# freudh/lbt

Measured on NVIDIA B200. Metric: quantized train imgs/sec, higher is better.
Workload: dtype s8/u8 mantissas, s32 accumulate (8-bit dfxp); fp32 master weights

## Files before the change

### include/lbt.h

```cpp
#ifndef LBT_H_
#define LBT_H_

#include <stddef.h>
#include <stdint.h>

#ifdef __cplusplus
extern "C" {
#endif

#define LBT_VERSION 100

enum lbt_status {
  LBT_OK = 0,
  LBT_EINVAL = -1,
  LBT_EUNSUPPORTED = -2,
  LBT_EARCH = -3,
  LBT_ECUDA = -4,
  LBT_EWORKSPACE = -5
};

enum lbt_round_mode {
  LBT_ROUND_NEAREST = 0,
  LBT_ROUND_STOCHASTIC_NOISE = 1,
  LBT_ROUND_STOCHASTIC_PHILOX = 2,
  LBT_STATS_MINMAX = 0x100
};

enum lbt_mant_kind {
  LBT_MANT_NONE = 0,
  LBT_MANT_S8 = 1,
  LBT_MANT_U8 = 2,
  LBT_MANT_S16 = 3,
  LBT_MANT_S9C3 = 4,
  LBT_MANT_PREPARED = 0x100
};

#define LBT_CNT_OVER 0
#define LBT_CNT_OVER_HALF 1
#define LBT_CNT_NUMEL 2
#define LBT_CNT_TICKET 3
#define LBT_CNT_WORDS 4

int lbt_version(void);
const char* lbt_strerror(int status);
const char* lbt_last_cuda_error(void);
uint64_t lbt_launch_count(void);

int lbt_quantize(const float* x, size_t n_outer, size_t n_inner, int bits, int32_t* integer_bits,
                 float target_overflow_rate, int mode, const float* noise, uint64_t seed,
                 uint64_t offset, const uint64_t* dev_step, float* out_fp32, void* out_mant,
                 int mant_kind, uint64_t* counters, int update_range, void* stream);

int lbt_noise_fill(float* u, size_t n_inner, uint64_t seed, uint64_t offset, const uint64_t* dev_step,
                   void* stream);

int lbt_update_ranges(int32_t* ranges, uint64_t* counters, const int32_t* bits, const float* target,
                      size_t n, void* stream);

int lbt_step_advance(uint64_t* dev_step, void* stream);

typedef struct lbt_qsite {
  int32_t bits;
  int32_t stats_minmax;
  const int32_t* ib;
  const float* noise;
  uint64_t seed, offset;
  const uint64_t* dev_step;
  uint64_t* counters;
} lbt_qsite;

enum lbt_gemm_epilogue {
  LBT_EPI_F32 = 0,
  LBT_EPI_ACC64 = 1
};

int lbt_gemm_i8(const void* A, int a_kind, size_t lda, const void* B, int b_kind, size_t ldb, size_t M,
                size_t N, size_t K, int epilogue, const int32_t* ibA, const int32_t* ibB, int exp_const,
                const float* bias, float* out_f32, int64_t* acc64, size_t ldc, int alpha, int k_splits,
                const lbt_qsite* q_out, int8_t* k_out, int64_t* sums, size_t rows_per_image, const float* addend,
                void* stream);

int lbt_gemm_i8_dual(const int8_t* A_hi, const uint8_t* A_lo, size_t lda, const void* B, int b_kind, size_t ldb, size_t M,
                     size_t N, size_t K, const int32_t* ibA, const int32_t* ibB, int exp_const, float* out_f32, size_t ldc,
                     const float* addend, void* stream);

int lbt_acc64_finalize(const int64_t* acc64, size_t n, const int32_t* ibA, const int32_t* ibB, int exp_const,
                       const float* add, float add_scale, float* out, void* stream);

int lbt_im2col_i8(const void* src, int src_kind, int N, int H, int W, int C, int OH, int OW, int kh, int kw,
                  int sh, int sw, int pad_top, int pad_left, int transposed, void* out, size_t ld,
                  void* stream);

int lbt_conv_i8_fprop(const void* src, int src_kind, int N, int H, int W, int C, const void* wp, int w_kind,
                      size_t ldw, int Cout, int kh, int kw, int sh, int sw, int pad_top, int pad_left, int OH,
                      int OW, const int32_t* ib_src, const int32_t* ib_w, int exp_const, const float* bias,
                      float* out, size_t ldc, const lbt_qsite* q_out, int8_t* k_out, int64_t* sums, const float* addend,
                      void* stream);

int lbt_conv_i8_fprop_dual(const int8_t* src_hi, const uint8_t* src_lo, int N, int H, int W, int C, const void* wp, int w_kind,
                           size_t ldw, int Cout, int kh, int kw, int pad_top, int pad_left, int OH, int OW,
                           const int32_t* ib_src, const int32_t* ib_w, int exp_const, float* out, size_t ldc,
                           const float* addend, void* stream);

int lbt_conv_i8_dgrad(const void* g, int g_kind, int N, int OH, int OW, int Cout, const void* wp, int w_kind,
                      size_t ldw, int Cin, int kh, int kw, int sh, int sw, int pad_top, int pad_left, int H, int W,
                      const int32_t* ib_g, const int32_t* ib_w, int exp_const, float* dx, size_t ldc, const float* addend,
                      void* stream);

int lbt_conv_i8_wgrad(const void* src, int src_kind, int N, int H, int W, int C, const void* g, int g_kind, int Cout,
                      int kh, int kw, int sh, int sw, int pad_top, int pad_left, int OH, int OW, int64_t* acc64,
                      int alpha, int k_splits, void* stream);

int lbt_conv_i8_wgrad_dual(const void* src, int src_kind, int N, int H, int W, int C, const int8_t* g_hi, const uint8_t* g_lo,
                           int Cout, int kh, int kw, int sh, int sw, int pad_top, int pad_left, int OH, int OW,
                           int64_t* acc64, int alpha, int k_splits, void* stream);

size_t lbt_stem_pack8_bytes(int N, int H, int OW);
int lbt_stem_pack8(const int8_t* x16, int N, int H, int W, int OW, int pad_left, int8_t* work8, void* stream);
int lbt_conv_i8_wgrad_c3(const int8_t* x16, int N, int H, int W, const void* g, int g_kind, int Cout, int kh, int kw,
                         int pad_top, int pad_left, int OH, int OW, int8_t* work8, int repack, int64_t* acc8, int alpha,
                         void* stream);

int lbt_split_s16(const int16_t* in, size_t n, int8_t* hi, uint8_t* lo, void* stream);

int lbt_transpose_i8(const void* in, size_t R, size_t C, size_t ld_in, void* out, size_t ld_out,
                     void* stream);

int lbt_colsum_i(const void* in, int kind, size_t R, size_t C, int64_t* acc64, void* stream);

typedef struct lbt_finalize_job {
  const int64_t* acc64;
  uint64_t n;
  const int32_t* ibA;
  const int32_t* ibB;
  int32_t exp_const;
  float add_scale;
  const float* add;
  float* out;
  uint64_t start;
} lbt_finalize_job;
int lbt_finalize_multi(const lbt_finalize_job* jobs_dev, size_t njobs, uint64_t total, void* stream);

typedef struct lbt_noise_job {
  float* u;
  uint64_t n;
  uint64_t offset;
  uint64_t start;
} lbt_noise_job;
int lbt_noise_fill_multi(const lbt_noise_job* jobs_dev, size_t njobs, uint64_t total_groups, uint64_t seed,
                         const uint64_t* dev_step, void* stream);

enum lbt_prep_layout { LBT_PREP_VECTOR = 0, LBT_PREP_CONV = 1, LBT_PREP_DENSE = 2 };
typedef struct lbt_prep_job {
  const float* x;
  uint64_t n_outer, n_inner;
  const int32_t* ib;
  uint64_t* counters;
  uint64_t offset;
  float* out_f32;
  int8_t* out_a;
  int8_t* out_b;
  uint64_t ld_a, ld_b;
  int32_t bits, layout;
  uint32_t kh, kw, Cin, Cout;
  int32_t c3pad, rot180;
  int32_t sh, sw;
} lbt_prep_job;
int lbt_param_prep(const lbt_prep_job* jobs_dev, const uint32_t* block_job_dev, const uint32_t* block_chunk_dev,
                   size_t nblocks, uint32_t chunk_elems, uint64_t seed, const uint64_t* dev_step, void* stream);

int lbt_sgd_momentum(float* w, float* accum, const float* grad, size_t n, float lr, const float* dev_lr,
                     float momentum, float grad_scale, void* stream);

int lbt_bn_fwd_quant_stats(const float* x, size_t n_outer, size_t n_inner, int C, int bits, const int32_t* ib,
                           const float* noise, uint64_t seed, uint64_t offset, const uint64_t* dev_step,
                           int8_t* k1, int64_t* sums, uint64_t* counters, int stats_minmax, void* stream);
int lbt_bn_fwd_apply(const int8_t* k1, size_t n_outer, size_t n_inner, int C, int bits1, const int32_t* ib1,
                     const int64_t* sums, float eps, int bits2, const int32_t* ib2, const float* noise2,
                     uint64_t seed, uint64_t offset2, const uint64_t* dev_step, uint64_t* counters2,
                     const float* gamma_q, const float* beta_q, const float* add, int relu, int8_t* k2,
                     float* out, float* batch_mean, float* batch_var, float* run_mean, float* run_var,
                     double momentum, int stats_minmax, const lbt_qsite* q_next, void* next_mant, int next_kind,
                     void* stream);
int lbt_bn_fwd_apply2(const int8_t* k1, size_t n_outer, size_t n_inner, int C, int bits1, const int32_t* ib1,
                      const int64_t* sums, float eps, int bits2, const int32_t* ib2, const float* noise2,
                      uint64_t seed, uint64_t offset2, const uint64_t* dev_step, uint64_t* counters2,
                      const float* gamma_q, const float* beta_q, const float* add, int relu, int8_t* k2,
                      float* out, float* batch_mean, float* batch_var, float* run_mean, float* run_var,
                      double momentum, int stats_minmax, const lbt_qsite* q_next, void* next_mant, int next_kind,
                      const lbt_qsite* q_next2, void* next_mant2, int next_kind2, void* stream);
int lbt_bn_fwd_apply_pooled(const int8_t* k1, size_t n_outer, int H, int W, int C, int bits1, const int32_t* ib1,
                            const int64_t* sums, float eps, int bits2, const int32_t* ib2, const float* noise2,
                            uint64_t seed, uint64_t offset2, const uint64_t* dev_step, uint64_t* counters2,
                            const float* gamma_q, const float* beta_q, int relu, int8_t* k2, float* run_mean,
                            float* run_var, double momentum, int stats_minmax, int k, int s, int pad_top, int pad_left,
                            int POH, int POW, float* pooled, uint8_t* pidx, const lbt_qsite* q_next, void* next_mant,
                            int next_kind, void* stream);
int lbt_bn_fwd_apply_running(const int8_t* k1, size_t n_outer, size_t n_inner, int C, int bits1, const int32_t* ib1,
                             const float* run_mean, const float* run_var, float eps, int bits2, const int32_t* ib2,
                             const float* noise2, uint64_t seed, uint64_t offset2, const uint64_t* dev_step,
                             uint64_t* counters2, const float* gamma_q, const float* beta_q, const float* add, int relu,
                             int8_t* k2, float* out, int stats_minmax, const lbt_qsite* q_next, void* next_mant,
                             int next_kind, const lbt_qsite* q_next2, void* next_mant2, int next_kind2, void* stream);
int lbt_bn_fwd_apply_running_pooled(const int8_t* k1, size_t n_outer, int H, int W, int C, int bits1, const int32_t* ib1,
                                    const float* run_mean, const float* run_var, float eps, int bits2, const int32_t* ib2,
                                    const float* noise2, uint64_t seed, uint64_t offset2, const uint64_t* dev_step,
                                    uint64_t* counters2, const float* gamma_q, const float* beta_q, int relu, int8_t* k2,
                                    int stats_minmax, int k, int s, int pad_top, int pad_left, int POH, int POW,
                                    float* pooled, uint8_t* pidx, const lbt_qsite* q_next, void* next_mant, int next_kind,
                                    void* stream);
int lbt_bn_bwd_quant_stats(const float* g, const float* out, int relu, const int8_t* k2, const int8_t* k1,
                           size_t n_outer, size_t n_inner, int C, int bits2, const int32_t* ib2,
                           const float* gamma_q, const float* beta_q, int bits_g2, const int32_t* ib_g2,
                           const float* noise_g2, uint64_t offset_g2, uint64_t* counters_g2, int bits_g1,
                           const int32_t* ib_g1, const float* noise_g1, uint64_t offset_g1,
                           uint64_t* counters_g1, uint64_t seed, const uint64_t* dev_step, float* d_add,
                           void* kg1, int64_t* sums, int stats_minmax, int kg1_kind, void* stream);
typedef struct lbt_pool_geom {
  const uint8_t* idx;
  int32_t H, W;
  int32_t k, s, pad_top, pad_left;
  int32_t OH, OW;
} lbt_pool_geom;
int lbt_bn_bwd_quant_stats_pooled(const float* g_pooled, const lbt_pool_geom* pool, int relu, const int8_t* k2,
                                  const int8_t* k1, size_t n_outer, size_t n_inner, int C, int bits2, const int32_t* ib2,
                                  const float* gamma_q, const float* beta_q, int bits_g2, const int32_t* ib_g2,
                                  const float* noise_g2, uint64_t offset_g2, uint64_t* counters_g2, int bits_g1,
                                  const int32_t* ib_g1, const float* noise_g1, uint64_t offset_g1,
                                  uint64_t* counters_g1, uint64_t seed, const uint64_t* dev_step, void* kg1,
                                  int64_t* sums, int stats_minmax, int kg1_kind, void* stream);
int lbt_bn_bwd_apply(const void* kg1, const int8_t* k1, size_t n_outer, size_t n_inner, int C, int bits1,
                     const int32_t* ib1, const int64_t* fwd_sums, float eps, int bits_g1, const int32_t* ib_g1,
                     const int64_t* bwd_sums, float* dx, const lbt_qsite* q_grad, int8_t* g_mant, int kg1_kind,
                     uint8_t* g_mant_lo, void* stream);

typedef struct lbt_bn_bwd_args {
  const float* g;
  const float* out;
  const int8_t* k2;
  const int8_t* k1;
  uint64_t n_outer, n_inner;
  int32_t C, relu;
  int32_t bits2, bits1;
  const int32_t* ib2;
  const int32_t* ib1;
  const float* gamma_q;
  const float* beta_q;
  lbt_qsite q_g2, q_g1;
  float* d_add;
  int64_t* bwd_sums;
  const int64_t* fwd_sums;
  float eps;
  int32_t has_q_grad;
  lbt_qsite q_grad;
  float* dx;
  int8_t* g_mant;
  uint64_t* barrier;
} lbt_bn_bwd_args;
int lbt_bn_bwd_fused(const lbt_bn_bwd_args* args, void* stream);

int lbt_maxpool_fwd(const float* x, int N, int H, int W, int C, int k, int s, int pad_top, int pad_left, int OH, int OW,
                    float* out, uint8_t* idx, void* stream);
int lbt_maxpool_bwd(const float* g, const uint8_t* idx, int N, int H, int W, int C, int k, int s, int pad_top,
                    int pad_left, int OH, int OW, float* dx, void* stream);

int lbt_avgpool_fwd(const float* x, int N, int H, int W, int C, int k, int s, int OH, int OW, float* out, void* stream);
int lbt_avgpool_bwd(const float* g, int N, int H, int W, int C, int k, int s, int OH, int OW, float* dx, void* stream);

int lbt_softmax_xent_fwd(const float* logits, const int64_t* labels, int B, int C, float* probs, float* loss, void* stream);
int lbt_softmax_xent_bwd(const float* probs, const int64_t* labels, const float* grad_loss, int B, int C, float* dlogits,
                         void* stream);

int lbt_relu(const float* x, const float* g, float* out, size_t n, void* stream);
int lbt_dropout(const float* x, const float* u, float keep_prob, uint64_t seed, uint64_t offset, const uint64_t* dev_step,
                float* out, size_t n, void* stream);

#define LBT_DP_MAX_WORLD 8
#define LBT_DP_PAD_READY 0
#define LBT_DP_PAD_DONE 8
#define LBT_DP_PAD_EPOCH 16
#define LBT_DP_PAD_TICKET 17
#define LBT_DP_PAD_ERROR 18
#define LBT_DP_PAD_WORDS 32
#define LBT_DP_HANDLE_BYTES 64
typedef struct lbt_dp_peers {
  int32_t world, rank;
  const float* grad[LBT_DP_MAX_WORLD];
  float* w[LBT_DP_MAX_WORLD];
  const uint64_t* counters[LBT_DP_MAX_WORLD];
  uint32_t* pad[LBT_DP_MAX_WORLD];
} lbt_dp_peers;
int lbt_dp_step(const lbt_dp_peers* peers, float* accum, size_t n, float lr, const float* dev_lr, float momentum,
                int shard, int32_t* ranges, const int32_t* bits, const float* target, size_t n_sites, uint64_t* dev_step,
                void* stream);
int lbt_dp_export(const void* ptr, void* handle64, size_t* offset);
int lbt_dp_open(const void* handle64, void** base);
int lbt_dp_close(void* base);

int lbt_augment_batch(const uint8_t* src, const double* mean, const int64_t* index, int B, int H, int W, int C, int pad,
                      int do_flip, const int32_t* params, uint64_t seed, uint64_t offset, const int64_t* labels,
                      int64_t* labels_out, float* out, void* stream);

int lbt_quantize_residual(const float* grad, size_t n_grad_rows, float* buffer, size_t n_outer, size_t n_inner, int bits,
                          int32_t* integer_bits, int mode, const float* noise, uint64_t seed, uint64_t offset,
                          const uint64_t* dev_step, float* out, uint64_t* counters, void* stream);

typedef struct lbt_bn_bwd_link {
  lbt_qsite q_g2, q_g1;
  int32_t bits2, relu;
  const int32_t* ib2;
  const float* gamma_q;
  const float* beta_q;
  const int8_t* k2;
  const int8_t* k1;
  int8_t* kg1;
  int64_t* sums;
} lbt_bn_bwd_link;
int lbt_conv_i8_dgrad_bn(const void* g, int g_kind, int N, int H, int W, int C, const void* wp, int w_kind, size_t ldw, int Cout,
                         int kh, int kw, int pad_top, int pad_left, int OH, int OW, const int32_t* ib_g, const int32_t* ib_w,
                         int exp_const, const lbt_bn_bwd_link* link, void* stream);

int lbt_conv_i8_dgrad_strided(const void* g, int g_kind, int N, int OH, int OW, int Cout, const void* w2, int w_kind, size_t ldw,
                              int Cin, int kh, int kw, int sh, int sw, int pad_top, int pad_left, int H, int W,
                              const int32_t* ib_g, const int32_t* ib_w, int exp_const, float* dx, size_t ldc,
                              const float* addend, void* stream);
int lbt_conv_i8_dgrad_strided_dual(const int8_t* g_hi, const uint8_t* g_lo, int N, int OH, int OW, int Cout, const void* w2,
                                   int w_kind, size_t ldw, int Cin, int kh, int kw, int sh, int sw, int pad_top, int pad_left,
                                   int H, int W, const int32_t* ib_g, const int32_t* ib_w, int exp_const, float* dx, size_t ldc,
                                   const float* addend, void* stream);

#ifdef __cplusplus
}
#endif
#endif
```

### lbt_b200/_lib.py

```python
import ctypes
import os

import torch

_HERE = os.path.dirname(os.path.abspath(__file__))
LIB_PATH = os.environ.get('LBT_LIB') or os.path.join(_HERE, 'liblbt_b200.so')

c_void_p, c_int, c_size_t, c_float = ctypes.c_void_p, ctypes.c_int, ctypes.c_size_t, ctypes.c_float
c_u64, c_char_p = ctypes.c_uint64, ctypes.c_char_p

SIGNATURES = {
    'lbt_version': (c_int, []),
    'lbt_strerror': (c_char_p, [c_int]),
    'lbt_last_cuda_error': (c_char_p, []),
    'lbt_launch_count': (c_u64, []),
    'lbt_quantize': (c_int, [c_void_p, c_size_t, c_size_t, c_int, c_void_p, c_float, c_int, c_void_p, c_u64, c_u64,
                             c_void_p, c_void_p, c_void_p, c_int, c_void_p, c_int, c_void_p]),
    'lbt_noise_fill': (c_int, [c_void_p, c_size_t, c_u64, c_u64, c_void_p, c_void_p]),
    'lbt_update_ranges': (c_int, [c_void_p, c_void_p, c_void_p, c_void_p, c_size_t, c_void_p]),
    'lbt_step_advance': (c_int, [c_void_p, c_void_p]),
    'lbt_gemm_i8': (c_int, [c_void_p, c_int, c_size_t, c_void_p, c_int, c_size_t, c_size_t, c_size_t, c_size_t, c_int,
                            c_void_p, c_void_p, c_int, c_void_p, c_void_p, c_void_p, c_size_t, c_int, c_int,
                            c_void_p, c_void_p, c_void_p, c_size_t, c_void_p, c_void_p]),
    'lbt_gemm_i8_dual': (c_int, [c_void_p, c_void_p, c_size_t, c_void_p, c_int, c_size_t, c_size_t, c_size_t, c_size_t, c_void_p,
                                 c_void_p, c_int, c_void_p, c_size_t, c_void_p, c_void_p]),
    'lbt_acc64_finalize': (c_int, [c_void_p, c_size_t, c_void_p, c_void_p, c_int, c_void_p, c_float, c_void_p,
                                   c_void_p]),
    'lbt_im2col_i8': (c_int, [c_void_p, c_int] + [c_int] * 13 + [c_void_p, c_size_t, c_void_p]),
    'lbt_conv_i8_fprop': (c_int, [c_void_p, c_int, c_int, c_int, c_int, c_int, c_void_p, c_int, c_size_t] + [c_int] * 9 +
                          [c_void_p, c_void_p, c_int, c_void_p, c_void_p, c_size_t, c_void_p, c_void_p, c_void_p, c_void_p,
                           c_void_p]),
    'lbt_conv_i8_fprop_dual': (c_int, [c_void_p, c_void_p, c_int, c_int, c_int, c_int, c_void_p, c_int, c_size_t] + [c_int] * 7 +
                               [c_void_p, c_void_p, c_int, c_void_p, c_size_t, c_void_p, c_void_p]),
    'lbt_conv_i8_dgrad': (c_int, [c_void_p, c_int, c_int, c_int, c_int, c_int, c_void_p, c_int, c_size_t] + [c_int] * 9 +
                          [c_void_p, c_void_p, c_int, c_void_p, c_size_t, c_void_p, c_void_p]),
    'lbt_conv_i8_wgrad': (c_int, [c_void_p, c_int, c_int, c_int, c_int, c_int, c_void_p, c_int] + [c_int] * 9 +
                          [c_void_p, c_int, c_int, c_void_p]),
    'lbt_conv_i8_wgrad_dual': (c_int, [c_void_p, c_int, c_int, c_int, c_int, c_int, c_void_p, c_void_p] + [c_int] * 9 +
                               [c_void_p, c_int, c_int, c_void_p]),
    'lbt_stem_pack8_bytes': (c_size_t, [c_int, c_int, c_int]),
    'lbt_stem_pack8': (c_int, [c_void_p, c_int, c_int, c_int, c_int, c_int, c_void_p, c_void_p]),
    'lbt_conv_i8_wgrad_c3': (c_int, [c_void_p, c_int, c_int, c_int, c_void_p] + [c_int] * 8 + [c_void_p, c_int, c_void_p, c_int, c_void_p]),
    'lbt_split_s16': (c_int, [c_void_p, c_size_t, c_void_p, c_void_p, c_void_p]),
    'lbt_transpose_i8': (c_int, [c_void_p, c_size_t, c_size_t, c_size_t, c_void_p, c_size_t, c_void_p]),
    'lbt_colsum_i': (c_int, [c_void_p, c_int, c_size_t, c_size_t, c_void_p, c_void_p]),
    'lbt_bn_bwd_fused': (c_int, [c_void_p, c_void_p]),
    'lbt_maxpool_fwd': (c_int, [c_void_p] + [c_int] * 10 + [c_void_p, c_void_p, c_void_p]),
    'lbt_maxpool_bwd': (c_int, [c_void_p, c_void_p] + [c_int] * 10 + [c_void_p, c_void_p]),
    'lbt_avgpool_fwd': (c_int, [c_void_p] + [c_int] * 8 + [c_void_p, c_void_p]),
    'lbt_avgpool_bwd': (c_int, [c_void_p] + [c_int] * 8 + [c_void_p, c_void_p]),
    'lbt_softmax_xent_fwd': (c_int, [c_void_p, c_void_p, c_int, c_int, c_void_p, c_void_p, c_void_p]),
    'lbt_softmax_xent_bwd': (c_int, [c_void_p, c_void_p, c_void_p, c_int, c_int, c_void_p, c_void_p]),
    'lbt_relu': (c_int, [c_void_p, c_void_p, c_void_p, c_size_t, c_void_p]),
    'lbt_dropout': (c_int, [c_void_p, c_void_p, c_float, c_u64, c_u64, c_void_p, c_void_p, c_size_t, c_void_p]),
    'lbt_sgd_momentum': (c_int, [c_void_p, c_void_p, c_void_p, c_size_t, c_float, c_void_p, c_float, c_float,
                                 c_void_p]),
    'lbt_finalize_multi': (c_int, [c_void_p, c_size_t, c_u64, c_void_p]),
    'lbt_noise_fill_multi': (c_int, [c_void_p, c_size_t, c_u64, c_u64, c_void_p, c_void_p]),
    'lbt_param_prep': (c_int, [c_void_p, c_void_p, c_void_p, c_size_t, ctypes.c_uint32, c_u64, c_void_p, c_void_p]),
    'lbt_bn_fwd_quant_stats': (c_int, [c_void_p, c_size_t, c_size_t, c_int, c_int, c_void_p, c_void_p, c_u64, c_u64,
                                       c_void_p, c_void_p, c_void_p, c_void_p, c_int, c_void_p]),
    'lbt_bn_fwd_apply': (c_int, [c_void_p, c_size_t, c_size_t, c_int, c_int, c_void_p, c_void_p, c_float, c_int,
                                 c_void_p, c_void_p, c_u64, c_u64, c_void_p, c_void_p, c_void_p, c_void_p, c_void_p,
                                 c_int, c_void_p, c_void_p, c_void_p, c_void_p, c_void_p, c_void_p, ctypes.c_double, c_int,
                                 c_void_p, c_void_p, c_int, c_void_p]),
    'lbt_bn_fwd_apply2': (c_int, [c_void_p, c_size_t, c_size_t, c_int, c_int, c_void_p, c_void_p, c_float, c_int,
                                  c_void_p, c_void_p, c_u64, c_u64, c_void_p, c_void_p, c_void_p, c_void_p, c_void_p,
                                  c_int, c_void_p, c_void_p, c_void_p, c_void_p, c_void_p, c_void_p, ctypes.c_double, c_int,
                                  c_void_p, c_void_p, c_int, c_void_p, c_void_p, c_int, c_void_p]),
    'lbt_bn_fwd_apply_pooled': (c_int, [c_void_p, c_size_t, c_int, c_int, c_int, c_int, c_void_p, c_void_p, c_float, c_int,
                                        c_void_p, c_void_p, c_u64, c_u64, c_void_p, c_void_p, c_void_p, c_void_p, c_int,
                                        c_void_p, c_void_p, c_void_p, ctypes.c_double, c_int, c_int, c_int, c_int, c_int,
                                        c_int, c_int, c_void_p, c_void_p, c_void_p, c_void_p, c_int, c_void_p]),
    'lbt_bn_fwd_apply_running': (c_int, [c_void_p, c_size_t, c_size_t, c_int, c_int, c_void_p, c_void_p, c_void_p, c_float, c_int,
                                         c_void_p, c_void_p, c_u64, c_u64, c_void_p, c_void_p, c_void_p, c_void_p, c_void_p, c_int,
                                         c_void_p, c_void_p, c_int, c_void_p, c_void_p, c_int, c_void_p, c_void_p, c_int, c_void_p]),
    'lbt_bn_fwd_apply_running_pooled': (c_int, [c_void_p, c_size_t, c_int, c_int, c_int, c_int, c_void_p, c_void_p, c_void_p,
                                                c_float, c_int, c_void_p, c_void_p, c_u64, c_u64, c_void_p, c_void_p, c_void_p,
                                                c_void_p, c_int, c_void_p, c_int, c_int, c_int, c_int, c_int, c_int, c_int,
                                                c_void_p, c_void_p, c_void_p, c_void_p, c_int, c_void_p]),
    'lbt_bn_bwd_quant_stats': (c_int, [c_void_p, c_void_p, c_int, c_void_p, c_void_p, c_size_t, c_size_t, c_int, c_int,
                                       c_void_p, c_void_p, c_void_p, c_int, c_void_p, c_void_p, c_u64, c_void_p, c_int,
                                       c_void_p, c_void_p, c_u64, c_void_p, c_u64, c_void_p, c_void_p, c_void_p,
                                       c_void_p, c_int, c_int, c_void_p]),
    'lbt_bn_bwd_quant_stats_pooled': (c_int, [c_void_p, c_void_p, c_int, c_void_p, c_void_p, c_size_t, c_size_t, c_int, c_int,
                                              c_void_p, c_void_p, c_void_p, c_int, c_void_p, c_void_p, c_u64, c_void_p, c_int,
                                              c_void_p, c_void_p, c_u64, c_void_p, c_u64, c_void_p, c_void_p,
                                              c_void_p, c_int, c_int, c_void_p]),
    'lbt_bn_bwd_apply': (c_int, [c_void_p, c_void_p, c_size_t, c_size_t, c_int, c_int, c_void_p, c_void_p, c_float,
                                 c_int, c_void_p, c_void_p, c_void_p, c_void_p, c_void_p, c_int, c_void_p, c_void_p]),
    'lbt_conv_i8_dgrad_strided_dual': (c_int, [c_void_p, c_void_p, c_int, c_int, c_int, c_int, c_void_p, c_int, c_size_t] + [c_int] * 9 +
                                       [c_void_p, c_void_p, c_int, c_void_p, c_size_t, c_void_p, c_void_p]),
    'lbt_conv_i8_dgrad_strided': (c_int, [c_void_p, c_int, c_int, c_int, c_int, c_int, c_void_p, c_int, c_size_t, c_int, c_int, c_int,
                                          c_int, c_int, c_int, c_int, c_int, c_int, c_void_p, c_void_p, c_int, c_void_p, c_size_t,
                                          c_void_p, c_void_p]),
    'lbt_dp_step': (c_int, [c_void_p, c_void_p, c_size_t, c_float, c_void_p, c_float, c_int, c_void_p, c_void_p, c_void_p,
                            c_size_t, c_void_p, c_void_p]),
    'lbt_dp_export': (c_int, [c_void_p, c_void_p, c_void_p]),
    'lbt_dp_open': (c_int, [c_void_p, c_void_p]),
    'lbt_dp_close': (c_int, [c_void_p]),
    'lbt_conv_i8_dgrad_bn': (c_int, [c_void_p, c_int, c_int, c_int, c_int, c_int, c_void_p, c_int, c_size_t] + [c_int] * 7 +
                             [c_void_p, c_void_p, c_int, c_void_p, c_void_p]),
    'lbt_quantize_residual': (c_int, [c_void_p, c_size_t, c_void_p, c_size_t, c_size_t, c_int, c_void_p, c_int, c_void_p, c_u64,
                                      c_u64, c_void_p, c_void_p, c_void_p, c_void_p]),
    'lbt_augment_batch': (c_int, [c_void_p, c_void_p, c_void_p, c_int, c_int, c_int, c_int, c_int, c_int, c_void_p, c_u64, c_u64,
                                  c_void_p, c_void_p, c_void_p, c_void_p]),
}

_INTERNAL = {
    'lbt_quantize_tune': (c_int, [c_int, c_int]),
    'lbt_gemm_debug_error': (c_int, []),
    'lbt_conv_debug_error': (c_int, []),
    'lbt_conv_ldg_debug_error': (c_int, []),
    'lbt_conv_set_path': (c_int, [c_int]),
    'lbt_conv_set_halo': (c_int, [c_int]),
    'lbt_conv_halo_launches': (ctypes.c_longlong, []),
    'lbt_gemm_set_pair': (c_int, [c_int]),
    'lbt_set_pdl': (c_int, [c_int]),
    'lbt_set_carveout': (c_int, [c_int]),
    'lbt_test_fdiv': (c_int, [c_u64, c_u64, c_void_p, c_void_p, c_void_p]),
    'lbt_bn_set_debug': (c_int, [c_void_p]),
    'lbt_conv_ldg_set_debug': (c_int, [c_void_p]),
    'lbt_dp_tune': (c_int, [c_int]),
    'lbt_dp_emulate_scratch_bytes': (c_size_t, [c_int]),
    'lbt_dp_step_emulate': (c_int, [c_int, c_void_p, c_void_p, c_size_t, c_float, c_void_p, c_float, c_int, c_void_p, c_void_p,
                                    c_void_p, c_size_t, c_void_p, c_void_p, c_void_p]),
    'lbt_bn_debug_error': (c_int, []),
}


class LbtError(RuntimeError):
    pass


class FinalizeJob(ctypes.Structure):
    _fields_ = [('acc64', c_void_p), ('n', c_u64), ('ibA', c_void_p), ('ibB', c_void_p), ('exp_const', ctypes.c_int32),
                ('add_scale', c_float), ('add', c_void_p), ('out', c_void_p), ('start', c_u64)]


class QSiteStruct(ctypes.Structure):
    _fields_ = [('bits', ctypes.c_int32), ('stats_minmax', ctypes.c_int32), ('ib', c_void_p), ('noise', c_void_p),
                ('seed', c_u64), ('offset', c_u64), ('dev_step', c_void_p), ('counters', c_void_p)]


class PoolGeom(ctypes.Structure):
    _fields_ = [('idx', c_void_p), ('H', ctypes.c_int32), ('W', ctypes.c_int32), ('k', ctypes.c_int32), ('s', ctypes.c_int32),
                ('pad_top', ctypes.c_int32), ('pad_left', ctypes.c_int32), ('OH', ctypes.c_int32), ('OW', ctypes.c_int32)]


class BnBwdLink(ctypes.Structure):
    _fields_ = [('q_g2', QSiteStruct), ('q_g1', QSiteStruct), ('bits2', ctypes.c_int32), ('relu', ctypes.c_int32), ('ib2', c_void_p),
                ('gamma_q', c_void_p), ('beta_q', c_void_p), ('k2', c_void_p), ('k1', c_void_p), ('kg1', c_void_p), ('sums', c_void_p)]


class BnBwdArgs(ctypes.Structure):
    _fields_ = [('g', c_void_p), ('out', c_void_p), ('k2', c_void_p), ('k1', c_void_p), ('n_outer', c_u64), ('n_inner', c_u64),
                ('C', ctypes.c_int32), ('relu', ctypes.c_int32), ('bits2', ctypes.c_int32), ('bits1', ctypes.c_int32),
                ('ib2', c_void_p), ('ib1', c_void_p), ('gamma_q', c_void_p), ('beta_q', c_void_p), ('q_g2', QSiteStruct),
                ('q_g1', QSiteStruct), ('d_add', c_void_p), ('bwd_sums', c_void_p), ('fwd_sums', c_void_p), ('eps', c_float),
                ('has_q_grad', ctypes.c_int32), ('q_grad', QSiteStruct), ('dx', c_void_p), ('g_mant', c_void_p),
                ('barrier', c_void_p)]


DP_MAX_WORLD, DP_PAD_WORDS, DP_PAD_ERROR, DP_HANDLE_BYTES = 8, 32, 18, 64


class DpPeers(ctypes.Structure):
    _fields_ = [('world', ctypes.c_int32), ('rank', ctypes.c_int32), ('grad', c_void_p * DP_MAX_WORLD),
                ('w', c_void_p * DP_MAX_WORLD), ('counters', c_void_p * DP_MAX_WORLD), ('pad', c_void_p * DP_MAX_WORLD)]


class NoiseJob(ctypes.Structure):
    _fields_ = [('u', c_void_p), ('n', c_u64), ('offset', c_u64), ('start', c_u64)]


class PrepJob(ctypes.Structure):
    _fields_ = [('x', c_void_p), ('n_outer', c_u64), ('n_inner', c_u64), ('ib', c_void_p), ('counters', c_void_p),
                ('offset', c_u64), ('out_f32', c_void_p), ('out_a', c_void_p), ('out_b', c_void_p), ('ld_a', c_u64),
                ('ld_b', c_u64), ('bits', ctypes.c_int32), ('layout', ctypes.c_int32), ('kh', ctypes.c_uint32),
                ('kw', ctypes.c_uint32), ('Cin', ctypes.c_uint32), ('Cout', ctypes.c_uint32), ('c3pad', ctypes.c_int32),
                ('rot180', ctypes.c_int32), ('sh', ctypes.c_int32), ('sw', ctypes.c_int32)]


def to_device_table(structs, device, keep=None):
    arr = (type(structs[0]) * len(structs))(*structs)
    host = torch.frombuffer(bytearray(bytes(arr)), dtype=torch.uint8).pin_memory()
    if keep is not None:
        keep.append(host)
    return host.to(device, non_blocking=True)


_lib = None


def lib():
    global _lib
    if _lib is None:
        if not os.path.exists(LIB_PATH):
            raise LbtError('%s not found — build it with `python -m lbt_b200.build` (needs nvcc); '
                           'there is no CPU or PyTorch fallback for the DFXP hot path' % LIB_PATH)
        h = ctypes.CDLL(LIB_PATH)
        for table in (SIGNATURES, _INTERNAL):
            for name, (res, args) in table.items():
                fn = getattr(h, name)
                fn.restype, fn.argtypes = res, args
        _lib = h
    return _lib


def check(status):
    if status != 0:
        h = lib()
        msg = h.lbt_strerror(status).decode()
        if status == -4:
            msg += ': ' + h.lbt_last_cuda_error().decode()
        raise LbtError('liblbt_b200: %s (status %d)' % (msg, status))


class Profiler:

    def __init__(self, external=False):
        self.records = []
        self.keep = []
        self.external = external

    def event(self):
        return torch.cuda.Event(enable_timing=True, external=True) if self.external else torch.cuda.Event(enable_timing=True)

    def summary(self):
        torch.cuda.synchronize()
        out = {}
        for name, a, b, meta in self.records:
            d = out.setdefault(name, dict(launches=0, ms=0.0, bytes=0, ops=0))
            d['launches'] += 1
            d['ms'] += a.elapsed_time(b)
            d['bytes'] += (meta or {}).get('bytes', 0)
            d['ops'] += (meta or {}).get('ops', 0)
        return out


profiler = None


def call(name, *args, meta=None):
    fn = getattr(lib(), name)
    if profiler is None:
        check(fn(*args))
        return
    a, b = profiler.event(), profiler.event()
    a.record()
    rc = fn(*args)
    b.record()
    profiler.records.append((name, a, b, meta))
    check(rc)


def try_call(name, *args, meta=None):
    fn = getattr(lib(), name)
    if profiler is None:
        rc = fn(*args)
    else:
        a, b = profiler.event(), profiler.event()
        a.record()
        rc = fn(*args)
        b.record()
        if rc == 0:
            profiler.records.append((name, a, b, meta))
        else:
            profiler.keep.append((a, b))
    if rc == -2:
        return False
    check(rc)
    return True


def ptr(t):
    if t is None:
        return None
    if not t.is_cuda:
        raise LbtError('lbt_b200 operates on CUDA tensors only (no CPU fallback); got a %s tensor' % t.device)
    return t.data_ptr()


def stream():
    return torch.cuda.current_stream().cuda_stream


def launch_count():
    return int(lib().lbt_launch_count())
```

### lbt_b200/csrc/conv_dgrad.cu

```cuda
#include "conv_classes.h"
#include "conv_internal.h"
#include "common.cuh"

namespace lbt {
namespace {

__global__ void __launch_bounds__(256) dgrad_fill_kernel(float* __restrict__ out, const float* __restrict__ addend, uint32_t Hc,
                                                          uint32_t Wc, uint32_t c4, long long sn, long long sy, long long sx,
                                                          size_t total) {
  pdl_trigger();
  pdl_wait();
  for (size_t i = (size_t)blockIdx.x * 256 + threadIdx.x; i < total; i += (size_t)gridDim.x * 256) {
    const uint32_t c = (uint32_t)(i % c4);
    size_t t = i / c4;
    const uint32_t x = (uint32_t)(t % Wc);
    t /= Wc;
    const uint32_t y = (uint32_t)(t % Hc), n = (uint32_t)(t / Hc);
    const long long o = (long long)n * sn + (long long)y * sy + (long long)x * sx + 4ll * c;
    const float4 v = addend ? __ldcs(reinterpret_cast<const float4*>(addend + o)) : make_float4(0.f, 0.f, 0.f, 0.f);
    *reinterpret_cast<float4*>(out + o) = v;
  }
}

}
}

using namespace lbt;

static int dgrad_strided_run(const void* g, int g_kind, const void* g_lo, int N, int OH, int OW, int Cout, const void* w2, int w_kind,
                             size_t ldw, int Cin, int kh, int kw, int sh, int sw, int pad_top, int pad_left, int H, int W,
                             const int32_t* ib_g, const int32_t* ib_w, int exp_const, float* dx, size_t ldc,
                             const float* addend, void* stream) {
  if (!g || !w2 || !dx) return LBT_EINVAL;
  if ((g_kind != LBT_MANT_S8 && g_kind != LBT_MANT_U8)) return LBT_EINVAL;
  if (g_lo && (g_kind != LBT_MANT_S8 || Cin < 64 || (Cout != 64 && Cout % 128))) return LBT_EUNSUPPORTED;
  if (N <= 0 || H <= 0 || W <= 0 || Cin <= 0 || Cout <= 0 || kh <= 0 || kw <= 0 || sh <= 0 || sw <= 0 || OH <= 0 || OW <= 0)
    return LBT_EINVAL;
  if (pad_top < 0 || pad_left < 0 || ldc < (size_t)Cin || ldw < (size_t)kh * kw * Cout) return LBT_EINVAL;
  if (sh > 4 || sw > 4 || (Cout & 15) || (Cin & 3) || (ldc & 3) || (reinterpret_cast<uintptr_t>(dx) & 15) ||
      (addend && (reinterpret_cast<uintptr_t>(addend) & 15)))
    return LBT_EUNSUPPORTED;
  for (int a = 0; a < sh; ++a) {
    const int r0 = (a + pad_top) % sh, nr = class_count(r0, kh, sh);
    if (nr && nr - 1 - (a + pad_top) / sh < 0) return LBT_EUNSUPPORTED;
  }
  for (int b = 0; b < sw; ++b) {
    const int s0 = (b + pad_left) % sw, nc = class_count(s0, kw, sw);
    if (nc && nc - 1 - (b + pad_left) / sw < 0) return LBT_EUNSUPPORTED;
  }
  LBT_REQUIRE_ARCH();
  cudaStream_t st = reinterpret_cast<cudaStream_t>(stream);
  for (int a = 0; a < sh && a < H; ++a)
    for (int b = 0; b < sw && b < W; ++b) {
      const int Hc = (H - a + sh - 1) / sh, Wc = (W - b + sw - 1) / sw;
      const int r0 = (a + pad_top) % sh, s0 = (b + pad_left) % sw;
      const int nr = class_count(r0, kh, sh), nc = class_count(s0, kw, sw);
      OutRemap rm{(long long)H * W * (long long)ldc, (long long)sh * W * (long long)ldc, (long long)sw * (long long)ldc};
      float* out = dx + ((size_t)a * W + b) * ldc;
      const float* ad = addend ? addend + ((size_t)a * W + b) * ldc : nullptr;
      if (nr == 0 || nc == 0) {
        const size_t total = (size_t)N * Hc * Wc * (Cin / 4);
        const size_t blocks = (total + 255) / 256, cap = (size_t)device_info().sm_count * 8;
        launch_pdl(dgrad_fill_kernel, (unsigned)(blocks < cap ? blocks : cap), 256, 0, st, out, ad, (uint32_t)Hc, (uint32_t)Wc,
                   (uint32_t)(Cin / 4), rm.sn, rm.sy, rm.sx, total);
        const int rc = check_launch("lbt_conv_i8_dgrad_strided (fill)");
        if (rc) return rc;
        continue;
      }
      const int pt2 = nr - 1 - (a + pad_top) / sh, pl2 = nc - 1 - (b + pad_left) / sw;
      const uint8_t* wp = reinterpret_cast<const uint8_t*>(w2) + (size_t)class_group_offset(r0, s0, kh, kw, sh, sw) * Cout;
      const int rc = conv_fprop_run(g, g_kind, N, OH, OW, Cout, wp, w_kind, ldw, Cin, nr, nc, 1, 1, pt2, pl2, Hc, Wc, ib_g, ib_w,
                                    exp_const, nullptr, out, ldc, nullptr, nullptr, nullptr, ad, stream, &rm, g_lo);
      if (rc) return rc;
    }
  return LBT_OK;
}

extern "C" int lbt_conv_i8_dgrad_strided(const void* g, int g_kind, int N, int OH, int OW, int Cout, const void* w2, int w_kind,
                                         size_t ldw, int Cin, int kh, int kw, int sh, int sw, int pad_top, int pad_left, int H, int W,
                                         const int32_t* ib_g, const int32_t* ib_w, int exp_const, float* dx, size_t ldc,
                                         const float* addend, void* stream) {
  return dgrad_strided_run(g, g_kind, nullptr, N, OH, OW, Cout, w2, w_kind, ldw, Cin, kh, kw, sh, sw, pad_top, pad_left, H, W, ib_g, ib_w,
                           exp_const, dx, ldc, addend, stream);
}

extern "C" int lbt_conv_i8_dgrad_strided_dual(const int8_t* g_hi, const uint8_t* g_lo, int N, int OH, int OW, int Cout, const void* w2,
                                              int w_kind, size_t ldw, int Cin, int kh, int kw, int sh, int sw, int pad_top, int pad_left,
                                              int H, int W, const int32_t* ib_g, const int32_t* ib_w, int exp_const, float* dx, size_t ldc,
                                              const float* addend, void* stream) {
  if (!g_lo) return LBT_EINVAL;
  return dgrad_strided_run(g_hi, LBT_MANT_S8, g_lo, N, OH, OW, Cout, w2, w_kind, ldw, Cin, kh, kw, sh, sw, pad_top, pad_left, H, W, ib_g,
                           ib_w, exp_const, dx, ldc, addend, stream);
}
```

### lbt_b200/csrc/conv_i8.cu

```cuda
#include "conv_internal.h"
#include "qsite.cuh"
#include "tcgen05.cuh"

namespace lbt {
namespace {

using namespace tc;

constexpr int kBlockM = 128;
constexpr int kStageK = 128;
constexpr int kThreads = 192;
constexpr int kEpiWarps = 8;
constexpr int kThreadsF = 32 * (2 + kEpiWarps);

__device__ int g_conv_error = 0;

struct ConvParams {
  uint32_t M, N;
  uint32_t OW, OHW;
  FastDiv d_OW, d_OHW;
  int lower_w, lower_h;
  int sw, sh;
  uint32_t kw;
  uint32_t taps, cchunks;
  uint32_t ksteps;
  uint32_t ksteps_real;
  uint32_t cb;
  uint32_t mode;
  uint32_t C;
  uint32_t m_tiles, n_tiles;
  const int32_t* ibA;
  const int32_t* ibB;
  int exp_const;
  const float* bias;
  const float* addend;
  float* out;
  size_t ldc;
  uint32_t idesc;
  uint32_t idesc2;
  BnqParams bnq;
  int remap;
  long long rs_n, rs_y, rs_x;
};

template <int BN>
struct Cfg {
  static constexpr int kStageA = kBlockM * kStageK;
  static constexpr int kStageB = BN * kStageK;
  static constexpr int kStageBytes = kStageA + kStageB;
  static constexpr int kCtasPerSm = BN <= 16 ? 3 : (BN <= 128 ? 2 : 1);
  static constexpr int kStages = BN <= 64 ? 4 : (BN == 128 ? 3 : 4);
  static constexpr int kSmemBytes = kStages * kStageBytes + 1024;
  static constexpr int kAccStages = BN <= 64 ? 4 : 2;
  static constexpr int kTmemCols = (kAccStages * BN) < 32 ? 32 : (kAccStages * BN);
  static_assert(kCtasPerSm * kSmemBytes <= 227 * 1024, "shared memory budget");
  static_assert(kCtasPerSm * kTmemCols <= 512, "tensor memory budget");
};

inline int ctas_per_sm(int bn) { return bn <= 16 ? 3 : (bn <= 128 ? 2 : 1); }

template <int BN, bool DUAL>
struct FCfg {
  static constexpr int kStageA = Cfg<BN>::kStageA;
  static constexpr int kStageB = Cfg<BN>::kStageB;
  static constexpr int kStageBytes = (DUAL ? 2 : 1) * kStageA + kStageB;
  static constexpr int kCtasPerSm = DUAL ? 1 : Cfg<BN>::kCtasPerSm;
  static constexpr int kStages = DUAL ? ((226 * 1024) / kStageBytes > 4 ? 4 : (226 * 1024) / kStageBytes) : Cfg<BN>::kStages;
  static constexpr int kSmemBytes = kStages * kStageBytes + 1024;
  static constexpr int kAccW = (DUAL ? 2 : 1) * BN;
  static constexpr int kAccStages = DUAL ? (512 / kAccW > 4 ? 4 : 512 / kAccW) : Cfg<BN>::kAccStages;
  static constexpr int kTmemCols = (kAccStages * kAccW) < 32 ? 32 : (kAccStages * kAccW);
  static_assert(kStages >= 2 && kAccStages >= 1, "fprop ring");
  static_assert(kCtasPerSm * kSmemBytes <= 227 * 1024, "shared memory budget");
  static_assert(kCtasPerSm * kTmemCols <= 512, "tensor memory budget");
};

template <int BN, bool DUAL>
struct WCfg {
  static constexpr int kStageA = Cfg<BN>::kStageA;
  static constexpr int kStageB1 = Cfg<BN>::kStageB;
  static constexpr int kStageBytes = kStageA + (DUAL ? 2 : 1) * kStageB1;
  static constexpr int kCtasPerSm = Cfg<BN>::kCtasPerSm;
  static constexpr int kBudget = (227 * 1024) / kCtasPerSm - 1024;
  static constexpr int kStages = !DUAL ? Cfg<BN>::kStages : (kBudget / kStageBytes > 4 ? 4 : kBudget / kStageBytes);
  static constexpr int kSmemBytes = kStages * kStageBytes + 1024;
  static constexpr int kAccW = (DUAL ? 2 : 1) * BN;
  static constexpr int kAccStages = !DUAL ? Cfg<BN>::kAccStages : ((512 / kCtasPerSm) / kAccW > 4 ? 4 : (512 / kCtasPerSm) / kAccW);
  static constexpr int kTmemCols = (kAccStages * kAccW) < 32 ? 32 : (kAccStages * kAccW);
  static_assert(kStages >= 2 && kAccStages >= 1, "wgrad ring");
  static_assert(kCtasPerSm * kSmemBytes <= 227 * 1024, "shared memory budget");
  static_assert(kCtasPerSm * kTmemCols <= 512, "tensor memory budget");
};

template <int BN, bool DUAL = false>
__global__ void __launch_bounds__(kThreadsF, FCfg<BN, DUAL>::kCtasPerSm)
conv_fprop_kernel(const __grid_constant__ CUtensorMap tmA, const __grid_constant__ CUtensorMap tmA2, const __grid_constant__ CUtensorMap tmB,
                  const ConvParams p) {
  using C = FCfg<BN, DUAL>;
  extern __shared__ uint8_t smem_raw[];
  uint8_t* smem = reinterpret_cast<uint8_t*>((reinterpret_cast<uintptr_t>(smem_raw) + 1023) & ~uintptr_t(1023));
  __shared__ __align__(8) uint64_t full_bar[C::kStages];
  __shared__ __align__(8) uint64_t empty_bar[C::kStages];
  __shared__ __align__(8) uint64_t tmem_full_bar[C::kAccStages];
  __shared__ __align__(8) uint64_t tmem_empty_bar[C::kAccStages];
  __shared__ uint32_t tmem_slot;
  __shared__ int s_abort;
  __shared__ int s_stat[kEpiWarps][2 * BN];
  __shared__ unsigned long long s_tot[2 * BN];

  const int warp = threadIdx.x >> 5, lane = threadIdx.x & 31;
  if (threadIdx.x == 0) {
    for (int s = 0; s < C::kStages; ++s) {
      mbar_init(&full_bar[s], 1);
      mbar_init(&empty_bar[s], 1);
    }
    for (int s = 0; s < C::kAccStages; ++s) {
      mbar_init(&tmem_full_bar[s], 1);
      mbar_init(&tmem_empty_bar[s], kEpiWarps);
    }
    s_abort = 0;
    fence_barrier_init();
    tma_prefetch_desc(&tmA);
    if (DUAL) tma_prefetch_desc(&tmA2);
    tma_prefetch_desc(&tmB);
  }
  if (warp == 1) tmem_alloc(&tmem_slot, C::kTmemCols);
  for (uint32_t i = threadIdx.x; i < 2 * BN; i += kThreadsF) s_tot[i] = 0ull;
  pdl_trigger();
  fence_before();
  __syncthreads();
  fence_after();
  pdl_wait();
  const uint32_t tmem_base = *reinterpret_cast<volatile uint32_t*>(&tmem_slot);
  volatile int* abort_flag = &s_abort;

  const uint32_t total_tiles = p.m_tiles * p.n_tiles;
  const uint32_t spb = kStageK / p.cb;
  const uint32_t a_block = kBlockM * p.cb, b_block = BN * p.cb;
  const uint32_t nstages_k = (p.ksteps + spb - 1) / spb;

  if (warp == 0) {
    if (lane == 0) {
      uint32_t stage = 0, phase = 0;
      bool ok = true;
      for (uint32_t tile = blockIdx.x; tile < total_tiles && ok; tile += gridDim.x) {
        const uint32_t m_tile = tile % p.m_tiles, n_tile = tile / p.m_tiles;
        const uint32_t m0 = m_tile * kBlockM;
        const uint32_t img = fastdiv(m0, p.d_OHW), rem = m0 - img * p.OHW;
        const uint32_t ohu = fastdiv(rem, p.d_OW);
        const int oh = (int)ohu, ow = (int)(rem - ohu * p.OW);
        const int base_w = p.lower_w + ow * p.sw, base_h = p.lower_h + oh * p.sh;
        uint32_t cc = 0, r = 0, s = 0;
        for (uint32_t ks = 0; ks < nstages_k; ++ks) {
          if (!(ok = mbar_wait(&empty_bar[stage], phase ^ 1, abort_flag, &g_conv_error))) break;
          uint8_t* sa = smem + stage * C::kStageBytes;
          uint8_t* sb = sa + (DUAL ? 2 : 1) * C::kStageA;
          const uint32_t k0 = ks * spb;
          const uint32_t nblk = min(spb, p.ksteps - k0);
          mbar_expect_tx(&full_bar[stage], nblk * ((DUAL ? 2u : 1u) * a_block + b_block));
          for (uint32_t j = 0; j < nblk; ++j) {
            const uint32_t kstep = k0 + j;
            const bool pad = kstep >= p.ksteps_real;
            tma_load_im2col_4d(&tmA, &full_bar[stage], sa + j * a_block, pad ? 0 : (int)(cc * p.cb), base_w, base_h, (int)img,
                               (uint16_t)(pad ? 0u : s), (uint16_t)(pad ? 0u : r));
            if (DUAL)
              tma_load_im2col_4d(&tmA2, &full_bar[stage], sa + C::kStageA + j * a_block, pad ? 0 : (int)(cc * p.cb), base_w, base_h,
                                 (int)img, (uint16_t)(pad ? 0u : s), (uint16_t)(pad ? 0u : r));
            tma_load_2d(&tmB, &full_bar[stage], sb + j * b_block, (int)(kstep * p.cb), (int)(n_tile * BN));
            if (++cc == p.cchunks) {
              cc = 0;
              if (++s == p.kw) {
                s = 0;
                ++r;
              }
            }
          }
          if (++stage == C::kStages) {
            stage = 0;
            phase ^= 1;
          }
        }
      }
    }
  } else if (warp == 1) {
    if (lane == 0) {
      uint32_t stage = 0, phase = 0, acc = 0, acc_phase = 0;
      bool ok = true;
      for (uint32_t tile = blockIdx.x; tile < total_tiles && ok; tile += gridDim.x) {
        if (!(ok = mbar_wait(&tmem_empty_bar[acc], acc_phase ^ 1, abort_flag, &g_conv_error))) break;
        fence_after();
        const uint32_t d_tmem = tmem_base + acc * C::kAccW;
        uint32_t first = 1;
        for (uint32_t ks = 0; ks < nstages_k; ++ks) {
          if (!(ok = mbar_wait(&full_bar[stage], phase, abort_flag, &g_conv_error))) break;
          fence_after();
          const uint32_t sa = smem_u32(smem + stage * C::kStageBytes);
          const uint32_t sb = sa + (DUAL ? 2 : 1) * C::kStageA;
          const uint32_t nblk = min(spb, p.ksteps - ks * spb);
          if (p.mode == 0) {
            for (uint32_t j = 0; j < nblk; j += 2) {
              const uint64_t db = make_desc_kmajor(sb + j * b_block, 0, b_block);
              umma_i8(d_tmem, make_desc_kmajor(sa + j * a_block, 0, a_block), db, p.idesc, first ? 0u : 1u);
              if (DUAL) umma_i8(d_tmem + BN, make_desc_kmajor(sa + C::kStageA + j * a_block, 0, a_block), db, p.idesc2, first ? 0u : 1u);
              first = 0;
            }
          } else {
            const uint32_t per_block = p.cb / 32;
            for (uint32_t j = 0; j < nblk; ++j)
              for (uint32_t kk = 0; kk < per_block; ++kk) {
                const uint64_t db = make_desc_kmajor(sb + j * b_block + kk * 32, (int)p.mode, 16);
                umma_i8(d_tmem, make_desc_kmajor(sa + j * a_block + kk * 32, (int)p.mode, 16), db, p.idesc, first ? 0u : 1u);
                if (DUAL)
                  umma_i8(d_tmem + BN, make_desc_kmajor(sa + C::kStageA + j * a_block + kk * 32, (int)p.mode, 16), db, p.idesc2,
                          first ? 0u : 1u);
                first = 0;
              }
          }
          umma_commit(&empty_bar[stage]);
          if (++stage == C::kStages) {
            stage = 0;
            phase ^= 1;
          }
        }
        if (!ok) break;
        umma_commit(&tmem_full_bar[acc]);
        if (++acc == C::kAccStages) {
          acc = 0;
          acc_phase ^= 1;
        }
      }
    }
  } else {
    const uint32_t quad = warp & 3;
    const uint32_t half = (uint32_t)(warp - 2) >> 2;
    int e = p.exp_const;
    if (p.ibA) e += *p.ibA;
    if (p.ibB) e += *p.ibB;
    const float scale = exp2i(e);
    const bool fused = p.bnq.q.bits != 0;
    int* my_stat = s_stat[warp - 2];
    BnqState bst;
    bst.tiles = 0;
    uint32_t stat_ntile = 0;
    if (fused) {
      bst.init(p.bnq);
      for (int i = lane; i < 2 * BN; i += 32) my_stat[i] = 0;
      __syncwarp();
    }
    uint32_t acc = 0, acc_phase = 0;
    bool ok = true;
    for (uint32_t tile = blockIdx.x; tile < total_tiles && ok; tile += gridDim.x) {
      const uint32_t m_tile = tile % p.m_tiles, n_tile = tile / p.m_tiles;
      const uint32_t row = m_tile * kBlockM + quad * 32 + lane;
      const uint32_t pix = fused ? row % p.bnq.rows_per_image : 0u;
      const uint32_t col0 = n_tile * BN;
      if (fused) {
#pragma unroll 1
        for (int c = (BN > 16 ? 16 * (int)half : 0); c < BN; c += (BN > 16 ? 32 : 16))
          bnq_prefetch(p.bnq, pix, p.N, col0 + (uint32_t)c, row < p.M && col0 + (uint32_t)c < p.N && !(BN == 16 && half));
      }
      ok = mbar_wait(&tmem_full_bar[acc], acc_phase, abort_flag, &g_conv_error);
      ok = __all_sync(0xffffffffu, ok);
      if (!ok) break;
      fence_after();
      const uint32_t taddr = tmem_base + acc * C::kAccW + ((quad * 32u) << 16);
      if (fused && (n_tile != stat_ntile || bst.tiles >= (uint32_t)kBnqFlushTiles)) {
        bnq_flush(p.bnq, my_stat, stat_ntile * BN, BN, p.N, lane);
        stat_ntile = n_tile;
        bst.tiles = 0;
      }
#pragma unroll 1
      for (int c = (BN > 16 ? 16 * (int)half : 0); c < BN; c += (BN > 16 ? 32 : 16)) {
        if (BN == 16 && half) break;
        uint32_t v[16];
        float4 u4[4];
        const bool fchunk = fused && col0 + c < p.N;
        if (BN > 16 && fchunk) bnq_load_noise(p.bnq, bst, pix, row < p.M, col0 + c, min(16u, p.N - (col0 + c)), p.N, u4);
        tmem_ld16(taddr + c, v);
        uint32_t w[DUAL ? 16 : 1];
        if constexpr (DUAL) tmem_ld16(taddr + BN + c, w);
        tmem_ld_wait();
        if (BN <= 16 && fchunk)
          bnq_load_noise(p.bnq, bst, pix, row < p.M, col0 + c, min(16u, p.N - (col0 + c)), p.N, u4);
        if (fused) {
          if (fchunk) {
            const uint32_t ncol = min(16u, p.N - (col0 + c));
            bnq_chunk(p.bnq, bst, v, u4, scale, p.bias ? p.bias + col0 + c : nullptr, row, row < p.M, col0 + c, ncol, p.N, my_stat, BN,
                      (uint32_t)c, lane);
          }
        } else if (row < p.M && col0 + c < p.N) {
          const uint32_t ncol = min(16u, p.N - (col0 + c));
          float* o;
          if (p.remap) {
            const uint32_t img = fastdiv(row, p.d_OHW), rem = row - img * p.OHW;
            const uint32_t oh = fastdiv(rem, p.d_OW), ow = rem - oh * p.OW;
            o = p.out + ((long long)img * p.rs_n + (long long)oh * p.rs_y + (long long)ow * p.rs_x) + col0 + c;
          } else {
            o = p.out + (size_t)row * p.ldc + col0 + c;
          }
          float f[16];
#pragma unroll
          for (int j = 0; j < 16; ++j) {
// ... 330 lines not shown
  if (!dual && !remap && conv_ldg_enabled() && (C <= 32 || (C == 64 && conv_ldg_c64_halo() && conv_ldg_halo_applies(N, OH, OW, kh, kw, sh, sw, C))) &&
      conv_ldg_ok(C, Cout, kh, kw) && !(reinterpret_cast<uintptr_t>(src) & 15) &&
      !(reinterpret_cast<uintptr_t>(wp) & 15) && !(ldw & 15) && ldw >= (size_t)kh * kw * C && (q_out || ldc >= (size_t)Cout)) {
    LBT_REQUIRE_ARCH();
    return conv_ldg_run(src, src_kind, N, H, W, C, wp, w_kind, ldw, Cout, kh, kw, sh, sw, pad_top, pad_left, OH, OW, 0, ib_src,
                        ib_w, exp_const, bias, out, ldc, q_out, k_out, sums, addend, stream, nullptr, w_prepared);
  }
  const uint32_t cb = C >= 128 ? 128u : (uint32_t)C;
  if (cb != 16 && cb != 32 && cb != 64 && cb != 128) return LBT_EUNSUPPORTED;
  if (C % cb) return LBT_EUNSUPPORTED;
  if ((reinterpret_cast<uintptr_t>(src) & 15) || (reinterpret_cast<uintptr_t>(wp) & 15) || (ldw & 15)) return LBT_EUNSUPPORTED;
  if (!q_out && ldc < (size_t)Cout) return LBT_EINVAL;
  const size_t Ktot = (size_t)kh * kw * C;
  if (ldw < Ktot) return LBT_EINVAL;
  if (conv_halo_applies(N, OH, OW, C, Cout, kh, kw, sh, sw)) {
    LBT_REQUIRE_ARCH();
    const int rc = conv_halo_run(src, src_kind, N, H, W, C, wp, w_kind, ldw, Cout, kh, kw, pad_top, pad_left, OH, OW, ib_src, ib_w,
                                 exp_const, bias, out, ldc, q_out, k_out, sums, addend, stream, remap, src_lo);
    if (!(dual && rc == LBT_EUNSUPPORTED)) return rc;
  }
  if (Ktot > 65536) return LBT_EUNSUPPORTED;
  if (kh > 255 || kw > 255) return LBT_EUNSUPPORTED;
  LBT_REQUIRE_ARCH();
  const DeviceInfo& di = device_info();
  static EncodeTiledFn enc_tiled = reinterpret_cast<EncodeTiledFn>(driver_fn("cuTensorMapEncodeTiled"));
  static EncodeIm2colFn enc_im2col = reinterpret_cast<EncodeIm2colFn>(driver_fn("cuTensorMapEncodeIm2col"));
  if (!enc_tiled || !enc_im2col) return LBT_ECUDA;

  int bn = 256;
  for (int c : {16, 32, 64, 128, 256})
    if (c >= Cout) {
      bn = c;
      break;
    }
  if (dual && bn > 128) bn = 128;
  if (dual && bn < 64) return LBT_EUNSUPPORTED;
  uint32_t mode = 0;
  while ((16u << mode) < cb) ++mode;

  ConvParams p{};
  p.M = (uint32_t)((size_t)N * OH * OW);
  p.N = (uint32_t)Cout;
  p.OW = (uint32_t)OW;
  p.OHW = (uint32_t)(OH * OW);
  p.d_OW = make_fastdiv(p.OW);
  p.d_OHW = make_fastdiv(p.OHW);
  if ((size_t)N * OH * OW >= (1ull << 31)) return LBT_EUNSUPPORTED;
  p.lower_w = -pad_left;
  p.lower_h = -pad_top;
  p.sw = sw;
  p.sh = sh;
  p.kw = (uint32_t)kw;
  p.taps = (uint32_t)(kh * kw);
  p.cchunks = (uint32_t)C / cb;
  p.ksteps_real = p.taps * p.cchunks;
  p.ksteps = p.ksteps_real + ((cb == 16 && (p.ksteps_real & 1)) ? 1 : 0);
  p.cb = cb;
  p.mode = mode;
  p.C = (uint32_t)C;
  p.m_tiles = (p.M + kBlockM - 1) / kBlockM;
  p.n_tiles = ((uint32_t)Cout + bn - 1) / bn;
  p.ibA = ib_src;
  p.ibB = ib_w;
  p.exp_const = exp_const;
  p.bias = bias;
  p.addend = q_out ? nullptr : addend;
  p.out = out;
  p.ldc = ldc;
  p.idesc = tc::make_idesc_i8(src_kind == LBT_MANT_S8, w_kind == LBT_MANT_S8, false, false, bn, kBlockM);
  p.idesc2 = tc::make_idesc_i8(false, w_kind == LBT_MANT_S8, false, false, bn, kBlockM);
  p.bnq.q = site_from_abi(q_out);
  p.bnq.k = k_out;
  p.bnq.sums = reinterpret_cast<long long*>(sums);
  p.bnq.rows_per_image = (uint32_t)(OH * OW);
  if (remap) {
    p.remap = 1;
    p.rs_n = remap->sn;
    p.rs_y = remap->sy;
    p.rs_x = remap->sx;
  }

  CUtensorMap ta, ta2, tb;
  {
    cuuint64_t gdim[4] = {(cuuint64_t)C, (cuuint64_t)W, (cuuint64_t)H, (cuuint64_t)N};
    cuuint64_t gstr[3] = {(cuuint64_t)C, (cuuint64_t)W * C, (cuuint64_t)H * W * C};
    const int upper_w = (OW - 1) * sw + 1 - W - pad_left;
    const int upper_h = (OH - 1) * sh + 1 - H - pad_top;
    int lower[2] = {-pad_left, -pad_top};
    int upper[2] = {upper_w, upper_h};
    cuuint32_t estr[4] = {1, (cuuint32_t)sw, (cuuint32_t)sh, 1};
    CUresult r = enc_im2col(&ta, CU_TENSOR_MAP_DATA_TYPE_UINT8, 4, const_cast<void*>(src), gdim, gstr, lower, upper, cb, kBlockM,
                            estr, CU_TENSOR_MAP_INTERLEAVE_NONE, swizzle_of(mode), CU_TENSOR_MAP_L2_PROMOTION_L2_128B,
                            CU_TENSOR_MAP_FLOAT_OOB_FILL_NONE);
    if (r != CUDA_SUCCESS) {
      set_cuda_error(cudaErrorInvalidValue, "cuTensorMapEncodeIm2col");
      return LBT_ECUDA;
    }
    ta2 = ta;
    if (dual) {
      r = enc_im2col(&ta2, CU_TENSOR_MAP_DATA_TYPE_UINT8, 4, const_cast<void*>(src_lo), gdim, gstr, lower, upper, cb, kBlockM,
                     estr, CU_TENSOR_MAP_INTERLEAVE_NONE, swizzle_of(mode), CU_TENSOR_MAP_L2_PROMOTION_L2_128B,
                     CU_TENSOR_MAP_FLOAT_OOB_FILL_NONE);
      if (r != CUDA_SUCCESS) {
        set_cuda_error(cudaErrorInvalidValue, "cuTensorMapEncodeIm2col(low plane)");
        return LBT_ECUDA;
      }
    }
  }
  {
    cuuint64_t gdim[2] = {(cuuint64_t)Ktot, (cuuint64_t)Cout};
    cuuint64_t gstr[1] = {(cuuint64_t)ldw};
    cuuint32_t box[2] = {cb, (cuuint32_t)bn};
    cuuint32_t estr[2] = {1, 1};
    CUresult r = enc_tiled(&tb, CU_TENSOR_MAP_DATA_TYPE_UINT8, 2, const_cast<void*>(wp), gdim, gstr, box, estr,
                           CU_TENSOR_MAP_INTERLEAVE_NONE, swizzle_of(mode), CU_TENSOR_MAP_L2_PROMOTION_L2_256B,
                           CU_TENSOR_MAP_FLOAT_OOB_FILL_NONE);
    if (r != CUDA_SUCCESS) {
      set_cuda_error(cudaErrorInvalidValue, "cuTensorMapEncodeTiled(weights)");
      return LBT_ECUDA;
    }
  }
  const uint64_t tiles = (uint64_t)p.m_tiles * p.n_tiles;
  const uint64_t cap = (uint64_t)di.sm_count * (dual ? 1 : ctas_per_sm(bn));
  const unsigned grid = (unsigned)(tiles < cap ? tiles : cap);
  cudaStream_t st = reinterpret_cast<cudaStream_t>(stream);
  if (dual) return bn == 64 ? launch<64, true>(ta, ta2, tb, p, grid, st) : launch<128, true>(ta, ta2, tb, p, grid, st);
  switch (bn) {
    case 16: return launch<16>(ta, ta2, tb, p, grid, st);
    case 32: return launch<32>(ta, ta2, tb, p, grid, st);
    case 64: return launch<64>(ta, ta2, tb, p, grid, st);
    case 128: return launch<128>(ta, ta2, tb, p, grid, st);
    default: return launch<256>(ta, ta2, tb, p, grid, st);
  }
}

namespace lbt {
namespace {
template <int BN, bool DUAL = false>
int launch_wgrad(const CUtensorMap& tx, const CUtensorMap& tg, const CUtensorMap& tg2, const WgradParams& p, unsigned grid, cudaStream_t st) {
  static bool attr_done[16] = {};
  const int dev = device_info().device;
  if (!attr_done[dev]) {
    cudaError_t e = cudaFuncSetAttribute(conv_wgrad_kernel<BN, DUAL>, cudaFuncAttributeMaxDynamicSharedMemorySize, WCfg<BN, DUAL>::kSmemBytes);
    if (e != cudaSuccess) {
      set_cuda_error(e, "cudaFuncSetAttribute(conv_wgrad_kernel)");
      return LBT_ECUDA;
    }
    attr_done[dev] = true;
  }
  launch_pdl(conv_wgrad_kernel<BN, DUAL>, grid, kThreads, WCfg<BN, DUAL>::kSmemBytes, st, tx, tg, tg2, p);
  return check_launch(DUAL ? "lbt_conv_i8_wgrad_dual" : "lbt_conv_i8_wgrad");
}
}
}

static int conv_wgrad_run(const void* src, int src_kind, int N, int H, int W, int C, const void* g, int g_kind, const void* g_lo, int Cout,
                          int kh, int kw, int sh, int sw, int pad_top, int pad_left, int OH, int OW, int64_t* acc64,
                          int alpha, int k_splits, void* stream) {
  const bool dual = g_lo != nullptr;
  if (!src || !g || !acc64) return LBT_EINVAL;
  if (dual && (g_kind != LBT_MANT_S8 || (reinterpret_cast<uintptr_t>(g_lo) & 15))) return LBT_EUNSUPPORTED;
  if ((src_kind != LBT_MANT_S8 && src_kind != LBT_MANT_U8) || (g_kind != LBT_MANT_S8 && g_kind != LBT_MANT_U8)) return LBT_EINVAL;
  if (N <= 0 || H <= 0 || W <= 0 || C <= 0 || Cout <= 0 || kh <= 0 || kw <= 0 || sh <= 0 || sw <= 0 || OH <= 0 || OW <= 0)
    return LBT_EINVAL;
  const uint32_t cb = C >= 128 ? 128u : (uint32_t)C;
  const uint32_t cbn = Cout >= 128 ? 128u : (uint32_t)Cout;
  if ((cb != 16 && cb != 32 && cb != 64 && cb != 128) || (C % cb)) return LBT_EUNSUPPORTED;
  if ((cbn != 16 && cbn != 32 && cbn != 64 && cbn != 128) || (Cout % cbn)) return LBT_EUNSUPPORTED;
  if ((reinterpret_cast<uintptr_t>(src) & 15) || (reinterpret_cast<uintptr_t>(g) & 15)) return LBT_EUNSUPPORTED;
  if (kh > 255 || kw > 255) return LBT_EUNSUPPORTED;
  LBT_REQUIRE_ARCH();
  if (!dual && conv_ldg_enabled() && k_splits <= 0 && C == 16 && Cout <= 16 && conv_wgrad_ldg_ok(C, Cout, kh, kw)) {
    const int rc = conv_wgrad_ldg_run(src, src_kind, N, H, W, C, g, g_kind, Cout, kh, kw, sh, sw, pad_top, pad_left, OH, OW, acc64,
                                      alpha, stream);
    if (rc != LBT_EUNSUPPORTED) return rc;
  }
  const DeviceInfo& di = device_info();
  static EncodeTiledFn enc_tiled = reinterpret_cast<EncodeTiledFn>(driver_fn("cuTensorMapEncodeTiled"));
  static EncodeIm2colFn enc_im2col = reinterpret_cast<EncodeIm2colFn>(driver_fn("cuTensorMapEncodeIm2col"));
  if (!enc_tiled || !enc_im2col) return LBT_ECUDA;

  int bn = Cout >= 256 ? 256 : Cout;
  if (Cout > 128 && Cout % 256) bn = 128;
  if (dual && bn > 128) bn = 128;
  uint32_t mode_a = 0, mode_b = 0;
  while ((16u << mode_a) < cb) ++mode_a;
  while ((16u << mode_b) < cbn) ++mode_b;

  WgradParams p{};
  p.Mpix = (uint32_t)((size_t)N * OH * OW);
  p.N = (uint32_t)Cout;
  p.OW = (uint32_t)OW;
  p.OHW = (uint32_t)(OH * OW);
  p.d_OW = make_fastdiv(p.OW);
  p.d_OHW = make_fastdiv(p.OHW);
  if ((size_t)N * OH * OW >= (1ull << 31)) return LBT_EUNSUPPORTED;
  p.lower_w = -pad_left;
  p.lower_h = -pad_top;
  p.sw = sw;
  p.sh = sh;
  p.kw = (uint32_t)kw;
  p.cchunks = (uint32_t)C / cb;
  p.ksteps = (uint32_t)(kh * kw) * p.cchunks;
  p.cb = cb;
  p.mode_a = mode_a;
  p.cbn = cbn;
  p.mode_b = mode_b;
  p.nchunks = (uint32_t)bn / cbn;
  const uint32_t spb = kStageK / cb;
  p.m_tiles = (p.ksteps + spb - 1) / spb;
  p.n_tiles = ((uint32_t)Cout + bn - 1) / bn;
  p.pix_blocks = (p.Mpix + kBlockM - 1) / kBlockM;
  uint32_t splits = k_splits > 0 ? (uint32_t)k_splits : 0;
  if (!splits) {
    const uint32_t tiles = p.m_tiles * p.n_tiles;
    splits = (uint32_t)(di.sm_count * ctas_per_sm(bn)) / (tiles ? tiles : 1);
    if (splits > p.pix_blocks / 8) splits = p.pix_blocks / 8;
    if (splits < 1) splits = 1;
  }
  if (splits > p.pix_blocks) splits = p.pix_blocks;
  p.blocks_per_split = (p.pix_blocks + splits - 1) / splits;
  if (p.blocks_per_split > 65536 / kBlockM) p.blocks_per_split = 65536 / kBlockM;
  p.k_splits = (p.pix_blocks + p.blocks_per_split - 1) / p.blocks_per_split;
  p.Kf = (uint32_t)(kh * kw * C);
  p.acc64 = reinterpret_cast<long long*>(acc64);
  p.alpha = alpha;
  p.idesc = tc::make_idesc_i8(src_kind == LBT_MANT_S8, g_kind == LBT_MANT_S8, true, true, bn, kBlockM);
  p.idesc2 = tc::make_idesc_i8(src_kind == LBT_MANT_S8, false, true, true, bn, kBlockM);

  CUtensorMap tx, tg, tg2;
  {
    cuuint64_t gdim[4] = {(cuuint64_t)C, (cuuint64_t)W, (cuuint64_t)H, (cuuint64_t)N};
    cuuint64_t gstr[3] = {(cuuint64_t)C, (cuuint64_t)W * C, (cuuint64_t)H * W * C};
    int lower[2] = {-pad_left, -pad_top};
    int upper[2] = {(OW - 1) * sw + 1 - W - pad_left, (OH - 1) * sh + 1 - H - pad_top};
    cuuint32_t estr[4] = {1, (cuuint32_t)sw, (cuuint32_t)sh, 1};
    CUresult r = enc_im2col(&tx, CU_TENSOR_MAP_DATA_TYPE_UINT8, 4, const_cast<void*>(src), gdim, gstr, lower, upper, cb, kBlockM,
                            estr, CU_TENSOR_MAP_INTERLEAVE_NONE, swizzle_of(mode_a), CU_TENSOR_MAP_L2_PROMOTION_L2_128B,
                            CU_TENSOR_MAP_FLOAT_OOB_FILL_NONE);
    if (r != CUDA_SUCCESS) {
      set_cuda_error(cudaErrorInvalidValue, "cuTensorMapEncodeIm2col(wgrad)");
      return LBT_ECUDA;
    }
  }
  {
    cuuint64_t gdim[2] = {(cuuint64_t)Cout, (cuuint64_t)p.Mpix};
    cuuint64_t gstr[1] = {(cuuint64_t)Cout};
    cuuint32_t box[2] = {cbn, (cuuint32_t)kBlockM};
    cuuint32_t estr[2] = {1, 1};
    CUresult r = enc_tiled(&tg, CU_TENSOR_MAP_DATA_TYPE_UINT8, 2, const_cast<void*>(g), gdim, gstr, box, estr,
                           CU_TENSOR_MAP_INTERLEAVE_NONE, swizzle_of(mode_b), CU_TENSOR_MAP_L2_PROMOTION_L2_128B,
                           CU_TENSOR_MAP_FLOAT_OOB_FILL_NONE);
    if (r != CUDA_SUCCESS) {
      set_cuda_error(cudaErrorInvalidValue, "cuTensorMapEncodeTiled(grad)");
      return LBT_ECUDA;
    }
    tg2 = tg;
    if (dual) {
      r = enc_tiled(&tg2, CU_TENSOR_MAP_DATA_TYPE_UINT8, 2, const_cast<void*>(g_lo), gdim, gstr, box, estr,
                    CU_TENSOR_MAP_INTERLEAVE_NONE, swizzle_of(mode_b), CU_TENSOR_MAP_L2_PROMOTION_L2_128B,
                    CU_TENSOR_MAP_FLOAT_OOB_FILL_NONE);
      if (r != CUDA_SUCCESS) {
        set_cuda_error(cudaErrorInvalidValue, "cuTensorMapEncodeTiled(grad, low plane)");
        return LBT_ECUDA;
      }
    }
  }
  const uint64_t items = (uint64_t)p.m_tiles * p.n_tiles * p.k_splits;
  const uint64_t cap = (uint64_t)di.sm_count * ctas_per_sm(bn);
  const unsigned grid = (unsigned)(items < cap ? items : cap);
  cudaStream_t st = reinterpret_cast<cudaStream_t>(stream);
  if (dual) {
    switch (bn) {
      case 16: return launch_wgrad<16, true>(tx, tg, tg2, p, grid, st);
      case 32: return launch_wgrad<32, true>(tx, tg, tg2, p, grid, st);
      case 64: return launch_wgrad<64, true>(tx, tg, tg2, p, grid, st);
      default: return launch_wgrad<128, true>(tx, tg, tg2, p, grid, st);
    }
  }
  switch (bn) {
    case 16: return launch_wgrad<16>(tx, tg, tg2, p, grid, st);
    case 32: return launch_wgrad<32>(tx, tg, tg2, p, grid, st);
    case 64: return launch_wgrad<64>(tx, tg, tg2, p, grid, st);
    case 128: return launch_wgrad<128>(tx, tg, tg2, p, grid, st);
    default: return launch_wgrad<256>(tx, tg, tg2, p, grid, st);
  }
}

extern "C" int lbt_conv_i8_wgrad(const void* src, int src_kind, int N, int H, int W, int C, const void* g, int g_kind, int Cout,
                                 int kh, int kw, int sh, int sw, int pad_top, int pad_left, int OH, int OW, int64_t* acc64,
                                 int alpha, int k_splits, void* stream) {
  return conv_wgrad_run(src, src_kind, N, H, W, C, g, g_kind, nullptr, Cout, kh, kw, sh, sw, pad_top, pad_left, OH, OW, acc64, alpha,
                        k_splits, stream);
}

extern "C" int lbt_conv_i8_wgrad_dual(const void* src, int src_kind, int N, int H, int W, int C, const int8_t* g_hi, const uint8_t* g_lo,
                                      int Cout, int kh, int kw, int sh, int sw, int pad_top, int pad_left, int OH, int OW,
                                      int64_t* acc64, int alpha, int k_splits, void* stream) {
  if (!g_lo) return LBT_EINVAL;
  return conv_wgrad_run(src, src_kind, N, H, W, C, g_hi, LBT_MANT_S8, g_lo, Cout, kh, kw, sh, sw, pad_top, pad_left, OH, OW, acc64,
                        alpha, k_splits, stream);
}

extern "C" int lbt_conv_debug_error(void) {
  int v = 0, zero = 0;
  if (cudaMemcpyFromSymbol(&v, g_conv_error, sizeof(int)) != cudaSuccess) return -1;
  cudaMemcpyToSymbol(g_conv_error, &zero, sizeof(int));
  const int h = conv_halo_debug_error();
  if (h > 0) v |= h;
  const int st = conv_stem_debug_error();
  if (st > 0) v |= st;
  return v;
}
```

### lbt_b200/csrc/conv_internal.h

```cpp
#pragma once

#include <stddef.h>
#include <stdint.h>

#include "../../include/lbt.h"

namespace lbt {

struct OutRemap {
  long long sn, sy, sx;
};

bool conv_ldg_ok(int C, int Cout, int kh, int kw);
bool conv_ldg_enabled();
bool conv_ldg_halo_applies(int N, int OH, int OW, int kh, int kw, int sh, int sw, int C);
int conv_ldg_c64_halo();
int conv_ldg_run(const void* src, int src_kind, int N, int SH, int SW, int C, const void* wp, int w_kind, size_t ldw, int Cout,
                 int kh, int kw, int sh, int sw, int pt, int pl, int OH, int OW, int gather, const int32_t* ibA,
                 const int32_t* ibB, int exp_const, const float* bias, float* out, size_t ldc, const lbt_qsite* q_out,
                 int8_t* k_out, int64_t* sums, const float* addend, void* stream, const lbt_bn_bwd_link* link = nullptr,
                 bool w_prepared = false);

bool conv_halo_applies(int N, int OH, int OW, int C, int Cout, int kh, int kw, int sh, int sw);
void conv_halo_enable(int mode);
int conv_halo_debug_error();
int conv_stem_debug_error();
int conv_halo_run(const void* src, int src_kind, int N, int H, int W, int C, const void* wp, int w_kind, size_t ldw, int Cout, int kh,
                  int kw, int pt, int pl, int OH, int OW, const int32_t* ibA, const int32_t* ibB, int exp_const, const float* bias,
                  float* out, size_t ldc, const lbt_qsite* q_out, int8_t* k_out, int64_t* sums, const float* addend, void* stream,
                  const OutRemap* remap = nullptr, const void* src_lo = nullptr);
int conv_fprop_run(const void* src, int src_kind, int N, int H, int W, int C, const void* wp, int w_kind, size_t ldw, int Cout, int kh,
                   int kw, int sh, int sw, int pad_top, int pad_left, int OH, int OW, const int32_t* ib_src, const int32_t* ib_w,
                   int exp_const, const float* bias, float* out, size_t ldc, const lbt_qsite* q_out, int8_t* k_out, int64_t* sums,
                   const float* addend, void* stream, const OutRemap* remap, const void* src_lo = nullptr);

bool conv_wgrad_ldg_ok(int C, int Cout, int kh, int kw);
int conv_wgrad_ldg_run(const void* src, int src_kind, int N, int H, int W, int C, const void* g, int g_kind, int Cout, int kh, int kw,
                       int sh, int sw, int pt, int pl, int OH, int OW, int64_t* acc64, int alpha, void* stream);

}
```

### lbt_b200/dfxp.py

```python
import contextlib
import ctypes
import os
import math

import torch
import torch.nn as nn

from . import _lib, gemm as G, quantizer as Q




class Runtime:

    def __init__(self, seed=0):
        self.seed = int(seed)
        self.sites = []
        self.dev_step = None
        self.noise_fn = None
        self.flat = None
        self.grad_sink = None
        self.prep = None
        self._arena = None
        self._arena_off = 0
# ... 287 lines not shown
            n_inner = Q.rows_view(x)[1]
            kw.update(mode=Q.ROUND_NOISE, noise=rt.noise_fn(self, n_inner, x.device))
        else:
            kw.update(mode=Q.ROUND_PHILOX, seed=rt.seed, offset=Q.make_offset(self.qid, 0), dev_step=rt.dev_step)
        if self.target == 0.0:
            kw['mode'] |= Q.STATS_MINMAX
        return Q.quantize(x, self.bits, self.range, **kw)

    def abi(self, n_inner, device, arena=False):
        rt = self.runtime
        qs = _lib.QSiteStruct(bits=self.bits, stats_minmax=int(self.target == 0.0), ib=self.range.data_ptr(),
                              noise=0, seed=rt.seed, offset=Q.make_offset(self.qid, 0),
                              dev_step=_lib.ptr(rt.dev_step) or 0, counters=self.counters.data_ptr())
        if rt.noise_fn is not None:
            nz = rt.noise_fn(self, n_inner, device).contiguous()
            qs.noise, qs.offset = nz.data_ptr(), 0
            qs._keep = nz
        elif arena:
            nz = rt.noise_for(self, n_inner, device)
            if nz is not None:
                qs.noise = nz.data_ptr()
        return qs

    def extra_repr(self):
        return '%s bits=%d' % (self.name, self.bits)


class _QuantSTE(torch.autograd.Function):

    @staticmethod
    def forward(ctx, x, site):
        q, _ = site.quantize(x)
        return q

    @staticmethod
    def backward(ctx, dy):
        return dy, None


class _GradQuant(torch.autograd.Function):

    @staticmethod
    def forward(ctx, y, site):
        ctx.site = site
        return y.view_as(y)

    @staticmethod
    def backward(ctx, dy):
        dy = _mem_contig(dy)
        q, _ = ctx.site.quantize(dy)
        return q, None


def _require_cuda_f32(x, who):
    if not x.is_cuda or x.dtype != torch.float32:
        raise _lib.LbtError('%s: expects an fp32 CUDA tensor (got %s on %s); there is no CPU or PyTorch fallback'
                            % (who, x.dtype, x.device))


def _mem_contig(x):
    if x.dim() == 4:
        return x if x.is_contiguous(memory_format=torch.channels_last) else x.contiguous(memory_format=torch.channels_last)
    return x.contiguous()


def same_pad(in_size, k, s):
    out = -(-in_size // s)
    total = max((out - 1) * s + k - in_size, 0)
    return out, total // 2, total - total // 2


def _pitch16(k):
    return -(-k // 16) * 16


def _as_operand(t):
    rows, K = t.shape
    if t.stride(1) == 1 and t.stride(0) % 16 == 0 and t.data_ptr() % 16 == 0:
        return t
    buf = torch.zeros(rows, _pitch16(K), dtype=t.dtype, device=t.device)
    buf[:, :K] = t
    return buf[:, :K]


def _transpose_bytes(t):
    R, C = t.shape
    assert t.stride(1) == 1
    out = torch.empty(C, _pitch16(R), dtype=t.dtype, device=t.device)
    _lib.call('lbt_transpose_i8', _lib.ptr(t), R, C, t.stride(0), _lib.ptr(out), out.stride(0), _lib.stream())
    return out[:, :R]


def _im2col(src_nhwc, src_kind, OH, OW, kh, kw, sh, sw, pt, pl, transposed):
    N, H, W, C = src_nhwc.shape
    segs = 3 if src_kind == Q.MANT_S16 else 1
    K = kh * kw * C * segs
    M = N * OH * OW
    out = torch.empty(M, _pitch16(K), dtype=torch.int8 if src_kind != Q.MANT_U8 else torch.uint8, device=src_nhwc.device)
    _lib.call('lbt_im2col_i8', _lib.ptr(src_nhwc), src_kind, N, H, W, C, OH, OW, kh, kw, sh, sw, pt, pl,
                                        1 if transposed else 0, _lib.ptr(out), out.stride(0), _lib.stream())
    return out[:, :K]


def _colsum(mant2d, kind, rt=None):
    acc = (rt.zeros_i64(mant2d.shape[1], mant2d.device) if rt is not None
           else torch.zeros(mant2d.shape[1], dtype=torch.int64, device=mant2d.device))
    _lib.call('lbt_colsum_i', _lib.ptr(mant2d), kind, mant2d.shape[0], mant2d.shape[1], _lib.ptr(acc),
                                       _lib.stream())
    return acc


def _implicit_ok(C, kh, kw):
    return (C in (16, 32, 64) or (C >= 128 and C % 128 == 0)) and kh * kw * C <= 65536 and kh <= 255 and kw <= 255


def _gather_ok(C, Cout, kh, kw):
    if C not in (16, 32, 64) or not 1 <= Cout <= 128:
        return False
    kcp = (kh * kw * (C // 16) + 1) & ~1
    bn = 16 if Cout <= 16 else (32 if Cout <= 32 else (64 if Cout <= 64 else 128))
    return kcp * bn * 16 + 2 * 16384 + 1024 <= 200 * 1024 and kh * kw * C <= 65536 and kcp <= 256 and kh * kw <= 64 and kh <= 16 and kw <= 16


def _class_perm(kh, kw, sh, sw):
    perm = []
    for r0 in range(sh):
        for s0 in range(sw):
            for r in reversed(range(r0, kh, sh)):
                for s_ in reversed(range(s0, kw, sw)):
                    perm.append(r * kw + s_)
    return perm


DGRAD_CLASSES = True


def _dgrad_classes_ok(layer, Cin, Cout, kh, kw, sh, sw):
    if layer.qG.bits > 8:
        return (DGRAD_CLASSES and DUAL_HALO and layer.implicit and (sh, sw) != (1, 1) and sh <= 4 and sw <= 4 and layer.qG.bits <= 16 and
                layer.qW.bits <= 8 and (Cout == 64 or Cout % 128 == 0) and Cin >= 64 and Cin % 4 == 0)
    return (DGRAD_CLASSES and layer.implicit and (sh, sw) != (1, 1) and sh <= 4 and sw <= 4 and layer.qG.bits <= 8 and
            layer.qW.bits <= 8 and (Cout in (16, 32, 64) or Cout % 128 == 0) and Cin % 4 == 0 and
            not _gather_ok(Cout, Cin, kh, kw))


FUSE_POOL_FWD = os.environ.get('LBT_FUSE_POOL_FWD', '1') != '0'

STEM_WGRAD = os.environ.get('LBT_STEM_WGRAD', '1') != '0'

_W_PREPARED = 0x100 if os.environ.get('LBT_W_PREFETCH', '0') == '1' else 0


def _conv_implicit(src_nhwc, src_kind, wp, Cout, kh, kw, sh, sw, pt, pl, OH, OW, ib_src, ib_w, exp_const, bias, out2d,
                   bnq=None, addend=None, w_prepared=False):
    N, H, W, C = src_nhwc.shape
    qs, k_out, sums = bnq if bnq is not None else (None, None, None)
    _lib.call('lbt_conv_i8_fprop', _lib.ptr(src_nhwc), src_kind, N, H, W, C, _lib.ptr(wp), Q.MANT_S8 | (_W_PREPARED if w_prepared else 0),
              wp.stride(0), Cout,
              kh, kw, sh, sw, pt, pl, OH, OW, _lib.ptr(ib_src), _lib.ptr(ib_w), int(exp_const), _lib.ptr(bias),
              _lib.ptr(out2d), out2d.stride(0) if out2d is not None else Cout,
              ctypes.addressof(qs) if qs is not None else None, _lib.ptr(k_out), _lib.ptr(sums), _lib.ptr(addend), _lib.stream(),
              meta=dict(ops=2 * N * OH * OW * Cout * kh * kw * C,
                        bytes=N * H * W * C + Cout * kh * kw * C + N * OH * OW * Cout * (1 if qs is not None else 4)))




def _conv_geom(layer, x, weight):
    N, Cin, H, W = x.shape
    kh, kw, _, Cout = weight.shape
    sh, sw = layer.stride
    if layer.padding == 'SAME':
        OH, pt, _ = same_pad(H, kh, sh)
        OW, pl, _ = same_pad(W, kw, sw)
    else:
        pt = pl = layer.pad_int
        OH = (H + 2 * pt - kh) // sh + 1
        OW = (W + 2 * pl - kw) // sw + 1
    return (N, H, W, Cin, Cout, kh, kw, sh, sw, pt, pl, OH, OW)


def _conv_xkind(layer, geom):
    N, H, W, Cin, Cout, kh, kw = geom[:7]
    xb = layer.qX.bits
    if layer.qW.bits > 8 or xb > 16:
        raise _lib.LbtError('Conv2d_q: weights wider than 8 bits need the hi/lo GEMM split (not built yet)')
    if xb <= 8:
        return Q.MANT_S8
    if xb <= 9 and not layer.input_signed:
        return Q.MANT_U8
    if xb <= 9 and Cin == 3 and layer.implicit and kh * kw * 16 <= 65536 and _implicit_ok(Cout, 1, 1):
        return Q.MANT_S9C3
    return Q.MANT_S16


def _conv_quantize_input(layer, x, geom):
    xkind = _conv_xkind(layer, geom)
    pre = getattr(x, '_lbt_q', None)
    if pre is not None and id(layer.qX) in pre:
        xm, kind = pre[id(layer.qX)]
        assert kind == xkind, (kind, xkind)
        return xm, xkind
    if getattr(x, '_lbt_hollow', False):
        raise _lib.LbtError('Conv2d_q: got a mantissa-only activation made for a different quantiser')
    N, H, W = geom[:3]
    x_nhwc = _mem_contig(x).permute(0, 2, 3, 1)
    if xkind == Q.MANT_S9C3:
        xm = torch.empty(N, H, W, 16, dtype=torch.int8, device=x.device)
        layer.qX.quantize(x_nhwc, want_fp32=False, mant_kind=xkind, out_mant=xm)
        return xm, xkind
    _, xm = layer.qX.quantize(x_nhwc, want_fp32=False, mant_kind=xkind)
    return xm, xkind


def _stem_applies(geom):
    N, H, W, Cin, Cout, kh, kw, sh, sw = geom[:9]
    return STEM_WGRAD and sh == 2 and sw == 2 and kh <= 8 and kw <= 8 and Cout == 64 and H % 2 == 0


def _stem_work(layer, geom, dev):
    N, H, OW = geom[0], geom[1], geom[12]
    nb = int(_lib.lib().lbt_stem_pack8_bytes(N, H, OW))
    work = getattr(layer, '_stem_work8', None)
    if work is None or work.numel() != nb or work.device != torch.device(dev):
        work = layer._stem_work8 = torch.empty(nb, dtype=torch.int8, device=dev)
        layer._stem_packed = False
    return work, nb


def _stem_prepack(layer, xm, xkind, geom):
    rt = layer.qX.runtime
    if (xkind != Q.MANT_S9C3 or not _stem_applies(geom) or not torch.is_grad_enabled() or not layer.weight.requires_grad or
            not (rt.overlap and rt._arena_on and rt.grad_sink is not None and rt.grad_sink.active and _lib.profiler is None)):
        return
    N, H, W = geom[:3]
    dev = xm.device
    work, _ = _stem_work(layer, geom, dev)
    main, side = torch.cuda.current_stream(dev), rt.side_stream(dev)
    side.wait_stream(main)
    with torch.cuda.stream(side):
        layer._stem_packed = _lib.try_call('lbt_stem_pack8', _lib.ptr(xm), N, H, W, geom[12], geom[10], _lib.ptr(work), _lib.stream(),
                                           meta=dict(bytes=N * H * W * 16 + work.numel()))
    xm.record_stream(side)
    rt._side_pending = True


def _flush_head_beside(rt, fork, main, side):
    sink = rt.grad_sink
    if sink is None or not sink.active:
        return
    if fork:
        ev = torch.cuda.Event()
        ev.record(side)
        with torch.cuda.stream(main):
            main.wait_event(ev)
            sink.flush_head()
    else:
        sink.flush_head()


def _conv_params(layer, weight, bias):
    if not weight.is_contiguous():
        weight = weight.contiguous()
    prep = _prepared(layer)
    bq = wm = None
    if prep is None:
        _, wm = layer.qW.quantize(weight, want_fp32=False, mant_kind=Q.MANT_S8)
        if bias is not None:
            bq, _ = layer.qb.quantize(bias)
    else:
        bq = prep.get('bq')
    return prep, wm, bq


def _conv_fprop(layer, geom, xm, xkind, prep, wm, bq, out2d, bnq=None):
    N, H, W, Cin, Cout, kh, kw, sh, sw, pt, pl, OH, OW = geom
    e = -(layer.qX.bits - 1) - (layer.qW.bits - 1)
    Kf = kh * kw * Cin
    ibx, ibw = layer.qX.range, layer.qW.range
    if xkind == Q.MANT_S9C3:
        if prep is not None:
            wt = prep['wt']
        else:
            w3 = wm.view(kh * kw, 3, Cout)
            w16 = torch.cat([w3, w3, w3, torch.zeros(kh * kw, 7, Cout, dtype=torch.int8, device=xm.device)], dim=1)
            wt = _transpose_bytes(w16.view(kh * kw * 16, Cout))
        _conv_implicit(xm, Q.MANT_S8, wt, Cout, kh, kw, sh, sw, pt, pl, OH, OW, ibx, ibw, e, bq, out2d, bnq, w_prepared=prep is not None)
        return
    segs = 3 if xkind == Q.MANT_S16 else 1
    wt = prep['wt'] if prep is not None else _transpose_bytes(wm.view(Kf, Cout))
    if segs == 3:
        wt = _as_operand(torch.cat([wt, wt, wt], dim=1))
    gbnq = None if bnq is None else (bnq[0], bnq[1], bnq[2], OH * OW)
    if kh == 1 and kw == 1 and sh == 1 and sw == 1 and segs == 1 and Cin % 16 == 0 and pt == 0 and pl == 0:
        G.gemm_i8(xm.reshape(N * H * W, Cin), wt, ibA=ibx, ibB=ibw, exp_const=e, bias=bq, out=out2d, bnq=gbnq)
    elif layer.implicit and segs == 1 and _implicit_ok(Cin, kh, kw):
        _conv_implicit(xm, xkind, wt, Cout, kh, kw, sh, sw, pt, pl, OH, OW, ibx, ibw, e, bq, out2d, bnq,
                       w_prepared=prep is not None)
    else:
        A = _im2col(xm, xkind, OH, OW, kh, kw, sh, sw, pt, pl, False)
        G.gemm_i8(A, wt, ibA=ibx, ibB=ibw, exp_const=e, bias=bq, out=out2d, bnq=gbnq)


def _conv_backward(layer, geom, xm, xkind, wm, prep, gm, need_dx, need_dw, need_db, addend=None, link=None):
    N, H, W, Cin, Cout, kh, kw, sh, sw, pt, pl, OH, OW = geom
    xb, wb, gb = layer.qX.bits, layer.qW.bits, layer.qG.bits
    dev = gm.device
    M = N * OH * OW
    g2 = gm.view(M, Cout)
    Kf = kh * kw * Cin
    dW = db = dx = None
    rt = layer.qX.runtime
    fork = need_dw and rt.overlap and rt._arena_on and rt.grad_sink is not None and rt.grad_sink.active and _lib.profiler is None
    main = torch.cuda.current_stream(dev) if fork else None
    side = rt.side_stream(dev) if fork else None
    if fork:
        side.wait_stream(main)
    if need_dw:
      with (torch.cuda.stream(side) if fork else contextlib.nullcontext()):
          acc = rt.zeros_i64(Kf * Cout, dev).view(Kf, Cout)
          at = gt = None
          if xkind == Q.MANT_S9C3:
              if not _implicit_ok(Cout, 1, 1):
                  raise _lib.LbtError('first-layer implicit wgrad needs Cout in {16,32,64} or a multiple of 128')
              done = False
              _flush_head_beside(rt, fork, main, side)
              if _stem_applies(geom):
                  work, nb = _stem_work(layer, geom, dev)
                  repack = 0 if getattr(layer, '_stem_packed', False) else 1
                  layer._stem_packed = False
                  acc8 = rt.zeros_i64(512 * Cout, dev)
                  done = _lib.try_call('lbt_conv_i8_wgrad_c3', _lib.ptr(xm), N, H, W, _lib.ptr(g2), Q.MANT_S8, Cout, kh, kw, pt, pl,
                                       OH, OW, _lib.ptr(work), repack, _lib.ptr(acc8), 1, _lib.stream(),
                                       meta=dict(ops=2 * M * Cout * Kf, bytes=N * H * W * 16 + nb + M * Cout + 8 * 512 * Cout))
                  if done:
                      a = acc8.view(8, 8, 8, Cout)[:kh, :kw]
                      acc = (2 * a[:, :, 0:3] + a[:, :, 4:7]).reshape(Kf, Cout).contiguous()
              if not done:
                  acc16 = rt.zeros_i64(kh * kw * 16 * Cout, dev).view(kh * kw * 16, Cout)
                  _lib.call('lbt_conv_i8_wgrad', _lib.ptr(xm), Q.MANT_S8, N, H, W, 16, _lib.ptr(g2), Q.MANT_S8, Cout, kh, kw,
                            sh, sw, pt, pl, OH, OW, _lib.ptr(acc16), 1, 0, _lib.stream(),
                            meta=dict(ops=2 * M * Cout * Kf, bytes=N * H * W * 16 + M * Cout + 8 * kh * kw * 16 * Cout))
                  a = acc16.view(kh * kw, 16, Cout)
                  acc = (a[:, 0:3] + a[:, 3:6] + a[:, 6:9]).reshape(Kf, Cout).contiguous()
          elif layer.implicit and xkind != Q.MANT_S16 and _implicit_ok(Cin, kh, kw) and _implicit_ok(Cout, 1, 1):
              _lib.call('lbt_conv_i8_wgrad', _lib.ptr(xm), xkind, N, H, W, Cin, _lib.ptr(g2), Q.MANT_S8, Cout, kh, kw,
                        sh, sw, pt, pl, OH, OW, _lib.ptr(acc), 1, 0, _lib.stream(),
                        meta=dict(ops=2 * M * Cout * Kf, bytes=N * H * W * Cin + M * Cout + 8 * Kf * Cout))
          else:
              gt = _transpose_bytes(g2)
              A = _im2col(xm, xkind, OH, OW, kh, kw, sh, sw, pt, pl, False)
              at = _transpose_bytes(A)
          if at is None:
              pass
          elif xkind == Q.MANT_S16:
              G.gemm_i8_acc64(at[:Kf], gt, acc, alpha=2)
              G.gemm_i8_acc64(at[2 * Kf:], gt, acc, alpha=1)
          else:
              G.gemm_i8_acc64(at, gt, acc, alpha=1)
          dW = _emit_grad(rt, layer.weight, acc, ibA=layer.qX.range, ibB=layer.qG.range, exp_const=-(xb - 1) - (gb - 1),
                          add_scale=2 * layer.weight_decay, shape=(kh, kw, Cin, Cout))
    if need_db:
        db = _emit_grad(rt, layer.bias, _colsum(g2, Q.MANT_S8, rt), ibA=layer.qG.range, exp_const=-(gb - 1))
    linked = False
    if (need_dx and link is not None and link.k1 is not None and addend is None and layer.implicit and sh == 1 and sw == 1 and
            kh * kw > 1 and _implicit_ok(Cout, kh, kw) and tuple(link.k1.shape) == (N, H, W, Cin)):
        K2 = kh * kw * Cout
        pw2 = prep['w2'] if prep is not None else None
        w2 = pw2 if pw2 is not None else _as_operand(wm.flip(0, 1).permute(2, 0, 1, 3).reshape(Cin, K2))
        rt = layer.qX.runtime
        kg1 = torch.empty_like(link.k1)
        bsums = rt.zeros_i64(4 * Cin + 2, dev)
        ls = link.struct(H * W * Cin, dev, kg1, bsums)
        linked = _lib.try_call('lbt_conv_i8_dgrad_bn', _lib.ptr(gm), Q.MANT_S8, N, OH, OW, Cout, _lib.ptr(w2),
                               Q.MANT_S8 | (_W_PREPARED if pw2 is not None else 0), w2.stride(0), Cin, kh, kw, kh - 1 - pt, kw - 1 - pl, H, W, _lib.ptr(layer.qG.range),
                               _lib.ptr(layer.qW.range), int(-(gb - 1) - (wb - 1)), ctypes.addressof(ls), _lib.stream(),
                               meta=dict(ops=2 * N * H * W * Cin * K2, bytes=N * OH * OW * Cout + Cin * K2 + 3 * N * H * W * Cin))
        if linked:
            global _link_count
            _link_count += 1
            link.kg1, link.bsums, link.done = kg1, bsums, True
            dx = torch.empty(1, dtype=torch.float32, device=dev).expand(N, H, W, Cin)
    if need_dx and not linked:
        K2 = kh * kw * Cout
        dx = torch.empty(N, H, W, Cin, dtype=torch.float32, device=dev)
        ad2 = addend.reshape(N * H * W, Cin) if addend is not None else None
        e = -(gb - 1) - (wb - 1)
        pw2 = prep['w2'] if prep is not None else None
        if prep is not None and pw2 is None:
            raise _lib.LbtError('Conv2d_q: no input gradient for a 3-channel first-layer convolution')
        if kh == 1 and kw == 1 and sh == 1 and sw == 1 and Cout % 16 == 0 and pt == 0 and pl == 0:
            w2 = pw2 if pw2 is not None else _as_operand(wm.view(Cin, Cout))
            G.gemm_i8(g2, w2, ibA=layer.qG.range, ibB=layer.qW.range, exp_const=e, out=dx.view(N * H * W, Cin), addend=ad2)
        elif layer.implicit and sh == 1 and sw == 1 and _implicit_ok(Cout, kh, kw):
            w2 = pw2 if pw2 is not None else _as_operand(wm.flip(0, 1).permute(2, 0, 1, 3).reshape(Cin, K2))
            _conv_implicit(gm, Q.MANT_S8, w2, Cin, kh, kw, 1, 1, kh - 1 - pt, kw - 1 - pl, H, W, layer.qG.range,
                           layer.qW.range, e, None, dx.view(N * H * W, Cin), addend=ad2, w_prepared=pw2 is not None)
        elif layer.implicit and _gather_ok(Cout, Cin, kh, kw) and sh <= 4 and sw <= 4:
            w2 = pw2 if pw2 is not None else _as_operand(wm.view(kh * kw, Cin, Cout).permute(1, 0, 2).reshape(Cin, K2))
            _lib.call('lbt_conv_i8_dgrad', _lib.ptr(gm), Q.MANT_S8, N, OH, OW, Cout, _lib.ptr(w2),
                      Q.MANT_S8 | (_W_PREPARED if pw2 is not None else 0), w2.stride(0),
                      Cin, kh, kw, sh, sw, pt, pl, H, W, _lib.ptr(layer.qG.range), _lib.ptr(layer.qW.range), int(e),
                      _lib.ptr(dx), Cin, _lib.ptr(ad2), _lib.stream(),
                      meta=dict(ops=2 * N * H * W * Cin * K2, bytes=N * OH * OW * Cout + Cin * K2 + N * H * W * Cin * 4))
        elif (prep['classes'] if prep is not None else _dgrad_classes_ok(layer, Cin, Cout, kh, kw, sh, sw)):
            if pw2 is not None:
                w2 = pw2
            else:
                perm = torch.tensor(_class_perm(kh, kw, sh, sw), device=dev)
                w2 = _as_operand(wm.view(kh * kw, Cin, Cout).index_select(0, perm).permute(1, 0, 2).reshape(Cin, K2))
            _lib.call('lbt_conv_i8_dgrad_strided', _lib.ptr(gm), Q.MANT_S8, N, OH, OW, Cout, _lib.ptr(w2),
                      Q.MANT_S8 | (_W_PREPARED if pw2 is not None else 0), w2.stride(0),
                      Cin, kh, kw, sh, sw, pt, pl, H, W, _lib.ptr(layer.qG.range), _lib.ptr(layer.qW.range), int(e),
                      _lib.ptr(dx), Cin, _lib.ptr(ad2), _lib.stream(),
                      meta=dict(ops=2 * N * OH * OW * Cin * K2, bytes=N * OH * OW * Cout * min(sh * sw, kh * kw) + Cin * K2 + N * H * W * Cin * 4))
        else:
            w2 = pw2 if pw2 is not None else _as_operand(wm.view(kh * kw, Cin, Cout).permute(1, 0, 2).reshape(Cin, K2))
            A2 = _im2col(gm, Q.MANT_S8, H, W, kh, kw, sh, sw, pt, pl, True)
            G.gemm_i8(A2, w2, ibA=layer.qG.range, ibB=layer.qW.range, exp_const=e, out=dx.view(N * H * W, Cin), addend=ad2)
    if fork:
        for t in (xm, gm):
            t.record_stream(side)
        rt._side_pending = True
    return dx, dW, db


def _check_layer_bits(who, bits, grad_bits):
    if not 2 <= int(bits) <= 8:
        raise _lib.LbtError('%s: bits=%d — the integer tensor-core layers take 2..8-bit weights/activations '
                            '(gradients up to 16 bits via grad_bits); wider DFXP only through weight_quantization()' % (who, bits))
    if grad_bits is not None and not 2 <= int(grad_bits) <= 16:
        raise _lib.LbtError('%s: grad_bits=%d — gradient quantisers take 2..16 bits' % (who, grad_bits))


def _split16(gm16):
    hi = torch.empty(gm16.shape, dtype=torch.int8, device=gm16.device)
    lo = torch.empty(gm16.shape, dtype=torch.uint8, device=gm16.device)
    _lib.call('lbt_split_s16', _lib.ptr(gm16), gm16.numel(), _lib.ptr(hi), _lib.ptr(lo), _lib.stream(),
              meta=dict(bytes=gm16.numel() * 4))
    return hi, lo


def _conv_backward16(layer, geom, xm, xkind, wm, prep, hi, lo, need_dx, need_dw, need_db, gm16=None, addend=None):
    N, H, W, Cin, Cout, kh, kw, sh, sw, pt, pl, OH, OW = geom
    xb, wb, gb = layer.qX.bits, layer.qW.bits, layer.qG.bits
    dev = hi.device
    M = N * OH * OW
    Kf = kh * kw * Cin
    rt = layer.qX.runtime
    halves = ((hi, Q.MANT_S8, 256), (lo, Q.MANT_U8, 1))
    dW = db = dx = None
    fork = need_dw and rt.overlap and rt._arena_on and rt.grad_sink is not None and rt.grad_sink.active and _lib.profiler is None
    main = torch.cuda.current_stream(dev) if fork else None
    side = rt.side_stream(dev) if fork else None
    if fork:
        side.wait_stream(main)
    if need_dw:
      with (torch.cuda.stream(side) if fork else contextlib.nullcontext()):
        acc = rt.zeros_i64(Kf * Cout, dev).view(Kf, Cout)
        if xkind == Q.MANT_S9C3:
            if not _implicit_ok(Cout, 1, 1):
                raise _lib.LbtError('first-layer implicit wgrad needs Cout in {16,32,64} or a multiple of 128')
            done = False
            _flush_head_beside(rt, fork, main, side)
            if _stem_applies(geom):
                work, nb = _stem_work(layer, geom, dev)
                repack = 0 if getattr(layer, '_stem_packed', False) else 1
                layer._stem_packed = False
                acc8 = rt.zeros_i64(512 * Cout, dev)
                done = True
                for i, (g_, kind, alpha) in enumerate(halves):
                    done = done and _lib.try_call('lbt_conv_i8_wgrad_c3', _lib.ptr(xm), N, H, W, _lib.ptr(g_), kind, Cout, kh, kw, pt,
                                                  pl, OH, OW, _lib.ptr(work), repack if i == 0 else 0, _lib.ptr(acc8), alpha, _lib.stream(),
                                                  meta=dict(ops=M * Cout * Kf, bytes=(N * H * W * 16 + nb if i == 0 else 0) + nb + M * Cout))
                if done:
                    a = acc8.view(8, 8, 8, Cout)[:kh, :kw]
                    acc = (2 * a[:, :, 0:3] + a[:, :, 4:7]).reshape(Kf, Cout).contiguous()
            if not done:
                acc16 = rt.zeros_i64(kh * kw * 16 * Cout, dev).view(kh * kw * 16, Cout)
                for g_, kind, alpha in halves:
                    _lib.call('lbt_conv_i8_wgrad', _lib.ptr(xm), Q.MANT_S8, N, H, W, 16, _lib.ptr(g_), kind, Cout, kh, kw, sh, sw,
                              pt, pl, OH, OW, _lib.ptr(acc16), alpha, 0, _lib.stream(),
                              meta=dict(ops=M * Cout * Kf, bytes=N * H * W * 16 + M * Cout + 8 * kh * kw * 16 * Cout))
                a = acc16.view(kh * kw, 16, Cout)
                acc = (a[:, 0:3] + a[:, 3:6] + a[:, 6:9]).reshape(Kf, Cout).contiguous()
        elif layer.implicit and xkind != Q.MANT_S16 and _implicit_ok(Cin, kh, kw) and _implicit_ok(Cout, 1, 1):
            done = DUAL_WGRAD and _lib.try_call('lbt_conv_i8_wgrad_dual', _lib.ptr(xm), xkind, N, H, W, Cin, _lib.ptr(hi), _lib.ptr(lo),
                                                Cout, kh, kw, sh, sw, pt, pl, OH, OW, _lib.ptr(acc), 1, 0, _lib.stream(),
                                                meta=dict(ops=2 * M * Cout * Kf, bytes=N * H * W * Cin + 2 * M * Cout + 8 * Kf * Cout))
            for g_, kind, alpha in (() if done else halves):
                _lib.call('lbt_conv_i8_wgrad', _lib.ptr(xm), xkind, N, H, W, Cin, _lib.ptr(g_), kind, Cout, kh, kw, sh, sw,
                          pt, pl, OH, OW, _lib.ptr(acc), alpha, 0, _lib.stream(),
                          meta=dict(ops=M * Cout * Kf, bytes=N * H * W * Cin + M * Cout + 8 * Kf * Cout))
        else:
            A = _im2col(xm, xkind, OH, OW, kh, kw, sh, sw, pt, pl, False)
            at = _transpose_bytes(A)
            for g_, kind, alpha in halves:
                gt = _transpose_bytes(g_.view(M, Cout))
                if xkind == Q.MANT_S16:
                    G.gemm_i8_acc64(at[:Kf], gt, acc, alpha=2 * alpha)
                    G.gemm_i8_acc64(at[2 * Kf:], gt, acc, alpha=alpha)
                else:
                    G.gemm_i8_acc64(at, gt, acc, alpha=alpha)
        dW = _emit_grad(rt, layer.weight, acc, ibA=layer.qX.range, ibB=layer.qG.range, exp_const=-(xb - 1) - (gb - 1),
                        add_scale=2 * layer.weight_decay, shape=(kh, kw, Cin, Cout))
    if need_db:
        if gm16 is None:
            raise _lib.LbtError('Conv2d_q: the bias gradient of a 16-bit gradient needs the s16 mantissas')
        db = _emit_grad(rt, layer.bias, _colsum(gm16.view(M, Cout), Q.MANT_S16, rt), ibA=layer.qG.range, exp_const=-(gb - 1))
    if need_dx:
        K2 = kh * kw * Cout
        e = -(gb - 1) - (wb - 1)
        pw2 = prep['w2'] if prep is not None else None
        if prep is not None and pw2 is None:
            raise _lib.LbtError('Conv2d_q: no input gradient for a 3-channel first-layer convolution')
        dx = torch.empty(N, H, W, Cin, dtype=torch.float32, device=dev)
        ad2 = addend.reshape(N * H * W, Cin) if addend is not None else None
        one_by_one = kh == 1 and kw == 1 and sh == 1 and sw == 1 and Cout % 16 == 0 and pt == 0 and pl == 0
        rot = bool(prep is not None and prep.get('rot180'))
        done = False
        if one_by_one:
            w2 = pw2 if pw2 is not None else _as_operand(wm.view(Cin, Cout))
            a_hi, a_lo = hi.view(M, Cout), lo.view(M, Cout)
        elif rot:
            w2 = pw2
            done = DUAL_HALO and _lib.try_call(
                'lbt_conv_i8_fprop_dual', _lib.ptr(hi), _lib.ptr(lo), N, OH, OW, Cout, _lib.ptr(w2),
                Q.MANT_S8, w2.stride(0), Cin, kh, kw, kh - 1 - pt, kw - 1 - pl, H, W, _lib.ptr(layer.qG.range),
                _lib.ptr(layer.qW.range), int(e), _lib.ptr(dx), Cin, _lib.ptr(ad2), _lib.stream(),
                meta=dict(ops=2 * 2 * N * H * W * Cin * K2, bytes=2 * N * OH * OW * Cout + Cin * K2 + N * H * W * Cin * 4))
            if not done:
                a_hi = _im2col(hi, Q.MANT_S8, H, W, kh, kw, 1, 1, kh - 1 - pt, kw - 1 - pl, False)
                a_lo = _im2col(lo, Q.MANT_U8, H, W, kh, kw, 1, 1, kh - 1 - pt, kw - 1 - pl, False)
        elif prep is not None and prep.get('classes'):
            _lib.call('lbt_conv_i8_dgrad_strided_dual', _lib.ptr(hi), _lib.ptr(lo), N, OH, OW, Cout, _lib.ptr(pw2), Q.MANT_S8,
                      pw2.stride(0), Cin, kh, kw, sh, sw, pt, pl, H, W, _lib.ptr(layer.qG.range), _lib.ptr(layer.qW.range), int(e),
                      _lib.ptr(dx), Cin, _lib.ptr(ad2), _lib.stream(),
                      meta=dict(ops=2 * 2 * N * OH * OW * Cin * K2, bytes=2 * N * OH * OW * Cout * min(sh * sw, kh * kw) + Cin * K2 + N * H * W * Cin * 4))
            done = True
        else:
            w2 = pw2 if pw2 is not None else _as_operand(wm.view(kh * kw, Cin, Cout).permute(1, 0, 2).reshape(Cin, K2))
            a_hi = _im2col(hi, Q.MANT_S8, H, W, kh, kw, sh, sw, pt, pl, True)
            a_lo = _im2col(lo, Q.MANT_U8, H, W, kh, kw, sh, sw, pt, pl, True)
        if not done:
            G.gemm_i8_dual(a_hi, a_lo, w2, ibA=layer.qG.range, ibB=layer.qW.range, exp_const=e, out=dx.view(N * H * W, Cin), addend=ad2)
    if fork:
        for t in (xm, hi, lo):
            t.record_stream(side)
        rt._side_pending = True
    return dx, dW, db


class _QConv2dFn(torch.autograd.Function):

    @staticmethod
    def forward(ctx, x, weight, bias, layer):
        geom = _conv_geom(layer, x, weight)
        N, H, W, Cin, Cout, kh, kw, sh, sw, pt, pl, OH, OW = geom
        xm, xkind = _conv_quantize_input(layer, x, geom)
        prep, wm, bq = _conv_params(layer, weight, bias)
        _stem_prepack(layer, xm, xkind, geom)
        y = torch.empty(N, OH, OW, Cout, dtype=torch.float32, device=x.device)
        _conv_fprop(layer, geom, xm, xkind, prep, wm, bq, y.view(N * OH * OW, Cout))
        ctx.layer, ctx.geom, ctx.xkind, ctx.prep = layer, geom, xkind, prep
        ctx.save_for_backward(xm, wm)
        return y.permute(0, 3, 1, 2)

    @staticmethod
    def backward(ctx, dy):
        layer = ctx.layer
        xm, wm = ctx.saved_tensors
        dy = _mem_contig(dy).permute(0, 2, 3, 1)
        needs = (ctx.needs_input_grad[0], ctx.needs_input_grad[1], layer.qb is not None and ctx.needs_input_grad[2])
        if layer.qG.bits > 8:
            if layer.qG.bits > 16:
                raise _lib.LbtError('Conv2d_q: gradient quantisers wider than 16 bits are not supported')
            _, gm16 = layer.qG.quantize(dy, want_fp32=False, mant_kind=Q.MANT_S16)
            hi, lo = _split16(gm16)
            dx, dW, db = _conv_backward16(layer, ctx.geom, xm, ctx.xkind, wm, ctx.prep, hi, lo, *needs, gm16=gm16)
            return (dx.permute(0, 3, 1, 2) if dx is not None else None), dW, db, None
        _, gm = layer.qG.quantize(dy, want_fp32=False, mant_kind=Q.MANT_S8)
        dx, dW, db = _conv_backward(layer, ctx.geom, xm, ctx.xkind, wm, ctx.prep, gm, ctx.needs_input_grad[0],
                                    ctx.needs_input_grad[1], layer.qb is not None and ctx.needs_input_grad[2])
        return (dx.permute(0, 3, 1, 2) if dx is not None else None), dW, db, None


class Conv2d_q(nn.Module):

    def __init__(self, bits, in_channels, out_channels, kernel_size, stride=1, padding='SAME', bias=True, *,
                 weight_decay=0.0, target_overflow_rate=0.0, input_range=2, weight_range=2, bias_range=2, grad_range=2,
                 grad_bits=None, input_signed=True, name='conv', runtime=None, implicit=True):
        super().__init__()
        rt = runtime or default_runtime()
        _check_layer_bits('Conv2d_q', bits, grad_bits)
        kh, kw = (kernel_size, kernel_size) if isinstance(kernel_size, int) else kernel_size
        self.stride = (stride, stride) if isinstance(stride, int) else tuple(stride)
        if isinstance(padding, str):
            assert padding in ('SAME', 'VALID')
            self.padding, self.pad_int = ('SAME', 0) if padding == 'SAME' else ('INT', 0)
        else:
            self.padding, self.pad_int = 'INT', int(padding)
        self.bits, self.weight_decay, self.input_signed, self.name = bits, float(weight_decay), input_signed, name
        self.implicit = implicit
        self.fuse_bn = True
        limit = (3 / (kh * kw * in_channels)) ** 0.5
        self.weight = nn.Parameter(torch.empty(kh, kw, in_channels, out_channels).uniform_(-limit, limit))
        self.bias = nn.Parameter(torch.zeros(out_channels)) if bias else None
        self.qX = QuantSite(rt, name + '/X', bits + 1, input_range, target_overflow_rate)
        self.qW = QuantSite(rt, name + '/W', bits, weight_range, target_overflow_rate)
        self.qb = QuantSite(rt, name + '/b', bits, bias_range, target_overflow_rate) if bias else None
        self.qG = QuantSite(rt, name + '/grad', grad_bits or bits, grad_range, target_overflow_rate)

    def forward(self, x):
        return _QConv2dFn.apply(x, self.weight, self.bias, self)

    def info(self):
        return '%d bits conv2d: %dx%dx%d stride %dx%d pad %s weight_decay %f' % (
            self.bits, self.weight.shape[0], self.weight.shape[1], self.weight.shape[3], self.stride[0], self.stride[1],
            self.padding, self.weight_decay)


Conv2d_pq = Conv2d_q




class _QLinearFn(torch.autograd.Function):

    @staticmethod
    def forward(ctx, x, weight, bias, layer):
        x = x.contiguous()
        Bsz, In = x.shape
        Out = weight.shape[1]
        if layer.qX.bits > 8 or layer.qW.bits > 8:
            raise _lib.LbtError('Linear_q: operands wider than 8 bits need the hi/lo GEMM split (not built yet)')
        _, xm = layer.qX.quantize(x, want_fp32=False, mant_kind=Q.MANT_S8)
        prep = _prepared(layer)
        bq = wm = None
        if prep is None:
            _, wm = layer.qW.quantize(weight, want_fp32=False, mant_kind=Q.MANT_S8)
            if bias is not None:
                bq, _ = layer.qb.quantize(bias)
            wt = _transpose_bytes(wm)
        else:
            wt, bq = prep['wt'], prep.get('bq')
        y = G.gemm_i8(_as_operand(xm), wt, ibA=layer.qX.range, ibB=layer.qW.range,
                      exp_const=-(layer.qX.bits - 1) - (layer.qW.bits - 1), bias=bq)
        ctx.layer, ctx.prep = layer, prep
        ctx.save_for_backward(xm, wm, weight)
        return y

    @staticmethod
    def backward(ctx, dy):
        layer = ctx.layer
        xm, wm, weight = ctx.saved_tensors
        xb, wb, gb = layer.qX.bits, layer.qW.bits, layer.qG.bits
        In, Out = weight.shape
        rt = layer.qX.runtime
        dX = dW = db = None
        if gb > 8:
            if gb > 16:
                raise _lib.LbtError('Linear_q: gradient quantisers wider than 16 bits are not supported')
            _, gm16 = layer.qG.quantize(dy.contiguous(), want_fp32=False, mant_kind=Q.MANT_S16)
            hi, lo = _split16(gm16)
            halves = ((hi, 256), (lo, 1))
            if ctx.needs_input_grad[1]:
                acc = rt.zeros_i64(In * Out, dy.device).view(In, Out)
                xt = _transpose_bytes(xm)
                for g_, alpha in halves:
                    G.gemm_i8_acc64(xt, _transpose_bytes(g_), acc, alpha=alpha, k_splits=1)
                dW = _emit_grad(rt, layer.weight, acc, ibA=layer.qX.range, ibB=layer.qG.range,
                                exp_const=-(xb - 1) - (gb - 1), add_scale=2 * layer.weight_decay)
            if layer.qb is not None and ctx.needs_input_grad[2]:
                db = _emit_grad(rt, layer.bias, _colsum(gm16, Q.MANT_S16, rt), ibA=layer.qG.range, exp_const=-(gb - 1))
            if ctx.needs_input_grad[0]:
                w2 = ctx.prep['w2'] if ctx.prep is not None else _as_operand(wm)
                dX = G.gemm_i8_dual(_as_operand(hi), _as_operand(lo), w2, ibA=layer.qG.range, ibB=layer.qW.range,
                                    exp_const=-(gb - 1) - (wb - 1))
            return dX, dW, db, None
        _, gm = layer.qG.quantize(dy.contiguous(), want_fp32=False, mant_kind=Q.MANT_S8)
        if ctx.needs_input_grad[1]:
            acc = rt.zeros_i64(In * Out, dy.device).view(In, Out)
            G.gemm_i8_acc64(_transpose_bytes(xm), _transpose_bytes(gm), acc, alpha=1, k_splits=1)
            dW = _emit_grad(rt, layer.weight, acc, ibA=layer.qX.range, ibB=layer.qG.range,
                            exp_const=-(xb - 1) - (gb - 1), add_scale=2 * layer.weight_decay)
        if layer.qb is not None and ctx.needs_input_grad[2]:
            db = _emit_grad(rt, layer.bias, _colsum(gm, Q.MANT_S8, rt), ibA=layer.qG.range, exp_const=-(gb - 1))
        if ctx.needs_input_grad[0]:
            w2 = ctx.prep['w2'] if ctx.prep is not None else _as_operand(wm)
            dX = G.gemm_i8(_as_operand(gm), w2, ibA=layer.qG.range, ibB=layer.qW.range,
                           exp_const=-(gb - 1) - (wb - 1))
        return dX, dW, db, None


class Linear_q(nn.Module):

    def __init__(self, bits, in_features, out_features, bias=True, *, weight_decay=0.0, target_overflow_rate=0.0,
                 input_range=2, weight_range=2, bias_range=2, grad_range=2, grad_bits=None, name='dense', runtime=None):
        super().__init__()
        rt = runtime or default_runtime()
        _check_layer_bits('Linear_q', bits, grad_bits)
        self.bits, self.weight_decay, self.name = bits, float(weight_decay), name
        limit = (6 / (in_features + out_features)) ** 0.5
        self.weight = nn.Parameter(torch.empty(in_features, out_features).uniform_(-limit, limit))
        self.bias = nn.Parameter(torch.zeros(out_features)) if bias else None
        self.qX = QuantSite(rt, name + '/X', bits, input_range, target_overflow_rate)
        self.qW = QuantSite(rt, name + '/W', bits, weight_range, target_overflow_rate)
        self.qb = QuantSite(rt, name + '/b', bits, bias_range, target_overflow_rate) if bias else None
        self.qG = QuantSite(rt, name + '/grad', grad_bits or bits, grad_range, target_overflow_rate)

    def forward(self, x):
        return _QLinearFn.apply(x, self.weight, self.bias, self)

    def info(self):
        return '%d bits dense: %dx%d weight_decay %f' % (self.bits, self.weight.shape[0], self.weight.shape[1],
                                                        self.weight_decay)


Dense_q = Linear_q




class _WeightDecayGrad(torch.autograd.Function):

    @staticmethod
    def forward(ctx, p, wd):
        ctx.wd = wd
        ctx.save_for_backward(p)
        return p.view_as(p)

    @staticmethod
    def backward(ctx, g):
        (p,) = ctx.saved_tensors
        return g + (2 * ctx.wd) * p.detach(), None


class Normalization_q(nn.Module):

    def __init__(self, bits, num_features, momentum=0.999, eps=1e-5, *, target_overflow_rate=0.0, input_range=2,
                 grad_range=2, grad_bits=None, name='norm', runtime=None):
        super().__init__()
        rt = runtime or default_runtime()
        self.bits, self.momentum, self.eps, self.name = bits, momentum, eps, name
        self.register_buffer('X_mean_running', torch.zeros(num_features))
        self.register_buffer('X_var_running', torch.ones(num_features))
        self.qX = QuantSite(rt, name + '/X', bits, input_range, target_overflow_rate)
        self.qG = QuantSite(rt, name + '/grad', grad_bits or bits, grad_range, target_overflow_rate)

    def forward(self, x):
        x = _mem_contig(x)
        xq = _QuantSTE.apply(x, self.qX)
        axes = (0, 2, 3) if x.dim() == 4 else (0,)
        shape = (1, -1, 1, 1) if x.dim() == 4 else (1, -1)
        if self.training:
            mean = xq.mean(dim=axes)
            var = ((xq - mean.view(shape)) ** 2).mean(dim=axes)
            with torch.no_grad():
                self.X_mean_running.mul_(self.momentum).add_((1 - self.momentum) * mean)
                self.X_var_running.mul_(self.momentum).add_((1 - self.momentum) * var)
        else:
            mean, var = self.X_mean_running, self.X_var_running
        y = (xq - mean.view(shape)) / ((var.view(shape) + self.eps) ** 0.5)
        return _GradQuant.apply(y, self.qG)


class Rescale_q(nn.Module):

    def __init__(self, bits, num_features, *, weight_decay=0.0, target_overflow_rate=0.0, input_range=2, gamma_range=2,
                 beta_range=2, grad_range=2, grad_bits=None, name='rescale', runtime=None):
        super().__init__()
        rt = runtime or default_runtime()
        self.bits, self.weight_decay, self.name = bits, float(weight_decay), name
        self.gamma = nn.Parameter(torch.ones(num_features))
        self.beta = nn.Parameter(torch.zeros(num_features))
        self.qX = QuantSite(rt, name + '/X', bits, input_range, target_overflow_rate)
        self.qg = QuantSite(rt, name + '/g', bits, gamma_range, target_overflow_rate)
        self.qb = QuantSite(rt, name + '/b', bits, beta_range, target_overflow_rate)
        self.qG = QuantSite(rt, name + '/grad', grad_bits or bits, grad_range, target_overflow_rate)

    def forward(self, x):
        x = _mem_contig(x)
        shape = (1, -1, 1, 1) if x.dim() == 4 else (1, -1)
        xq = _QuantSTE.apply(x, self.qX)
        gq = _QuantSTE.apply(_WeightDecayGrad.apply(self.gamma, self.weight_decay), self.qg)
        bq = _QuantSTE.apply(self.beta, self.qb)
        y = xq * gq.view(shape) + bq.view(shape)
        return _GradQuant.apply(y, self.qG)


def _site_args(site, x_like):
    rt = site.runtime
    if rt.noise_fn is not None:
        return rt.noise_fn(site, Q.rows_view(x_like)[1], x_like.device).contiguous(), 0
    return None, Q.make_offset(site.qid, 0)


def _to_mem(x):
    x = _mem_contig(x)
    return x.permute(0, 2, 3, 1) if x.dim() == 4 else x


def _from_mem(t):
    return t.permute(0, 3, 1, 2) if t.dim() == 4 else t


def _bn_params(resc, gamma, beta):
    prep = _prepared(resc)
    if prep is not None:
        return prep['gq'], prep['bq']
    gq, _ = resc.qg.quantize(gamma.detach())
    bq, _ = resc.qb.quantize(beta.detach())
    return gq, bq


def _bn_fwd1(bn, xm_):
    norm = bn[0]
    rt = norm.qX.runtime
    N, C = xm_.shape[0], xm_.shape[-1]
    n_inner = xm_.numel() // N
    sums = rt.zeros_i64(2 * C, xm_.device)
    k1 = torch.empty(xm_.shape, dtype=torch.int8, device=xm_.device)
    nz1, off1 = _site_args(norm.qX, xm_)
    _lib.call('lbt_bn_fwd_quant_stats', _lib.ptr(xm_), N, n_inner, C, norm.qX.bits, _lib.ptr(norm.qX.range),
              _lib.ptr(nz1), rt.seed, off1, _lib.ptr(rt.dev_step), _lib.ptr(k1), _lib.ptr(sums),
              _lib.ptr(norm.qX.counters), int(norm.qX.target == 0), _lib.stream(), meta=dict(bytes=xm_.numel() * 5))
    return k1, sums


def _bn_fwd2(bn, k1, sums, gq, bq, add_, relu, next_site=None, next_kind=Q.MANT_NONE, want_fp32=True, next2=None,
             running=False):
    norm, resc = bn[0], bn[1]
    rt = norm.qX.runtime
    N, C = k1.shape[0], k1.shape[-1]
    n_inner = k1.numel() // N
    dev = k1.device
    k2 = None if running else torch.empty_like(k1)
    out = torch.empty(k1.shape, dtype=torch.float32, device=dev) if want_fp32 else None
    nz2, off2 = _site_args(resc.qX, k1)
    relu_mode = 0 if not relu else (2 if add_ is not None else 1)
    qn = nm = None
    if next_site is not None:
        qn = next_site.abi(n_inner, dev)
        nm = torch.empty(k1.shape, dtype=torch.uint8 if next_kind == Q.MANT_U8 else torch.int8, device=dev)
    qn2 = nm2 = None
    if next2 is not None and qn is not None:
        site2, kind2 = next2[0], next2[1]
        qn2 = site2.abi(n_inner, dev)
        nm2 = torch.empty(k1.shape, dtype=torch.uint8 if kind2 == Q.MANT_U8 else torch.int8, device=dev)
        next2[2] = nm2
    nbytes = k1.numel() * ((1 if running else 2) + (4 if want_fp32 else 0) + (4 if add_ is not None else 0) +
                           (1 if nm is not None else 0) + (1 if nm2 is not None else 0))
    head = (_lib.ptr(k1), N, n_inner, C, norm.qX.bits, _lib.ptr(norm.qX.range))
    site = (float(norm.eps), resc.qX.bits, _lib.ptr(resc.qX.range), _lib.ptr(nz2), rt.seed, off2,
            _lib.ptr(rt.dev_step), _lib.ptr(resc.qX.counters), _lib.ptr(gq), _lib.ptr(bq), _lib.ptr(add_),
            1 if relu else 0, _lib.ptr(k2), _lib.ptr(out))
    nxt = (ctypes.addressof(qn) if qn is not None else None, _lib.ptr(nm), int(next_kind))
    nxt2 = (ctypes.addressof(qn2), _lib.ptr(nm2), int(next2[1])) if qn2 is not None else ()
    if running:
        _lib.call('lbt_bn_fwd_apply_running', *head, _lib.ptr(norm.X_mean_running), _lib.ptr(norm.X_var_running), *site,
                  int(resc.qX.target == 0), *nxt, *(nxt2 or (None, None, 0)), _lib.stream(), meta=dict(bytes=nbytes))
        return k2, out, nm, relu_mode
    args = head + (_lib.ptr(sums),) + site + (None, None, _lib.ptr(norm.X_mean_running), _lib.ptr(norm.X_var_running),
                                               float(norm.momentum), int(resc.qX.target == 0)) + nxt
    if nxt2:
        _lib.call('lbt_bn_fwd_apply2', *args, *nxt2, _lib.stream(), meta=dict(bytes=nbytes))
    else:
        _lib.call('lbt_bn_fwd_apply', *args, _lib.stream(), meta=dict(bytes=nbytes))
    return k2, out, nm, relu_mode


def _bn_backward(bn, g_, k1, k2, sums, gq, bq, out_, relu_mode, has_add, grad_site=None, want_dx=True, pre=None, pool=None):
    norm, resc = bn[0], bn[1]
    rt = norm.qX.runtime
    N, C = k1.shape[0], k1.shape[-1]
    n_inner = k1.numel() // N
    dev = k1.device
    bsums = pre[1] if pre is not None else rt.zeros_i64(4 * C + 2, dev)
    d_add = torch.empty(k1.shape, dtype=torch.float32, device=dev) if has_add else None
    dx = torch.empty(k1.shape, dtype=torch.float32, device=dev) if want_dx else None
    wide = max(resc.qG.bits, norm.qG.bits) > 8
    kg1_kind = Q.MANT_S16 if wide else Q.MANT_S8
    qg = gm = gm_lo = None
    if grad_site is not None:
        qg = grad_site.abi(n_inner, dev)
        gm = torch.empty_like(k1)
        if grad_site.bits > 8:
            gm_lo = torch.empty(k1.shape, dtype=torch.uint8, device=dev)
    nbytes = k1.numel() * (6 + (4 if relu_mode == 2 else 0) + (4 if has_add else 0) + (4 if want_dx else 0) +
                           (1 if gm is not None else 0))
    fused = False
    if FUSE_BN_BWD and pre is None and pool is None and not wide and gm_lo is None and not getattr(rt, '_side_pending', False):
        a = _lib.BnBwdArgs(g=_lib.ptr(g_), out=_lib.ptr(out_), k2=_lib.ptr(k2), k1=_lib.ptr(k1), n_outer=N, n_inner=n_inner, C=C,
                           relu=relu_mode, bits2=resc.qX.bits, bits1=norm.qX.bits, ib2=_lib.ptr(resc.qX.range),
                           ib1=_lib.ptr(norm.qX.range), gamma_q=_lib.ptr(gq), beta_q=_lib.ptr(bq),
                           q_g2=resc.qG.abi(n_inner, dev), q_g1=norm.qG.abi(n_inner, dev), d_add=_lib.ptr(d_add),
                           bwd_sums=_lib.ptr(bsums), fwd_sums=_lib.ptr(sums), eps=float(norm.eps),
                           has_q_grad=int(qg is not None), dx=_lib.ptr(dx), g_mant=_lib.ptr(gm),
                           barrier=bsums[4 * C:].data_ptr())
        if qg is not None:
            a.q_grad = qg
        fused = _lib.try_call('lbt_bn_bwd_fused', ctypes.addressof(a), _lib.stream(), meta=dict(bytes=nbytes))
    if not fused and pre is not None:
        kg1 = pre[0]
    elif not fused and pool is not None:
        kg1 = torch.empty(k1.shape, dtype=torch.int16 if wide else torch.int8, device=dev)
        nzg2, offg2 = _site_args(resc.qG, k1)
        nzg1, offg1 = _site_args(norm.qG, k1)
        pidx, pk, ps, ppt, ppl, POH, POW = pool
        geo = _lib.PoolGeom(idx=_lib.ptr(pidx), H=k1.shape[1], W=k1.shape[2], k=pk, s=ps, pad_top=ppt, pad_left=ppl, OH=POH, OW=POW)
        _lib.call('lbt_bn_bwd_quant_stats_pooled', _lib.ptr(g_), ctypes.addressof(geo), relu_mode, _lib.ptr(k2), _lib.ptr(k1), N,
                  n_inner, C, resc.qX.bits, _lib.ptr(resc.qX.range), _lib.ptr(gq), _lib.ptr(bq), resc.qG.bits,
                  _lib.ptr(resc.qG.range), _lib.ptr(nzg2), offg2, _lib.ptr(resc.qG.counters), norm.qG.bits,
                  _lib.ptr(norm.qG.range), _lib.ptr(nzg1), offg1, _lib.ptr(norm.qG.counters), rt.seed,
                  _lib.ptr(rt.dev_step), _lib.ptr(kg1), _lib.ptr(bsums),
                  int(resc.qG.target == 0 and norm.qG.target == 0), kg1_kind, _lib.stream(),
                  meta=dict(bytes=g_.numel() * 5 + k1.numel() * (3 + (1 if wide else 0))))
    elif not fused:
        kg1 = torch.empty(k1.shape, dtype=torch.int16 if wide else torch.int8, device=dev)
        nzg2, offg2 = _site_args(resc.qG, g_)
        nzg1, offg1 = _site_args(norm.qG, g_)
        _lib.call('lbt_bn_bwd_quant_stats', _lib.ptr(g_), _lib.ptr(out_), relu_mode, _lib.ptr(k2), _lib.ptr(k1), N, n_inner,
                  C, resc.qX.bits, _lib.ptr(resc.qX.range), _lib.ptr(gq), _lib.ptr(bq), resc.qG.bits,
                  _lib.ptr(resc.qG.range), _lib.ptr(nzg2), offg2, _lib.ptr(resc.qG.counters), norm.qG.bits,
                  _lib.ptr(norm.qG.range), _lib.ptr(nzg1), offg1, _lib.ptr(norm.qG.counters), rt.seed,
                  _lib.ptr(rt.dev_step), _lib.ptr(d_add), _lib.ptr(kg1), _lib.ptr(bsums),
                  int(resc.qG.target == 0 and norm.qG.target == 0), kg1_kind, _lib.stream(),
                  meta=dict(bytes=g_.numel() * (7 + (1 if wide else 0) + (4 if relu_mode == 2 else 0) + (4 if has_add else 0))))
    if not fused:
        _lib.call('lbt_bn_bwd_apply', _lib.ptr(kg1), _lib.ptr(k1), N, n_inner, C, norm.qX.bits, _lib.ptr(norm.qX.range),
                  _lib.ptr(sums), float(norm.eps), norm.qG.bits, _lib.ptr(norm.qG.range), _lib.ptr(bsums), _lib.ptr(dx),
                  ctypes.addressof(qg) if qg is not None else None, _lib.ptr(gm), kg1_kind, _lib.ptr(gm_lo), _lib.stream(),
                  meta=dict(bytes=k1.numel() * (2 + (1 if wide else 0) + (4 if want_dx else 0) + (1 if gm is not None else 0) +
                                                (1 if gm_lo is not None else 0))))
    dbeta = _emit_grad(rt, resc.beta, bsums[:C], ibA=resc.qG.range, exp_const=-(resc.qG.bits - 1))
    dgamma = _emit_grad(rt, resc.gamma, bsums[C:2 * C], ibA=resc.qG.range, ibB=resc.qX.range,
                        exp_const=-(resc.qG.bits - 1) - (resc.qX.bits - 1), add_scale=2 * resc.weight_decay)
    return dx, (gm if gm_lo is None else (gm, gm_lo)), dgamma, dbeta, d_add


class _FusedBNFn(torch.autograd.Function):

    @staticmethod
    def forward(ctx, x, gamma, beta, add, bn, relu, running=False):
        x_ = _to_mem(x)
        k1, sums = _bn_fwd1(bn, x_)
        gq, bq = _bn_params(bn[1], gamma, beta)
        add_ = _to_mem(add) if add is not None else None
        k2, out, _, relu_mode = _bn_fwd2(bn, k1, sums, gq, bq, add_, relu, running=running)
        if not running:
            ctx.bn, ctx.relu_mode, ctx.has_add = bn, relu_mode, add is not None
            ctx.save_for_backward(k1, k2, sums, gq, bq, out if relu_mode == 2 else None)
        return _from_mem(out)

    @staticmethod
    def backward(ctx, g):
        k1, k2, sums, gq, bq, out = ctx.saved_tensors
        dx, _, dgamma, dbeta, d_add = _bn_backward(ctx.bn, _to_mem(g), k1, k2, sums, gq, bq, out, ctx.relu_mode, ctx.has_add)
        return _from_mem(dx), dgamma, dbeta, (_from_mem(d_add) if d_add is not None else None), None, None, None


_link_count = 0
FUSE_BWD_LINK = os.environ.get('LBT_BWD_LINK', '0') == '1'


class _BwdLink:

    def __init__(self):
        self.bn = self.k1 = self.k2 = self.gq = self.bq = None
        self.relu_mode = 0
        self.kg1 = self.bsums = None
        self.done = False

    def offer(self, bn, k1, k2, gq, bq, relu_mode, has_add):
        norm, resc = bn[0], bn[1]
        if has_add or relu_mode not in (0, 1) or resc.qG.bits > 8 or norm.qG.bits > 8 or k1.shape[-1] % 4:
            return
        self.bn, self.k1, self.k2, self.gq, self.bq, self.relu_mode = bn, k1, k2, gq, bq, relu_mode

    def struct(self, n_inner, dev, kg1, bsums):
        norm, resc = self.bn[0], self.bn[1]
        return _lib.BnBwdLink(q_g2=resc.qG.abi(n_inner, dev, arena=True), q_g1=norm.qG.abi(n_inner, dev, arena=True), bits2=resc.qX.bits,
                              relu=self.relu_mode, ib2=_lib.ptr(resc.qX.range), gamma_q=_lib.ptr(self.gq), beta_q=_lib.ptr(self.bq),
                              k2=_lib.ptr(self.k2), k1=_lib.ptr(self.k1), kg1=_lib.ptr(kg1), sums=_lib.ptr(bsums))


class _ConvBNFn(torch.autograd.Function):

    @staticmethod
    def forward(ctx, x, weight, gamma, beta, add, conv, bn, relu, next_site, next_kind, want_fp32, alias, link_in, link_out, pool=None,
                next2=None, running=False):
        geom = _conv_geom(conv, x, weight)
        N, H, W, Cin, Cout, kh, kw, sh, sw, pt, pl, OH, OW = geom
        norm, resc = bn[0], bn[1]
        rt = norm.qX.runtime
        dev = x.device
        xm, xkind = _conv_quantize_input(conv, x, geom)
        prep, wm, _ = _conv_params(conv, weight, None)
        _stem_prepack(conv, xm, xkind, geom)
        sums = rt.zeros_i64(2 * Cout, dev)
        k1 = torch.empty(N, OH, OW, Cout, dtype=torch.int8, device=dev)
        _conv_fprop(conv, geom, xm, xkind, prep, wm, None, None,
                    bnq=(norm.qX.abi(OH * OW * Cout, dev, arena=True), k1, sums))
        gq, bq = _bn_params(resc, gamma, beta)
        add_ = _to_mem(add) if add is not None else None
        pooled = pidx = None
        if pool is not None and (add is not None or not FUSE_POOL_FWD or Cout != 64 or pool[:4] != (3, 2, 0, 0)):
            next_site, next_kind = None, Q.MANT_NONE
        if pool is not None and FUSE_POOL_FWD and add is None and Cout == 64 and pool[:4] == (3, 2, 0, 0):
            pk, ps, ppt, ppl, POH, POW = pool
            k2 = None if running else torch.empty_like(k1)
            pooled = torch.empty(N, POH, POW, Cout, dtype=torch.float32, device=dev)
            pidx = torch.empty(N, POH, POW, Cout, dtype=torch.uint8, device=dev)
            nz2, off2 = _site_args(resc.qX, k1)
            qn = nmp = None
            if next_site is not None:
                qn = next_site.abi(POH * POW * Cout, dev)
                nmp = torch.empty(N, POH, POW, Cout, dtype=torch.uint8 if next_kind == Q.MANT_U8 else torch.int8, device=dev)
            head = (_lib.ptr(k1), N, OH, OW, Cout, norm.qX.bits, _lib.ptr(norm.qX.range))
            site = (float(norm.eps), resc.qX.bits, _lib.ptr(resc.qX.range), _lib.ptr(nz2), rt.seed, off2,
                    _lib.ptr(rt.dev_step), _lib.ptr(resc.qX.counters), _lib.ptr(gq), _lib.ptr(bq), 1 if relu else 0, _lib.ptr(k2))
            tail = (pk, ps, ppt, ppl, POH, POW, _lib.ptr(pooled), _lib.ptr(pidx),
                    ctypes.addressof(qn) if qn is not None else None, _lib.ptr(nmp), int(next_kind), _lib.stream())
            meta = dict(bytes=k1.numel() * (1 if running else 2) + pooled.numel() * (5 + (1 if nmp is not None else 0)))
            if running:
                done = _lib.try_call('lbt_bn_fwd_apply_running_pooled', *head, _lib.ptr(norm.X_mean_running),
                                     _lib.ptr(norm.X_var_running), *site, int(resc.qX.target == 0), *tail, meta=meta)
            else:
                done = _lib.try_call('lbt_bn_fwd_apply_pooled', *head, _lib.ptr(sums), *site, _lib.ptr(norm.X_mean_running),
                                     _lib.ptr(norm.X_var_running), float(norm.momentum), int(resc.qX.target == 0), *tail,
                                     meta=meta)
            if done:
                out, nm, relu_mode = None, nmp, (1 if relu else 0)
            else:
                pooled = pidx = None
                next_site, next_kind = None, Q.MANT_NONE
        if pooled is None:
            k2, out, nm, relu_mode = _bn_fwd2(bn, k1, sums, gq, bq, add_, relu, next_site, next_kind, True if pool is not None else want_fp32,
                                              next2=next2 if pool is None else None, running=running)
        ctx.conv, ctx.bn, ctx.geom, ctx.xkind, ctx.prep = conv, bn, geom, xkind, prep
        ctx.relu_mode, ctx.has_add = relu_mode, add is not None
        ctx.link_in, ctx.link_out = link_in, link_out
        if link_out is not None and out is None and not running:
            link_out.offer(bn, k1, k2, gq, bq, relu_mode, add is not None)
        ctx.pool = None
        if pooled is not None:
            ctx.pool = tuple(pool)
            out = pooled
        elif pool is not None:
            pk, ps, ppt, ppl, POH, POW = pool
            pooled = torch.empty(N, POH, POW, Cout, dtype=torch.float32, device=dev)
            pidx = torch.empty(N, POH, POW, Cout, dtype=torch.uint8, device=dev)
            _lib.call('lbt_maxpool_fwd', _lib.ptr(out), N, OH, OW, Cout, pk, ps, ppt, ppl, POH, POW, _lib.ptr(pooled), _lib.ptr(pidx),
                      _lib.stream(), meta=dict(bytes=out.numel() * 4 + pooled.numel() * 5))
            ctx.pool = (pk, ps, ppt, ppl, POH, POW)
            out = pooled
        if not running:
            ctx.save_for_backward(xm, wm, k1, k2, sums, gq, bq, out if relu_mode == 2 else None, pidx)
        if out is None:
            out = torch.empty(1, dtype=torch.float32, device=dev).expand(N, OH, OW, Cout)
        if nm is None:
            nm = torch.empty(0, dtype=torch.uint8, device=dev)
        ctx.mark_non_differentiable(nm)
        ctx.set_materialize_grads(False)
        xa = x.view_as(x) if alias else torch.empty(0, dtype=torch.float32, device=dev)
        return _from_mem(out), nm, xa

    @staticmethod
    def backward(ctx, g, _g_nm, g_alias):
        conv = ctx.conv
        xm, wm, k1, k2, sums, gq, bq, out, pidx = ctx.saved_tensors
        need_dx, need_dw = ctx.needs_input_grad[0], ctx.needs_input_grad[1]
        lo = ctx.link_out
        pre = (lo.kg1, lo.bsums) if (lo is not None and lo.done) else None
        pool = ((pidx,) + ctx.pool) if ctx.pool is not None else None
        if pool is not None and not FUSE_POOL:
            _, pk, ps, ppt, ppl, POH, POW = pool
            g_ = _to_mem(g)
            Np, Hp, Wp_, Cp = k1.shape
            gd = torch.empty(k1.shape, dtype=torch.float32, device=k1.device)
            _lib.call('lbt_maxpool_bwd', _lib.ptr(g_), _lib.ptr(pidx), Np, Hp, Wp_, Cp, pk, ps, ppt, ppl, POH, POW, _lib.ptr(gd),
                      _lib.stream(), meta=dict(bytes=gd.numel() * 4 + g_.numel() * 5))
            g, pool = _from_mem(gd), None
        _, gm, dgamma, dbeta, d_add = _bn_backward(ctx.bn, _to_mem(g) if pre is None else None, k1, k2, sums, gq, bq, out,
                                                   ctx.relu_mode, ctx.has_add, grad_site=conv.qG, want_dx=False, pre=pre,
                                                   pool=pool)
        addend = _to_mem(g_alias) if (g_alias is not None and need_dx) else None
        li = ctx.link_in if (addend is None and FUSE_BWD_LINK) else None
        if isinstance(gm, tuple):
            dx, dW, _ = _conv_backward16(conv, ctx.geom, xm, ctx.xkind, wm, ctx.prep, gm[0], gm[1], need_dx, need_dw, False, addend=addend)
        else:
            dx, dW, _ = _conv_backward(conv, ctx.geom, xm, ctx.xkind, wm, ctx.prep, gm, need_dx, need_dw, False, addend=addend, link=li)
        return ((_from_mem(dx) if dx is not None else None), dW, dgamma, dbeta,
                (_from_mem(d_add) if d_add is not None else None), None, None, None, None, None, None, None, None, None, None, None,
                None)


FUSE_POOL = os.environ.get('LBT_FUSE_POOL', '0') == '1'
FUSE_BN_BWD = False
FUSE_UNITS = True
DUAL_WGRAD = os.environ.get('LBT_DUAL_WGRAD', '1') != '0'
DUAL_HALO = os.environ.get('LBT_DUAL_HALO', '1') != '0'
FUSE_NEXT2 = os.environ.get('LBT_FUSE_NEXT2', '1') != '0'


def _unit_fusable(conv, bn, x, running=False):
    return (FUSE_UNITS and isinstance(conv, Conv2d_q) and isinstance(bn, BatchNorm2d_q) and conv.bias is None and conv.fuse_bn and
            bn._can_fuse_c(conv.weight.shape[3], 4, running) and conv.qG.bits <= 16 and conv.qW.bits <= 8 and conv.qX.bits <= 9 and
            x.is_cuda)


def conv_bn_unit(conv, bn, x, add=None, relu=False, next_conv=None, want_fp32=True, alias=False, link_in=None, link_out=None,
                 pool=None):
    relu = relu or getattr(bn, 'relu', False)
    running = isinstance(bn, BatchNorm2d_q) and bn._running(x, add, conv.weight)
    if not _unit_fusable(conv, bn, x, running):
        y = bn(conv(x), add=add, relu=relu) if isinstance(bn, BatchNorm2d_q) else bn(conv(x))
        if pool is not None:
            y = pool(y)
        return (y, x) if alias else y
    pgeom = None
    if pool is not None:
        if add is not None or alias or not pool_fusable(pool):
            y = conv_bn_unit(conv, bn, x, add=add, relu=relu, alias=alias, link_in=link_in, link_out=link_out)
            return (pool(y[0]), y[1]) if alias else pool(y)
        Hc, Wc = _conv_geom(conv, x, conv.weight)[11:13]
        pgeom = pool.geometry(Hc, Wc)
        if not FUSE_POOL_FWD:
            next_conv = None
    next_conv2 = None
    if isinstance(next_conv, (tuple, list)):
        next_conv, next_conv2 = (tuple(next_conv) + (None, None))[:2]

    def _site_of(nc):
        if nc is not None and isinstance(nc, Conv2d_q) and nc.fuse_bn:
            nb = nc.qX.bits
            if nb <= 8:
                return nc.qX, Q.MANT_S8
            if nb == 9 and relu and not nc.input_signed:
                return nc.qX, Q.MANT_U8
        return None, Q.MANT_NONE

    next_site, next_kind = _site_of(next_conv)
    next2 = None
    if next_site is not None and next_conv2 is not None and pool is None and FUSE_NEXT2:
        s2, k2_ = _site_of(next_conv2)
        if s2 is not None and s2 is not next_site:
            next2 = [s2, k2_, None]
    if next_site is None or add is not None or pool is not None:
        want_fp32 = True
    use_alias = bool(alias and x.requires_grad and not getattr(x, '_lbt_hollow', False) and conv.weight.shape[2] <= 128)
    out, nm, xa = _ConvBNFn.apply(x, conv.weight, bn[1].gamma, bn[1].beta, add, conv, bn, relu, next_site, next_kind,
                                  want_fp32, use_alias, link_in if FUSE_BWD_LINK else None, link_out if FUSE_BWD_LINK else None,
                                  pgeom, next2, running)
    if next_site is not None and nm.numel():
        out._lbt_q = {id(next_site): (nm, next_kind)}
        if next2 is not None and next2[2] is not None:
            out._lbt_q[id(next2[0])] = (next2[2], next2[1])
    if not want_fp32:
        out._lbt_hollow = True
    if alias:
        return out, (xa if use_alias else x)
    return out


def run_layers(layers, x, next_conv=None):
    layers = list(layers)
    i = 0
    while i < len(layers):
        m = layers[i]
        nxt = layers[i + 1] if i + 1 < len(layers) else None
        if isinstance(m, Conv2d_q) and isinstance(nxt, BatchNorm2d_q):
            after = layers[i + 2] if i + 2 < len(layers) else next_conv
            if (FUSE_POOL or FUSE_POOL_FWD) and isinstance(after, MaxPool_q) and i + 2 < len(layers):
                after2 = layers[i + 3] if i + 3 < len(layers) else next_conv
                x = conv_bn_unit(m, nxt, x, pool=after, next_conv=_first_conv(after2))
                i += 3
                continue
            x = conv_bn_unit(m, nxt, x, next_conv=_first_conv(after))
            i += 2
        elif isinstance(m, ResidualBlock_q):
            x = m(x, next_conv=_first_conv(nxt if nxt is not None else next_conv))
            i += 1
        else:
            x = m(x)
            i += 1
    return x


def _first_conv(m):
    if isinstance(m, Conv2d_q):
        return m
    if isinstance(m, ResidualBlock_q):
        first = m.residual[0] if isinstance(m.residual[0], Conv2d_q) else None
        sc = list(m.shortcut) if isinstance(m.shortcut, nn.Sequential) else []
        if first is not None and sc and isinstance(sc[0], Conv2d_q):
            return (first, sc[0])
        return first
    return None


class BatchNorm2d_q(nn.Sequential):

    def __init__(self, bits, num_features, momentum=0.999, eps=1e-5, *, weight_decay=0.0, target_overflow_rate=0.0,
                 input_range=2, gamma_range=2, beta_range=2, grad_range=2, grad_bits=None, name='bn', runtime=None,
                 fused=True, relu=False):
        super().__init__(
            Normalization_q(bits, num_features, momentum, eps, target_overflow_rate=target_overflow_rate,
                            input_range=input_range, grad_range=grad_range, grad_bits=grad_bits, name=name + '-norm',
                            runtime=runtime),
            Rescale_q(bits, num_features, weight_decay=weight_decay, target_overflow_rate=target_overflow_rate,
                      input_range=2, gamma_range=gamma_range, beta_range=beta_range, grad_range=grad_range,
                      grad_bits=grad_bits, name=name + '-rescale', runtime=runtime))
        self.fused = fused
        self.relu = relu

    def _can_fuse_c(self, C, dim, running=False):
        norm, resc = self[0], self[1]
        return (self.fused and (self.training or running) and dim in (2, 4) and C % 4 == 0 and
                max(norm.qX.bits, resc.qX.bits) <= 8 and max(norm.qG.bits, resc.qG.bits) <= 16 and
                min(norm.qX.bits, resc.qX.bits, norm.qG.bits, resc.qG.bits) >= 2)

    def _can_fuse(self, x, running=False):
        return self._can_fuse_c(x.shape[1], x.dim(), running)

    def _running(self, *inputs):
        if self.training or not FUSE_UNITS:
            return False
        return not torch.is_grad_enabled() or not any(t is not None and t.requires_grad
                                                      for t in inputs + (self[1].gamma, self[1].beta))

    def forward(self, x, add=None, relu=False):
        relu = relu or self.relu
        running = self._running(x, add)
        if self._can_fuse(x, running):
            return _FusedBNFn.apply(x, self[1].gamma, self[1].beta, add, self, relu, running)
        y = self[1](self[0](x))
        if add is not None:
            y = y + add
        return _ReLUFn.apply(y) if relu else y

    def info(self):
        return 'BatchNorm'


BatchNorm_q = BatchNorm2d_q




class _ReLUFn(torch.autograd.Function):

    @staticmethod
    def forward(ctx, x):
        x = _mem_contig(x)
        y = torch.empty_like(x)
        _lib.call('lbt_relu', _lib.ptr(x), None, _lib.ptr(y), x.numel(), _lib.stream(), meta=dict(bytes=x.numel() * 8))
        ctx.save_for_backward(y)
        return y

    @staticmethod
    def backward(ctx, g):
        (y,) = ctx.saved_tensors
        g = _mem_contig(g)
        dx = torch.empty_like(y)
        _lib.call('lbt_relu', _lib.ptr(y), _lib.ptr(g), _lib.ptr(dx), y.numel(), _lib.stream(), meta=dict(bytes=y.numel() * 12))
        return dx


class ReLU_q(nn.Module):

    def forward(self, x):
        _require_cuda_f32(x, 'ReLU_q')
        return _ReLUFn.apply(x)

    def info(self):
        return 'ReLU'


class _MaxPoolFn(torch.autograd.Function):

    @staticmethod
    def forward(ctx, x, k, s, pt, pl, OH, OW):
        x_ = _to_mem(x)
        N, H, W, C = x_.shape
        out = torch.empty(N, OH, OW, C, dtype=torch.float32, device=x.device)
        idx = torch.empty(N, OH, OW, C, dtype=torch.uint8, device=x.device)
        _lib.call('lbt_maxpool_fwd', _lib.ptr(x_), N, H, W, C, k, s, pt, pl, OH, OW, _lib.ptr(out), _lib.ptr(idx),
                  _lib.stream(), meta=dict(bytes=x_.numel() * 4 + out.numel() * 5))
        ctx.geom = (N, H, W, C, k, s, pt, pl, OH, OW)
        ctx.save_for_backward(idx)
        return _from_mem(out)

    @staticmethod
    def backward(ctx, g):
        (idx,) = ctx.saved_tensors
        N, H, W, C, k, s, pt, pl, OH, OW = ctx.geom
        g_ = _to_mem(g)
        dx = torch.empty(N, H, W, C, dtype=torch.float32, device=g.device)
        _lib.call('lbt_maxpool_bwd', _lib.ptr(g_), _lib.ptr(idx), N, H, W, C, k, s, pt, pl, OH, OW, _lib.ptr(dx),
                  _lib.stream(), meta=dict(bytes=g_.numel() * 5 + dx.numel() * 4))
        return _from_mem(dx), None, None, None, None, None, None


class MaxPool_q(nn.Module):

    def __init__(self, kernel_size, stride, padding='SAME'):
        super().__init__()
        self.k, self.s, self.padding = kernel_size, stride, padding

    def geometry(self, H, W):
        if self.padding == 'SAME':
            OH, pt, pb = same_pad(H, self.k, self.s)
            OW, pl, pr = same_pad(W, self.k, self.s)
        else:
            pt = pl = 0
            OH, OW = (H - self.k) // self.s + 1, (W - self.k) // self.s + 1
        return self.k, self.s, pt, pl, OH, OW

    def forward(self, x):
        H, W = x.shape[2], x.shape[3]
        _, _, pt, pl, OH, OW = self.geometry(H, W)
        _require_cuda_f32(x, 'MaxPool_q')
        if x.dim() != 4 or self.k > 15:
            raise _lib.LbtError('MaxPool_q: needs a 4-d tensor and a window of at most 15x15')
        return _MaxPoolFn.apply(x, self.k, self.s, pt, pl, OH, OW)


def pool_fusable(pool):
    return isinstance(pool, MaxPool_q) and pool.k <= 2 * pool.s and pool.k <= 15


class _AvgPoolFn(torch.autograd.Function):

    @staticmethod
    def forward(ctx, x, k, s):
        x_ = _to_mem(x)
        N, H, W, C = x_.shape
        OH, OW = (H - k) // s + 1, (W - k) // s + 1
        out = torch.empty(N, OH, OW, C, dtype=torch.float32, device=x.device)
        _lib.call('lbt_avgpool_fwd', _lib.ptr(x_), N, H, W, C, k, s, OH, OW, _lib.ptr(out), _lib.stream(),
                  meta=dict(bytes=(x_.numel() + out.numel()) * 4))
        ctx.geom = (N, H, W, C, k, s, OH, OW)
        return _from_mem(out)

    @staticmethod
    def backward(ctx, g):
        N, H, W, C, k, s, OH, OW = ctx.geom
        g_ = _to_mem(g)
        dx = torch.empty(N, H, W, C, dtype=torch.float32, device=g.device)
        _lib.call('lbt_avgpool_bwd', _lib.ptr(g_), N, H, W, C, k, s, OH, OW, _lib.ptr(dx), _lib.stream(),
                  meta=dict(bytes=(g_.numel() + dx.numel()) * 4))
        return _from_mem(dx), None, None


class AvgPool_q(nn.Module):

    def __init__(self, kernel_size, stride=1):
        super().__init__()
        self.k, self.s = kernel_size, stride

    def forward(self, x):
        _require_cuda_f32(x, 'AvgPool_q')
        if x.dim() != 4:
            raise _lib.LbtError('AvgPool_q: needs a 4-d tensor')
        return _AvgPoolFn.apply(x, self.k, self.s)


class _XentFn(torch.autograd.Function):

    @staticmethod
    def forward(ctx, logits, labels):
        logits = logits.contiguous()
        B, C = logits.shape
        probs = torch.empty_like(logits)
        loss = torch.empty((), dtype=torch.float32, device=logits.device)
        _lib.call('lbt_softmax_xent_fwd', _lib.ptr(logits), _lib.ptr(labels), B, C, _lib.ptr(probs), _lib.ptr(loss), _lib.stream())
        ctx.save_for_backward(probs, labels)
        return loss

    @staticmethod
    def backward(ctx, gout):
        probs, labels = ctx.saved_tensors
        B, C = probs.shape
        d = torch.empty_like(probs)
        _lib.call('lbt_softmax_xent_bwd', _lib.ptr(probs), _lib.ptr(labels), _lib.ptr(gout.contiguous()), B, C, _lib.ptr(d),
                  _lib.stream())
        return d, None


def softmax_cross_entropy(logits, labels):
    _require_cuda_f32(logits, 'softmax_cross_entropy')
    if logits.dim() != 2 or not labels.is_cuda:
        raise _lib.LbtError('softmax_cross_entropy: expects [batch, classes] logits and CUDA integer labels')
    return _XentFn.apply(logits, labels.to(torch.int64).contiguous())


class _DropoutFn(torch.autograd.Function):

    @staticmethod
    def forward(ctx, x, keep, u, seed, offset, dev_step):
        x = _mem_contig(x)
        y = torch.empty_like(x)
        _lib.call('lbt_dropout', _lib.ptr(x), _lib.ptr(u), float(keep), int(seed), int(offset), _lib.ptr(dev_step), _lib.ptr(y),
                  x.numel(), _lib.stream(), meta=dict(bytes=x.numel() * 8))
        ctx.args = (keep, seed, offset, dev_step)
        ctx.fmt4 = x.dim() == 4
        ctx.save_for_backward(u)
        return y

    @staticmethod
    def backward(ctx, g):
        (u,) = ctx.saved_tensors
        keep, seed, offset, dev_step = ctx.args
        g = _mem_contig(g)
        dx = torch.empty_like(g)
        _lib.call('lbt_dropout', _lib.ptr(g), _lib.ptr(u), float(keep), int(seed), int(offset), _lib.ptr(dev_step), _lib.ptr(dx),
                  g.numel(), _lib.stream(), meta=dict(bytes=g.numel() * 8))
        return dx, None, None, None, None, None


class Dropout_q(nn.Module):

    def __init__(self, keep_prob, runtime=None):
        super().__init__()
        self.keep_prob = keep_prob
        self.uniform_fn = None
        self.runtime = runtime or default_runtime()
        self.did = self.runtime.next_dropout_id()

    def forward(self, x):
        if not self.training or self.keep_prob >= 1.0:
            return x
        _require_cuda_f32(x, 'Dropout_q')
        rt = self.runtime
        if self.uniform_fn is not None:
            u = _mem_contig(self.uniform_fn(x).to(torch.float32))
            return _DropoutFn.apply(x, self.keep_prob, u, 0, 0, None)
        return _DropoutFn.apply(x, self.keep_prob, None, rt.seed, Q.make_offset(0x7fffffff - self.did, 0), rt.dev_step)


class Flatten_q(nn.Module):

    def __init__(self, dim):
        super().__init__()
        self.dim = dim

    def forward(self, x):
        if x.dim() == 4:
            x = x.permute(0, 2, 3, 1)
        return x.reshape(-1, self.dim)


class _GradBufferFn(torch.autograd.Function):
    @staticmethod
    def forward(ctx, x, layer):
        ctx.layer = layer
        return x.view_as(x)

    @staticmethod
    def backward(ctx, dy):
        layer = ctx.layer
        site, rt = layer.qG, layer.qG.runtime
        g = _to_mem(dy).contiguous()
        n_outer = layer.buffer.shape[0]
        n_inner = layer.buffer.numel() // n_outer
        if g.shape[0] > n_outer or g.numel() // max(1, g.shape[0]) != n_inner:
            raise _lib.LbtError('GradientBuffer_q: gradient %s does not fit the buffer %s' % (tuple(g.shape), tuple(layer.buffer.shape)))
        out = torch.empty_like(g)
        if rt.noise_fn is not None:
            mode, noise, dev_step = Q.ROUND_NOISE, rt.noise_fn(site, n_inner, g.device).contiguous(), None
        else:
            mode, noise, dev_step = Q.ROUND_PHILOX, None, rt.dev_step
        _lib.call('lbt_quantize_residual', _lib.ptr(g), g.shape[0], _lib.ptr(layer.buffer), n_outer, n_inner, site.bits,
                  _lib.ptr(site.range), mode, _lib.ptr(noise), rt.seed, Q.make_offset(site.qid, 0), _lib.ptr(dev_step),
                  _lib.ptr(out), _lib.ptr(site.counters), _lib.stream(), meta=dict(bytes=n_outer * n_inner * 16))
        return _from_mem(out), None


class GradientBuffer_q(nn.Module):

    def __init__(self, bits, shape, *, target_overflow_rate=0.0, grad_range=2, name='grad_buffer', runtime=None):
        super().__init__()
        rt = runtime or default_runtime()
        self.bits, self.name = bits, name
        self.register_buffer('buffer', torch.zeros(*shape))
        self.qG = QuantSite(rt, name + '/grad', bits, grad_range, target_overflow_rate)

    def forward(self, x):
        return _GradBufferFn.apply(x, self)

    def info(self):
        return 'Gradient buffer'


class Sequential_q(nn.Sequential):
    """dfxp:512-536."""




class ResidualBlock_q(nn.Module):
    expansion = 1

    def __init__(self, bits, in_channels, channels, stride, batch_norm=True, *, weight_decay=0.0, target_overflow_rate=0.0,
                 input_range=2, weight_range=2, bias_range=2, grad_range=2, grad_bits=None, name='block', runtime=None):
        super().__init__()
        ckw = dict(bias=not batch_norm, weight_decay=weight_decay, input_range=input_range, weight_range=weight_range,
                   bias_range=bias_range, grad_range=grad_range, grad_bits=grad_bits, input_signed=False, runtime=runtime)
        self._bn = lambda n, c, relu=False: (
            BatchNorm2d_q(bits, c, weight_decay=weight_decay, target_overflow_rate=target_overflow_rate,
                          input_range=input_range, grad_range=grad_range, grad_bits=grad_bits, name=n, runtime=runtime,
                          relu=relu) if batch_norm else (ReLU_q() if relu else nn.Identity()))
        self.residual = self._build_residual(bits, in_channels, channels, stride, name, ckw)
        if stride == 1 and in_channels == self.expansion * channels:
            self.shortcut = nn.Sequential()
        else:
            self.shortcut = nn.Sequential(
                Conv2d_q(bits, in_channels, self.expansion * channels, 1, stride, 'SAME', name=name + '-shortcut',
                         target_overflow_rate=target_overflow_rate, **ckw),
                self._bn(name + '-shortcut-bn', self.expansion * channels))
        del self._bn

    def _build_residual(self, bits, in_channels, channels, stride, name, ckw):
        return nn.Sequential(
            Conv2d_q(bits, in_channels, channels, 3, stride, 'SAME', name=name + '-1', **ckw),
            self._bn(name + '-bn1', channels, relu=True),
            Conv2d_q(bits, channels, channels, 3, 1, 'SAME', name=name + '-2', **ckw),
            self._bn(name + '-bn2', channels))

    def forward(self, x, next_conv=None):
        res = list(self.residual)
        sc_layers = list(self.shortcut)
        paired = len(res) % 2 == 0 and all(isinstance(res[i], Conv2d_q) and isinstance(res[i + 1], BatchNorm2d_q)
                                           for i in range(0, len(res), 2))
        if paired:
            link = _BwdLink()
            r, xs = conv_bn_unit(res[0], res[1], x, next_conv=res[2], want_fp32=False, alias=True, link_out=link)
            if xs is not x and getattr(x, '_lbt_q', None) is not None:
                xs._lbt_q = x._lbt_q
            for i in range(2, len(res) - 2, 2):
                nxt = _BwdLink()
                r = conv_bn_unit(res[i], res[i + 1], r, next_conv=res[i + 2], want_fp32=False, link_in=link, link_out=nxt)
                link = nxt
            sc = conv_bn_unit(sc_layers[0], sc_layers[1], xs) if len(sc_layers) == 2 else self.shortcut(xs)
            return conv_bn_unit(res[-2], res[-1], r, add=sc, relu=True, next_conv=next_conv, link_in=link)
        r = x
        for m in res[:-1]:
            r = m(r)
        last = res[-1]
        sc = self.shortcut(x)
        if isinstance(last, BatchNorm2d_q):
            return last(r, add=sc, relu=True)
        return _ReLUFn.apply(last(r) + sc)

    def info(self):
        return 'Residual block'


class ResidualBottleneck_q(ResidualBlock_q):
    expansion = 4

    def _build_residual(self, bits, in_channels, channels, stride, name, ckw):
        return nn.Sequential(
            Conv2d_q(bits, in_channels, channels, 1, 1, 'SAME', name=name + '-1', **ckw),
            self._bn(name + '-bn1', channels, relu=True),
            Conv2d_q(bits, channels, channels, 3, stride, 'SAME', name=name + '-2', **ckw),
            self._bn(name + '-bn2', channels, relu=True),
            Conv2d_q(bits, channels, 4 * channels, 1, 1, 'SAME', name=name + '-3', **ckw),
            self._bn(name + '-bn3', 4 * channels))
```

Measured before the change: 32410.

## Fuse strided residual and 1x1 shortcut dgrad into one block kernel

```diff
diff --git a/include/lbt.h b/include/lbt.h
--- a/include/lbt.h
+++ b/include/lbt.h
@@ -324,6 +324,12 @@
                               int Cin, int kh, int kw, int sh, int sw, int pad_top, int pad_left, int H, int W,
                               const int32_t* ib_g, const int32_t* ib_w, int exp_const, float* dx, size_t ldc,
                               const float* addend, void* stream);
+int lbt_conv_i8_dgrad_block(const void* g, int g_kind, int N, int OH, int OW, int Cout, const void* w2, int w_kind, size_t ldw,
+                            int Cin, int kh, int kw, int sh, int sw, int pad_top, int pad_left, int H, int W,
+                            const int32_t* ib_g, const int32_t* ib_w, int exp_const, const void* g_short, int gs_kind,
+                            int OHs, int OWs, int Cout_s, const void* w_short, int ws_kind, size_t ldws,
+                            const int32_t* ib_gs, const int32_t* ib_ws, int exp_short, float* dx, size_t ldc,
+                            const float* addend, void* stream);
 int lbt_conv_i8_dgrad_strided_dual(const int8_t* g_hi, const uint8_t* g_lo, int N, int OH, int OW, int Cout, const void* w2,
                                    int w_kind, size_t ldw, int Cin, int kh, int kw, int sh, int sw, int pad_top, int pad_left,
                                    int H, int W, const int32_t* ib_g, const int32_t* ib_w, int exp_const, float* dx, size_t ldc,
diff --git a/lbt_b200/_lib.py b/lbt_b200/_lib.py
--- a/lbt_b200/_lib.py
+++ b/lbt_b200/_lib.py
@@ -94,6 +94,9 @@
     'lbt_conv_i8_dgrad_strided': (c_int, [c_void_p, c_int, c_int, c_int, c_int, c_int, c_void_p, c_int, c_size_t, c_int, c_int, c_int,
                                           c_int, c_int, c_int, c_int, c_int, c_int, c_void_p, c_void_p, c_int, c_void_p, c_size_t,
                                           c_void_p, c_void_p]),
+    'lbt_conv_i8_dgrad_block': (c_int, [c_void_p, c_int, c_int, c_int, c_int, c_int, c_void_p, c_int, c_size_t] + [c_int] * 9 +
+                                [c_void_p, c_void_p, c_int, c_void_p, c_int, c_int, c_int, c_int, c_void_p, c_int, c_size_t,
+                                 c_void_p, c_void_p, c_int, c_void_p, c_size_t, c_void_p, c_void_p]),
     'lbt_dp_step': (c_int, [c_void_p, c_void_p, c_size_t, c_float, c_void_p, c_float, c_int, c_void_p, c_void_p, c_void_p,
                             c_size_t, c_void_p, c_void_p]),
     'lbt_dp_export': (c_int, [c_void_p, c_void_p, c_void_p]),
diff --git a/lbt_b200/csrc/conv_dgrad.cu b/lbt_b200/csrc/conv_dgrad.cu
--- a/lbt_b200/csrc/conv_dgrad.cu
+++ b/lbt_b200/csrc/conv_dgrad.cu
@@ -84,6 +84,49 @@
                            exp_const, dx, ldc, addend, stream);
 }
 
+extern "C" int lbt_conv_i8_dgrad_block(const void* g, int g_kind, int N, int OH, int OW, int Cout, const void* w2, int w_kind, size_t ldw,
+                                       int Cin, int kh, int kw, int sh, int sw, int pad_top, int pad_left, int H, int W,
+                                       const int32_t* ib_g, const int32_t* ib_w, int exp_const, const void* g_short, int gs_kind,
+                                       int OHs, int OWs, int Cout_s, const void* w_short, int ws_kind, size_t ldws,
+                                       const int32_t* ib_gs, const int32_t* ib_ws, int exp_short, float* dx, size_t ldc,
+                                       const float* addend, void* stream) {
+  w_kind &= ~LBT_MANT_PREPARED;
+  ws_kind &= ~LBT_MANT_PREPARED;
+  if (!g || !w2 || !dx || !ib_g || !ib_w) return LBT_EINVAL;
+  if ((g_kind != LBT_MANT_S8 && g_kind != LBT_MANT_U8) || (w_kind != LBT_MANT_S8 && w_kind != LBT_MANT_U8)) return LBT_EINVAL;
+  if (N <= 0 || H <= 0 || W <= 0 || Cin <= 0 || Cout <= 0 || kh <= 0 || kw <= 0 || sh <= 0 || sw <= 0 || OH <= 0 || OW <= 0)
+    return LBT_EINVAL;
+  if (pad_top < 0 || pad_left < 0 || ldc < (size_t)Cin || ldw < (size_t)kh * kw * Cout) return LBT_EINVAL;
+  if (g_short) {
+    if (!w_short || !ib_gs || !ib_ws) return LBT_EINVAL;
+    if ((gs_kind != LBT_MANT_S8 && gs_kind != LBT_MANT_U8) || (ws_kind != LBT_MANT_S8 && ws_kind != LBT_MANT_U8)) return LBT_EINVAL;
+    if (OHs <= 0 || OWs <= 0 || Cout_s <= 0 || ldws < (size_t)Cout_s) return LBT_EINVAL;
+    if (OHs != (H + sh - 1) / sh || OWs != (W + sw - 1) / sw) return LBT_EUNSUPPORTED;
+    if (addend) return LBT_EUNSUPPORTED;
+  }
+  const int cb = Cout >= 128 ? 128 : Cout;
+  if (Cin % 4) return LBT_EUNSUPPORTED;
+  if (sh > 2 || sw > 2 || (cb != 32 && cb != 64 && cb != 128) || Cout % cb || (Cin != 64 && Cin % 128)) return LBT_EUNSUPPORTED;
+  if (g_short && (Cout_s % cb || Cout_s > 65536 || (Cout_s >= 128 ? 128 : Cout_s) != cb)) return LBT_EUNSUPPORTED;
+  if ((size_t)kh * kw * Cout > 65536 || kh > 255 || kw > 255) return LBT_EUNSUPPORTED;
+  if ((size_t)N * H * W >= (1ull << 31)) return LBT_EUNSUPPORTED;
+  if ((reinterpret_cast<uintptr_t>(g) & 15) || (reinterpret_cast<uintptr_t>(w2) & 15) || (ldw & 15) || (ldc & 3) ||
+      (reinterpret_cast<uintptr_t>(dx) & 15) || (addend && (reinterpret_cast<uintptr_t>(addend) & 15)) ||
+      (g_short && ((reinterpret_cast<uintptr_t>(g_short) & 15) || (reinterpret_cast<uintptr_t>(w_short) & 15) || (ldws & 15))))
+    return LBT_EUNSUPPORTED;
+  for (int a = 0; a < sh; ++a) {
+    const int r0 = (a + pad_top) % sh, nr = class_count(r0, kh, sh);
+    if (nr && nr - 1 - (a + pad_top) / sh < 0) return LBT_EUNSUPPORTED;
+  }
+  for (int b = 0; b < sw; ++b) {
+    const int s0 = (b + pad_left) % sw, nc = class_count(s0, kw, sw);
+    if (nc && nc - 1 - (b + pad_left) / sw < 0) return LBT_EUNSUPPORTED;
+  }
+  return conv_dgrad_block_run(g, g_kind, N, OH, OW, Cout, w2, w_kind, ldw, Cin, kh, kw, sh, sw, pad_top, pad_left, H, W, ib_g, ib_w,
+                              exp_const, g_short, gs_kind, Cout_s, w_short, ws_kind, ldws, ib_gs, ib_ws, exp_short, dx, ldc, addend,
+                              stream);
+}
+
 extern "C" int lbt_conv_i8_dgrad_strided_dual(const int8_t* g_hi, const uint8_t* g_lo, int N, int OH, int OW, int Cout, const void* w2,
                                               int w_kind, size_t ldw, int Cin, int kh, int kw, int sh, int sw, int pad_top, int pad_left,
                                               int H, int W, const int32_t* ib_g, const int32_t* ib_w, int exp_const, float* dx, size_t ldc,
diff --git a/lbt_b200/csrc/conv_i8.cu b/lbt_b200/csrc/conv_i8.cu
--- a/lbt_b200/csrc/conv_i8.cu
+++ b/lbt_b200/csrc/conv_i8.cu
@@ -1,3 +1,4 @@
+#include "conv_classes.h"
 #include "conv_internal.h"
 #include "qsite.cuh"
 #include "tcgen05.cuh"
@@ -934,6 +935,423 @@
                         alpha, k_splits, stream);
 }
 
+namespace lbt {
+namespace {
+
+constexpr int kBlkMaxClasses = 4;
+
+struct BlkClass {
+  uint32_t M, OW, OHW;
+  FastDiv d_OW, d_OHW;
+  int lower_w, lower_h;
+  uint32_t kw;
+  uint32_t ksteps;
+  uint32_t kcol;
+  uint32_t shortcut;
+  uint32_t tile0, m_tiles;
+  long long out_off;
+};
+
+struct BlkParams {
+  uint32_t nclasses;
+  BlkClass cls[kBlkMaxClasses];
+  uint32_t total_tiles, n_tiles, N;
+  uint32_t cb, mode;
+  uint32_t cchunks_g;
+  uint32_t ks_short;
+  const int32_t *ib_g, *ib_w, *ib_gs, *ib_ws;
+  int exp_const, exp_short;
+  const float* addend;
+  float* out;
+  long long rs_n, rs_y, rs_x;
+  uint32_t idesc, idesc_s;
+};
+
+struct BlkMaps {
+  CUtensorMap a[kBlkMaxClasses];
+  CUtensorMap b;
+  CUtensorMap as, bs;
+};
+
+template <int BN>
+struct BCfg {
+  static constexpr int kStageA = Cfg<BN>::kStageA;
+  static constexpr int kStageB = Cfg<BN>::kStageB;
+  static constexpr int kStageBytes = kStageA + kStageB;
+  static constexpr int kCtasPerSm = 2;
+  static constexpr int kStages = BN <= 64 ? 4 : 3;
+  static constexpr int kSmemBytes = kStages * kStageBytes + 1024;
+  static constexpr int kAccW = 2 * BN;
+  static constexpr int kAccStages = (512 / kCtasPerSm) / kAccW;
+  static constexpr int kTmemCols = kAccStages * kAccW;
+  static_assert(kAccStages >= 1, "block dgrad accumulators");
+  static_assert(kCtasPerSm * kSmemBytes <= 227 * 1024, "shared memory budget");
+  static_assert(kCtasPerSm * kTmemCols <= 512, "tensor memory budget");
+};
+
+__device__ __forceinline__ uint32_t blk_class_of(const BlkParams& p, uint32_t tile) {
+  uint32_t c = 0;
+  while (c + 1 < p.nclasses && tile >= p.cls[c + 1].tile0) ++c;
+  return c;
+}
+
+template <int BN>
+__global__ void __launch_bounds__(kThreadsF, BCfg<BN>::kCtasPerSm)
+conv_dgrad_block_kernel(const __grid_constant__ BlkMaps maps, const __grid_constant__ BlkParams p) {
+  using C = BCfg<BN>;
+  extern __shared__ uint8_t smem_raw[];
+  uint8_t* smem = reinterpret_cast<uint8_t*>((reinterpret_cast<uintptr_t>(smem_raw) + 1023) & ~uintptr_t(1023));
+  __shared__ __align__(8) uint64_t full_bar[C::kStages];
+  __shared__ __align__(8) uint64_t empty_bar[C::kStages];
+  __shared__ __align__(8) uint64_t tmem_full_bar[C::kAccStages];
+  __shared__ __align__(8) uint64_t tmem_empty_bar[C::kAccStages];
+  __shared__ uint32_t tmem_slot;
+  __shared__ int s_abort;
+
+  const int warp = threadIdx.x >> 5, lane = threadIdx.x & 31;
+  if (threadIdx.x == 0) {
+    for (int s = 0; s < C::kStages; ++s) {
+      mbar_init(&full_bar[s], 1);
+      mbar_init(&empty_bar[s], 1);
+    }
+    for (int s = 0; s < C::kAccStages; ++s) {
+      mbar_init(&tmem_full_bar[s], 1);
+      mbar_init(&tmem_empty_bar[s], kEpiWarps);
+    }
+    s_abort = 0;
+    fence_barrier_init();
+    for (uint32_t c = 0; c < p.nclasses; ++c)
+      if (p.cls[c].ksteps) tma_prefetch_desc(&maps.a[c]);
+    tma_prefetch_desc(&maps.b);
+    if (p.ks_short) {
+      tma_prefetch_desc(&maps.as);
+      tma_prefetch_desc(&maps.bs);
+    }
+  }
+  if (warp == 1) tmem_alloc(&tmem_slot, C::kTmemCols);
+  pdl_trigger();
+  fence_before();
+  __syncthreads();
+  fence_after();
+  pdl_wait();
+  const uint32_t tmem_base = *reinterpret_cast<volatile uint32_t*>(&tmem_slot);
+  volatile int* abort_flag = &s_abort;
+
+  const uint32_t spb = kStageK / p.cb;
+  const uint32_t a_block = kBlockM * p.cb, b_block = BN * p.cb;
+  const uint32_t ss_short = (p.ks_short + spb - 1) / spb;
+
+  if (warp == 0) {
+    if (lane == 0) {
+      uint32_t stage = 0, phase = 0;
+      bool ok = true;
+      for (uint32_t tile = blockIdx.x; tile < p.total_tiles && ok; tile += gridDim.x) {
+        const uint32_t ci = blk_class_of(p, tile);
+        const BlkClass& k = p.cls[ci];
+        const uint32_t ss_main = (k.ksteps + spb - 1) / spb, ss_sc = k.shortcut ? ss_short : 0u;
+        if (ss_main + ss_sc == 0) continue;
+        const uint32_t local = tile - k.tile0;
+        const uint32_t m_tile = local % k.m_tiles, n_tile = local / k.m_tiles;
+        const uint32_t m0 = m_tile * kBlockM;
+        const uint32_t img = fastdiv(m0, k.d_OHW), rem = m0 - img * k.OHW;
+        const uint32_t ohu = fastdiv(rem, k.d_OW);
+        const int base_w = k.lower_w + (int)(rem - ohu * k.OW), base_h = k.lower_h + (int)ohu;
+        uint32_t cc = 0, r = 0, s = 0;
+        for (uint32_t ks = 0; ks < ss_main + ss_sc && ok; ++ks) {
+          if (!(ok = mbar_wait(&empty_bar[stage], phase ^ 1, abort_flag, &g_conv_error))) break;
+          uint8_t* sa = smem + stage * C::kStageBytes;
+          uint8_t* sb = sa + C::kStageA;
+          if (ks < ss_main) {
+            const uint32_t k0 = ks * spb, nblk = min(spb, k.ksteps - k0);
+            mbar_expect_tx(&full_bar[stage], nblk * (a_block + b_block));
+            for (uint32_t j = 0; j < nblk; ++j) {
+              tma_load_im2col_4d(&maps.a[ci], &full_bar[stage], sa + j * a_block, (int)(cc * p.cb), base_w, base_h, (int)img,
+                                 (uint16_t)s, (uint16_t)r);
+              tma_load_2d(&maps.b, &full_bar[stage], sb + j * b_block, (int)(k.kcol + (k0 + j) * p.cb), (int)(n_tile * BN));
+              if (++cc == p.cchunks_g) {
+                cc = 0;
+                if (++s == k.kw) {
+                  s = 0;
+                  ++r;
+                }
+              }
+            }
+          } else {
+            const uint32_t k0 = (ks - ss_main) * spb, nblk = min(spb, p.ks_short - k0);
+            mbar_expect_tx(&full_bar[stage], nblk * (a_block + b_block));
+            for (uint32_t j = 0; j < nblk; ++j) {
+              tma_load_2d(&maps.as, &full_bar[stage], sa + j * a_block, (int)((k0 + j) * p.cb), (int)m0);
+              tma_load_2d(&maps.bs, &full_bar[stage], sb + j * b_block, (int)((k0 + j) * p.cb), (int)(n_tile * BN));
+            }
+          }
+          if (++stage == C::kStages) {
+            stage = 0;
+            phase ^= 1;
+          }
+        }
+      }
+    }
+  } else if (warp == 1) {
+    if (lane == 0) {
+      uint32_t stage = 0, phase = 0, acc = 0, acc_phase = 0;
+      bool ok = true;
+      for (uint32_t tile = blockIdx.x; tile < p.total_tiles && ok; tile += gridDim.x) {
+        const BlkClass& k = p.cls[blk_class_of(p, tile)];
+        const uint32_t ss_main = (k.ksteps + spb - 1) / spb, ss_sc = k.shortcut ? ss_short : 0u;
+        if (ss_main + ss_sc == 0) continue;
+        if (!(ok = mbar_wait(&tmem_empty_bar[acc], acc_phase ^ 1, abort_flag, &g_conv_error))) break;
+        fence_after();
+        const uint32_t d_main = tmem_base + acc * C::kAccW;
+        for (uint32_t ks = 0; ks < ss_main + ss_sc; ++ks) {
+          if (!(ok = mbar_wait(&full_bar[stage], phase, abort_flag, &g_conv_error))) break;
+          fence_after();
+          const uint32_t sa = smem_u32(smem + stage * C::kStageBytes);
+          const uint32_t sb = sa + C::kStageA;
+          const bool sc = ks >= ss_main;
+          const uint32_t k0 = (sc ? ks - ss_main : ks) * spb;
+          const uint32_t nblk = min(spb, (sc ? p.ks_short : k.ksteps) - k0);
+          const uint32_t d = sc ? d_main + BN : d_main;
+          const uint32_t idesc = sc ? p.idesc_s : p.idesc;
+          const uint32_t per_block = p.cb / 32;
+          for (uint32_t j = 0; j < nblk; ++j)
+            for (uint32_t kk = 0; kk < per_block; ++kk) {
+              const uint32_t accumulate = (k0 + j > 0 || kk > 0) ? 1u : 0u;
+              umma_i8(d, make_desc_kmajor(sa + j * a_block + kk * 32, (int)p.mode, 16),
+                      make_desc_kmajor(sb + j * b_block + kk * 32, (int)p.mode, 16), idesc, accumulate);
+            }
+          umma_commit(&empty_bar[stage]);
+          if (++stage == C::kStages) {
+            stage = 0;
+            phase ^= 1;
+          }
+        }
+        if (!ok) break;
+        umma_commit(&tmem_full_bar[acc]);
+        if (++acc == C::kAccStages) {
+          acc = 0;
+          acc_phase ^= 1;
+        }
+      }
+    }
+  } else {
+    const uint32_t quad = warp & 3;
+    const uint32_t half = (uint32_t)(warp - 2) >> 2;
+    const float scale = exp2i(p.exp_const + *p.ib_g + *p.ib_w);
+    const float scale_s = p.ks_short ? exp2i(p.exp_short + *p.ib_gs + *p.ib_ws) : 0.f;
+    uint32_t acc = 0, acc_phase = 0;
+    bool ok = true;
+    for (uint32_t tile = blockIdx.x; tile < p.total_tiles && ok; tile += gridDim.x) {
+      const BlkClass& k = p.cls[blk_class_of(p, tile)];
+      const bool has_m = k.ksteps != 0, has_s = k.shortcut && p.ks_short;
+      const bool has_acc = has_m || has_s;
+      const uint32_t local = tile - k.tile0;
+      const uint32_t m_tile = local % k.m_tiles, n_tile = local / k.m_tiles;
+      const uint32_t row = m_tile * kBlockM + quad * 32 + lane;
+      const uint32_t col0 = n_tile * BN;
+      if (has_acc) {
+        ok = mbar_wait(&tmem_full_bar[acc], acc_phase, abort_flag, &g_conv_error);
+        ok = __all_sync(0xffffffffu, ok);
+        if (!ok) break;
+        fence_after();
+      }
+      const uint32_t taddr = tmem_base + acc * C::kAccW + ((quad * 32u) << 16);
+      float* orow = nullptr;
+      if (row < k.M) {
+        const uint32_t img = fastdiv(row, k.d_OHW), rem = row - img * k.OHW;
+        const uint32_t oh = fastdiv(rem, k.d_OW), ow = rem - oh * k.OW;
+        orow = p.out + (k.out_off + (long long)img * p.rs_n + (long long)oh * p.rs_y + (long long)ow * p.rs_x) + col0;
+      }
+#pragma unroll 1
+      for (int c = 16 * (int)half; c < BN; c += 32) {
+        uint32_t v[16], w[16];
+        if (has_m) tmem_ld16(taddr + c, v);
+        if (has_s) tmem_ld16(taddr + BN + c, w);
+        if (has_acc) tmem_ld_wait();
+        if (orow && col0 + c < p.N) {
+          float* o = orow + c;
+          float f[16];
+#pragma unroll
+          for (int j = 0; j < 16; ++j) f[j] = has_m ? __int2float_rn((int)v[j]) * scale : 0.f;
+          if (has_s) {
+#pragma unroll
+            for (int j = 0; j < 16; ++j) {
+              const float fs = __int2float_rn((int)w[j]) * scale_s;
+              f[j] = has_m ? __fadd_rn(f[j], fs) : fs;
+            }
+          } else if (p.addend) {
+            const float4* ad = reinterpret_cast<const float4*>(p.addend + (o - p.out));
+#pragma unroll
+            for (int j = 0; j < 4; ++j) {
+              const float4 a4 = __ldcs(ad + j);
+              f[4 * j + 0] = has_m ? __fadd_rn(f[4 * j + 0], a4.x) : a4.x;
+              f[4 * j + 1] = has_m ? __fadd_rn(f[4 * j + 1], a4.y) : a4.y;
+              f[4 * j + 2] = has_m ? __fadd_rn(f[4 * j + 2], a4.z) : a4.z;
+              f[4 * j + 3] = has_m ? __fadd_rn(f[4 * j + 3], a4.w) : a4.w;
+            }
+          }
+#pragma unroll
+          for (int j = 0; j < 16; j += 4) *reinterpret_cast<float4*>(o + j) = make_float4(f[j], f[j + 1], f[j + 2], f[j + 3]);
+        }
+      }
+      if (has_acc) {
+        fence_before();
+        __syncwarp();
+        if (lane == 0) mbar_arrive(&tmem_empty_bar[acc]);
+        if (++acc == C::kAccStages) {
+          acc = 0;
+          acc_phase ^= 1;
+        }
+      }
+    }
+  }
+
+  fence_before();
+  __syncthreads();
+  fence_after();
+  if (warp == 1) tmem_dealloc(tmem_base, C::kTmemCols);
+}
+
+template <int BN>
+int launch_block(const BlkMaps& maps, const BlkParams& p, unsigned grid, cudaStream_t st) {
+  static bool attr_done[16] = {};
+  const int dev = device_info().device;
+  if (!attr_done[dev]) {
+    cudaError_t e = cudaFuncSetAttribute(conv_dgrad_block_kernel<BN>, cudaFuncAttributeMaxDynamicSharedMemorySize, BCfg<BN>::kSmemBytes);
+    if (e != cudaSuccess) {
+      set_cuda_error(e, "cudaFuncSetAttribute(conv_dgrad_block_kernel)");
+      return LBT_ECUDA;
+    }
+    attr_done[dev] = true;
+  }
+  launch_pdl(conv_dgrad_block_kernel<BN>, grid, kThreadsF, BCfg<BN>::kSmemBytes, st, maps, p);
+  return check_launch("lbt_conv_i8_dgrad_block");
+}
+
+}
+}
+
+int lbt::conv_dgrad_block_run(const void* g, int g_kind, int N, int OH, int OW, int Cout, const void* w2, int w_kind, size_t ldw, int Cin,
+                              int kh, int kw, int sh, int sw, int pad_top, int pad_left, int H, int W, const int32_t* ib_g,
+                              const int32_t* ib_w, int exp_const, const void* gs, int gs_kind, int Cout_s, const void* ws, int ws_kind,
+                              size_t ldws, const int32_t* ib_gs, const int32_t* ib_ws, int exp_short, float* dx, size_t ldc,
+                              const float* addend, void* stream) {
+  const uint32_t cb = Cout >= 128 ? 128u : (uint32_t)Cout;
+  uint32_t mode = 0;
+  while ((16u << mode) < cb) ++mode;
+  const int bn = Cin == 64 ? 64 : 128;
+  LBT_REQUIRE_ARCH();
+  const DeviceInfo& di = device_info();
+  static EncodeTiledFn enc_tiled = reinterpret_cast<EncodeTiledFn>(driver_fn("cuTensorMapEncodeTiled"));
+  static EncodeIm2colFn enc_im2col = reinterpret_cast<EncodeIm2colFn>(driver_fn("cuTensorMapEncodeIm2col"));
+  if (!enc_tiled || !enc_im2col) return LBT_ECUDA;
+
+  BlkParams p{};
+  BlkMaps maps;
+  memset(&maps, 0, sizeof(maps));
+  p.n_tiles = (uint32_t)Cin / bn;
+  p.N = (uint32_t)Cin;
+  p.cb = cb;
+  p.mode = mode;
+  p.cchunks_g = (uint32_t)Cout / cb;
+  p.ks_short = gs ? (uint32_t)Cout_s / cb : 0u;
+  p.ib_g = ib_g;
+  p.ib_w = ib_w;
+  p.ib_gs = ib_gs;
+  p.ib_ws = ib_ws;
+  p.exp_const = exp_const;
+  p.exp_short = exp_short;
+  p.addend = addend;
+  p.out = dx;
+  p.rs_n = (long long)H * W * (long long)ldc;
+  p.rs_y = (long long)sh * W * (long long)ldc;
+  p.rs_x = (long long)sw * (long long)ldc;
+  p.idesc = tc::make_idesc_i8(g_kind == LBT_MANT_S8, w_kind == LBT_MANT_S8, false, false, bn, kBlockM);
+  p.idesc_s = tc::make_idesc_i8(gs_kind == LBT_MANT_S8, ws_kind == LBT_MANT_S8, false, false, bn, kBlockM);
+
+  struct Cls {
+    int a, b, work;
+  } order[kBlkMaxClasses];
+  int nc = 0;
+  for (int a = 0; a < sh && a < H; ++a)
+    for (int b = 0; b < sw && b < W; ++b) {
+      const int r0 = (a + pad_top) % sh, s0 = (b + pad_left) % sw;
+      const int work = class_count(r0, kh, sh) * class_count(s0, kw, sw) * (int)p.cchunks_g + (a == 0 && b == 0 ? (int)p.ks_short : 0);
+      int i = nc++;
+      while (i > 0 && order[i - 1].work < work) {
+        order[i] = order[i - 1];
+        --i;
+      }
+      order[i] = Cls{a, b, work};
+    }
+  p.nclasses = (uint32_t)nc;
+  uint32_t tile0 = 0;
+  for (int i = 0; i < nc; ++i) {
+    const int a = order[i].a, b = order[i].b;
+    const int Hc = (H - a + sh - 1) / sh, Wc = (W - b + sw - 1) / sw;
+    const int r0 = (a + pad_top) % sh, s0 = (b + pad_left) % sw;
+    const int nr = class_count(r0, kh, sh), ncol = class_count(s0, kw, sw);
+    BlkClass& k = p.cls[i];
+    k.M = (uint32_t)N * (uint32_t)(Hc * Wc);
+    k.OW = (uint32_t)Wc;
+    k.OHW = (uint32_t)(Hc * Wc);
+    k.d_OW = make_fastdiv(k.OW);
+    k.d_OHW = make_fastdiv(k.OHW);
+    k.shortcut = (a == 0 && b == 0 && gs) ? 1u : 0u;
+    k.m_tiles = (k.M + kBlockM - 1) / kBlockM;
+    k.tile0 = tile0;
+    tile0 += k.m_tiles * p.n_tiles;
+    k.out_off = ((long long)a * W + b) * (long long)ldc;
+    k.ksteps = (uint32_t)(nr * ncol) * p.cchunks_g;
+    if (!k.ksteps) continue;
+    const int pt2 = nr - 1 - (a + pad_top) / sh, pl2 = ncol - 1 - (b + pad_left) / sw;
+    k.lower_w = -pl2;
+    k.lower_h = -pt2;
+    k.kw = (uint32_t)ncol;
+    k.kcol = class_group_offset(r0, s0, kh, kw, sh, sw) * (uint32_t)Cout;
+    cuuint64_t gdim[4] = {(cuuint64_t)Cout, (cuuint64_t)OW, (cuuint64_t)OH, (cuuint64_t)N};
+    cuuint64_t gstr[3] = {(cuuint64_t)Cout, (cuuint64_t)OW * Cout, (cuuint64_t)OH * OW * Cout};
+    int lower[2] = {-pl2, -pt2};
+    int upper[2] = {Wc - OW - pl2, Hc - OH - pt2};
+    cuuint32_t estr[4] = {1, 1, 1, 1};
+    CUresult r = enc_im2col(&maps.a[i], CU_TENSOR_MAP_DATA_TYPE_UINT8, 4, const_cast<void*>(g), gdim, gstr, lower, upper, cb, kBlockM,
+                            estr, CU_TENSOR_MAP_INTERLEAVE_NONE, swizzle_of(mode), CU_TENSOR_MAP_L2_PROMOTION_L2_128B,
+                            CU_TENSOR_MAP_FLOAT_OOB_FILL_NONE);
+    if (r != CUDA_SUCCESS) {
+      set_cuda_error(cudaErrorInvalidValue, "cuTensorMapEncodeIm2col(block dgrad)");
+      return LBT_ECUDA;
+    }
+  }
+  p.total_tiles = tile0;
+  auto tiled = [&](CUtensorMap* m, const void* base, uint64_t inner, uint64_t outer, uint64_t pitch, uint32_t rows,
+                   CUtensorMapL2promotion l2, const char* what) {
+    cuuint64_t gdim[2] = {(cuuint64_t)inner, (cuuint64_t)outer};
+    cuuint64_t gstr[1] = {(cuuint64_t)pitch};
+    cuuint32_t box[2] = {cb, rows};
+    cuuint32_t estr[2] = {1, 1};
+    if (enc_tiled(m, CU_TENSOR_MAP_DATA_TYPE_UINT8, 2, const_cast<void*>(base), gdim, gstr, box, estr, CU_TENSOR_MAP_INTERLEAVE_NONE,
+                  swizzle_of(mode), l2, CU_TENSOR_MAP_FLOAT_OOB_FILL_NONE) != CUDA_SUCCESS) {
+      set_cuda_error(cudaErrorInvalidValue, what);
+      return false;
+    }
+    return true;
+  };
+  if (!tiled(&maps.b, w2, (uint64_t)kh * kw * Cout, (uint64_t)Cin, ldw, (uint32_t)bn, CU_TENSOR_MAP_L2_PROMOTION_L2_256B,
+             "cuTensorMapEncodeTiled(block dgrad weights)"))
+    return LBT_ECUDA;
+  if (gs) {
+    const uint64_t rows_s = (uint64_t)N * ((H + sh - 1) / sh) * ((W + sw - 1) / sw);
+    if (!tiled(&maps.as, gs, (uint64_t)Cout_s, rows_s, (uint64_t)Cout_s, (uint32_t)kBlockM, CU_TENSOR_MAP_L2_PROMOTION_L2_128B,
+               "cuTensorMapEncodeTiled(block dgrad shortcut gradient)") ||
+        !tiled(&maps.bs, ws, (uint64_t)Cout_s, (uint64_t)Cin, ldws, (uint32_t)bn, CU_TENSOR_MAP_L2_PROMOTION_L2_256B,
+               "cuTensorMapEncodeTiled(block dgrad shortcut weights)"))
+      return LBT_ECUDA;
+  }
+  const uint64_t cap = (uint64_t)di.sm_count * BCfg<64>::kCtasPerSm;
+  const unsigned grid = (unsigned)(p.total_tiles < cap ? p.total_tiles : cap);
+  cudaStream_t st = reinterpret_cast<cudaStream_t>(stream);
+  return bn == 64 ? launch_block<64>(maps, p, grid, st) : launch_block<128>(maps, p, grid, st);
+}
+
 extern "C" int lbt_conv_debug_error(void) {
   int v = 0, zero = 0;
   if (cudaMemcpyFromSymbol(&v, g_conv_error, sizeof(int)) != cudaSuccess) return -1;
diff --git a/lbt_b200/csrc/conv_internal.h b/lbt_b200/csrc/conv_internal.h
--- a/lbt_b200/csrc/conv_internal.h
+++ b/lbt_b200/csrc/conv_internal.h
@@ -34,6 +34,12 @@
                    int exp_const, const float* bias, float* out, size_t ldc, const lbt_qsite* q_out, int8_t* k_out, int64_t* sums,
                    const float* addend, void* stream, const OutRemap* remap, const void* src_lo = nullptr);
 
+int conv_dgrad_block_run(const void* g, int g_kind, int N, int OH, int OW, int Cout, const void* w2, int w_kind, size_t ldw, int Cin,
+                         int kh, int kw, int sh, int sw, int pad_top, int pad_left, int H, int W, const int32_t* ib_g,
+                         const int32_t* ib_w, int exp_const, const void* gs, int gs_kind, int Cout_s, const void* ws, int ws_kind,
+                         size_t ldws, const int32_t* ib_gs, const int32_t* ib_ws, int exp_short, float* dx, size_t ldc,
+                         const float* addend, void* stream);
+
 bool conv_wgrad_ldg_ok(int C, int Cout, int kh, int kw);
 int conv_wgrad_ldg_run(const void* src, int src_kind, int N, int H, int W, int C, const void* g, int g_kind, int Cout, int kh, int kw,
                        int sh, int sw, int pt, int pl, int OH, int OW, int64_t* acc64, int alpha, void* stream);
diff --git a/lbt_b200/dfxp.py b/lbt_b200/dfxp.py
--- a/lbt_b200/dfxp.py
+++ b/lbt_b200/dfxp.py
@@ -613,7 +613,7 @@
         G.gemm_i8(A, wt, ibA=ibx, ibB=ibw, exp_const=e, bias=bq, out=out2d, bnq=gbnq)
 
 
-def _conv_backward(layer, geom, xm, xkind, wm, prep, gm, need_dx, need_dw, need_db, addend=None, link=None):
+def _conv_backward(layer, geom, xm, xkind, wm, prep, gm, need_dx, need_dw, need_db, addend=None, link=None, shortcut=None):
     N, H, W, Cin, Cout, kh, kw, sh, sw, pt, pl, OH, OW = geom
     xb, wb, gb = layer.qX.bits, layer.qW.bits, layer.qG.bits
     dev = gm.device
@@ -720,11 +720,16 @@
             else:
                 perm = torch.tensor(_class_perm(kh, kw, sh, sw), device=dev)
                 w2 = _as_operand(wm.view(kh * kw, Cin, Cout).index_select(0, perm).permute(1, 0, 2).reshape(Cin, K2))
-            _lib.call('lbt_conv_i8_dgrad_strided', _lib.ptr(gm), Q.MANT_S8, N, OH, OW, Cout, _lib.ptr(w2),
-                      Q.MANT_S8 | (_W_PREPARED if pw2 is not None else 0), w2.stride(0),
-                      Cin, kh, kw, sh, sw, pt, pl, H, W, _lib.ptr(layer.qG.range), _lib.ptr(layer.qW.range), int(e),
-                      _lib.ptr(dx), Cin, _lib.ptr(ad2), _lib.stream(),
-                      meta=dict(ops=2 * N * OH * OW * Cin * K2, bytes=N * OH * OW * Cout * min(sh * sw, kh * kw) + Cin * K2 + N * H * W * Cin * 4))
+            done = shortcut is not None and addend is None and _dgrad_block(layer, geom, gm, w2, pw2 is not None, e, dx, shortcut)
+            if not done:
+                if shortcut is not None:
+                    ad2 = _shortcut_dgrad(shortcut).reshape(N * H * W, Cin)
+                _lib.call('lbt_conv_i8_dgrad_strided', _lib.ptr(gm), Q.MANT_S8, N, OH, OW, Cout, _lib.ptr(w2),
+                          Q.MANT_S8 | (_W_PREPARED if pw2 is not None else 0), w2.stride(0),
+                          Cin, kh, kw, sh, sw, pt, pl, H, W, _lib.ptr(layer.qG.range), _lib.ptr(layer.qW.range), int(e),
+                          _lib.ptr(dx), Cin, _lib.ptr(ad2), _lib.stream(),
+                          meta=dict(ops=2 * N * OH * OW * Cin * K2,
+                                    bytes=N * OH * OW * Cout * min(sh * sw, kh * kw) + Cin * K2 + N * H * W * Cin * 4))
         else:
             w2 = pw2 if pw2 is not None else _as_operand(wm.view(kh * kw, Cin, Cout).permute(1, 0, 2).reshape(Cin, K2))
             A2 = _im2col(gm, Q.MANT_S8, H, W, kh, kw, sh, sw, pt, pl, True)
@@ -734,6 +739,59 @@
             t.record_stream(side)
         rt._side_pending = True
     return dx, dW, db
+
+
+FUSE_BLOCK_DGRAD = os.environ.get('LBT_FUSE_BLOCK_DGRAD', '1') != '0'
+_block_dgrad_count = 0
+
+
+class _BlockDgrad:
+
+    def __init__(self):
+        self.armed = False
+        self.parked = None
+
+    def take(self):
+        p, self.parked = self.parked, None
+        return p
+
+
+def _block_dgrad_ok(layer, geom, prep):
+    N, H, W, Cin, Cout, kh, kw, sh, sw, pt, pl, OH, OW = geom
+    if (sh, sw) == (1, 1) or layer.qG.bits > 8:
+        return False
+    if layer.implicit and _gather_ok(Cout, Cin, kh, kw) and sh <= 4 and sw <= 4:
+        return False
+    return bool(prep['classes'] if prep is not None else _dgrad_classes_ok(layer, Cin, Cout, kh, kw, sh, sw))
+
+
+def _shortcut_dgrad(parked):
+    layer, geom, xkind, wm, prep, gm = parked
+    dx, _, _ = _conv_backward(layer, geom, None, xkind, wm, prep, gm, True, False, False)
+    return dx
+
+
+def _dgrad_block(layer, geom, gm, w2, w_prepared, e, dx, shortcut):
+    global _block_dgrad_count
+    N, H, W, Cin, Cout, kh, kw, sh, sw, pt, pl, OH, OW = geom
+    sl, sgeom, _, swm, sprep, sgm = shortcut
+    sN, sH, sW, sCin, sCout, skh, skw, ssh, ssw, spt, spl, sOH, sOW = sgeom
+    if (sN, sH, sW, sCin) != (N, H, W, Cin) or (skh, skw, ssh, ssw, spt, spl) != (1, 1, sh, sw, 0, 0):
+        return False
+    spw2 = sprep['w2'] if sprep is not None else None
+    sw2 = spw2 if spw2 is not None else _as_operand(swm.view(Cin, sCout))
+    se = -(sl.qG.bits - 1) - (sl.qW.bits - 1)
+    K2 = kh * kw * Cout
+    done = _lib.try_call('lbt_conv_i8_dgrad_block', _lib.ptr(gm), Q.MANT_S8, N, OH, OW, Cout, _lib.ptr(w2),
+                         Q.MANT_S8 | (_W_PREPARED if w_prepared else 0), w2.stride(0), Cin, kh, kw, sh, sw, pt, pl, H, W,
+                         _lib.ptr(layer.qG.range), _lib.ptr(layer.qW.range), int(e), _lib.ptr(sgm), Q.MANT_S8, sOH, sOW, sCout,
+                         _lib.ptr(sw2), Q.MANT_S8 | (_W_PREPARED if spw2 is not None else 0), sw2.stride(0),
+                         _lib.ptr(sl.qG.range), _lib.ptr(sl.qW.range), int(se), _lib.ptr(dx), Cin, None, _lib.stream(),
+                         meta=dict(ops=2 * N * OH * OW * Cin * K2 + 2 * N * sOH * sOW * Cin * sCout,
+                                   bytes=N * OH * OW * Cout + N * sOH * sOW * sCout + Cin * (K2 + sCout) + N * H * W * Cin * 4))
+    if done:
+        _block_dgrad_count += 1
+    return done
 
 
 def _check_layer_bits(who, bits, grad_bits):
@@ -1300,7 +1358,7 @@
 
     @staticmethod
     def forward(ctx, x, weight, gamma, beta, add, conv, bn, relu, next_site, next_kind, want_fp32, alias, link_in, link_out, pool=None,
-                next2=None, running=False):
+                next2=None, running=False, block=None):
         geom = _conv_geom(conv, x, weight)
         N, H, W, Cin, Cout, kh, kw, sh, sw, pt, pl, OH, OW = geom
         norm, resc = bn[0], bn[1]
@@ -1352,6 +1410,14 @@
         ctx.conv, ctx.bn, ctx.geom, ctx.xkind, ctx.prep = conv, bn, geom, xkind, prep
         ctx.relu_mode, ctx.has_add = relu_mode, add is not None
         ctx.link_in, ctx.link_out = link_in, link_out
+        ctx.block = None
+        if block is not None and not running:
+            if alias:
+                block.armed = conv.qG.bits <= 8 and _block_dgrad_ok(conv, geom, prep)
+                ctx.block = block if block.armed else None
+            elif block.armed:
+                ctx.block = block
+        ctx.block_first = bool(alias)
         if link_out is not None and out is None and not running:
             link_out.offer(bn, k1, k2, gq, bq, relu_mode, add is not None)
         ctx.pool = None
@@ -1396,15 +1462,35 @@
         _, gm, dgamma, dbeta, d_add = _bn_backward(ctx.bn, _to_mem(g) if pre is None else None, k1, k2, sums, gq, bq, out,
                                                    ctx.relu_mode, ctx.has_add, grad_site=conv.qG, want_dx=False, pre=pre,
                                                    pool=pool)
-        addend = _to_mem(g_alias) if (g_alias is not None and need_dx) else None
-        li = ctx.link_in if (addend is None and FUSE_BWD_LINK) else None
+        bd = ctx.block
+        if bd is not None and not ctx.block_first:
+            ctx.block = None
+            if need_dx and not isinstance(gm, tuple):
+                _, dW, _ = _conv_backward(conv, ctx.geom, xm, ctx.xkind, wm, ctx.prep, gm, False, need_dw, False)
+                bd.parked = (conv, ctx.geom, ctx.xkind, wm, ctx.prep, gm)
+                N, H, W, Cin = ctx.geom[:4]
+                dx = torch.empty(1, dtype=torch.float32, device=gm.device).expand(N, H, W, Cin)
+                return ((_from_mem(dx),) + (dW, dgamma, dbeta, (_from_mem(d_add) if d_add is not None else None)) + (None,) * 13)
+        parked = bd.take() if (bd is not None and need_dx) else None
+        shortcut = None
+        if parked is not None:
+            if not isinstance(gm, tuple) and _block_dgrad_ok(conv, ctx.geom, ctx.prep):
+                shortcut = parked
+                addend = None
+            else:
+                addend = _shortcut_dgrad(parked)
+        else:
+            addend = _to_mem(g_alias) if (g_alias is not None and need_dx) else None
+        ctx.block = None
+        li = ctx.link_in if (addend is None and shortcut is None and FUSE_BWD_LINK) else None
         if isinstance(gm, tuple):
             dx, dW, _ = _conv_backward16(conv, ctx.geom, xm, ctx.xkind, wm, ctx.prep, gm[0], gm[1], need_dx, need_dw, False, addend=addend)
         else:
-            dx, dW, _ = _conv_backward(conv, ctx.geom, xm, ctx.xkind, wm, ctx.prep, gm, need_dx, need_dw, False, addend=addend, link=li)
+            dx, dW, _ = _conv_backward(conv, ctx.geom, xm, ctx.xkind, wm, ctx.prep, gm, need_dx, need_dw, False, addend=addend, link=li,
+                                       shortcut=shortcut)
         return ((_from_mem(dx) if dx is not None else None), dW, dgamma, dbeta,
                 (_from_mem(d_add) if d_add is not None else None), None, None, None, None, None, None, None, None, None, None, None,
-                None)
+                None, None)
 
 
 FUSE_POOL = os.environ.get('LBT_FUSE_POOL', '0') == '1'
@@ -1422,7 +1508,7 @@
 
 
 def conv_bn_unit(conv, bn, x, add=None, relu=False, next_conv=None, want_fp32=True, alias=False, link_in=None, link_out=None,
-                 pool=None):
+                 pool=None, block=None):
     relu = relu or getattr(bn, 'relu', False)
     running = isinstance(bn, BatchNorm2d_q) and bn._running(x, add, conv.weight)
     if not _unit_fusable(conv, bn, x, running):
@@ -1460,10 +1546,12 @@
             next2 = [s2, k2_, None]
     if next_site is None or add is not None or pool is not None:
         want_fp32 = True
-    use_alias = bool(alias and x.requires_grad and not getattr(x, '_lbt_hollow', False) and conv.weight.shape[2] <= 128)
+    block = block if (FUSE_BLOCK_DGRAD and not running) else None
+    use_alias = bool(alias and x.requires_grad and not getattr(x, '_lbt_hollow', False) and
+                     (conv.weight.shape[2] <= 128 or (block is not None and tuple(conv.stride) != (1, 1) and conv.qG.bits <= 8)))
     out, nm, xa = _ConvBNFn.apply(x, conv.weight, bn[1].gamma, bn[1].beta, add, conv, bn, relu, next_site, next_kind,
                                   want_fp32, use_alias, link_in if FUSE_BWD_LINK else None, link_out if FUSE_BWD_LINK else None,
-                                  pgeom, next2, running)
+                                  pgeom, next2, running, block)
     if next_site is not None and nm.numel():
         out._lbt_q = {id(next_site): (nm, next_kind)}
         if next2 is not None and next2[2] is not None:
@@ -1847,14 +1935,15 @@
                                            for i in range(0, len(res), 2))
         if paired:
             link = _BwdLink()
-            r, xs = conv_bn_unit(res[0], res[1], x, next_conv=res[2], want_fp32=False, alias=True, link_out=link)
+            bd = _BlockDgrad() if len(sc_layers) == 2 and tuple(res[0].stride) != (1, 1) else None
+            r, xs = conv_bn_unit(res[0], res[1], x, next_conv=res[2], want_fp32=False, alias=True, link_out=link, block=bd)
             if xs is not x and getattr(x, '_lbt_q', None) is not None:
                 xs._lbt_q = x._lbt_q
             for i in range(2, len(res) - 2, 2):
                 nxt = _BwdLink()
                 r = conv_bn_unit(res[i], res[i + 1], r, next_conv=res[i + 2], want_fp32=False, link_in=link, link_out=nxt)
                 link = nxt
-            sc = conv_bn_unit(sc_layers[0], sc_layers[1], xs) if len(sc_layers) == 2 else self.shortcut(xs)
+            sc = conv_bn_unit(sc_layers[0], sc_layers[1], xs, block=bd) if len(sc_layers) == 2 else self.shortcut(xs)
             return conv_bn_unit(res[-2], res[-1], r, add=sc, relu=True, next_conv=next_conv, link_in=link)
         r = x
         for m in res[:-1]:
```

Result: faster. 33870, median of 6 (+4.5%).
